# npit/video-learning-tf

Measured on AMD Instinct MI355X. Metric: clips/sec (16-frame 227x227) LRCN train step, higher is better.
Workload: dtype f32; 1 GPU; LRCN AlexNet(fc6)+LSTM(256) 16-frame 227x227x3 clips, 101 classes, UCF-101-shaped synthetic, full train step; global_batch=64, clips_per_gpu=64, frames_per_clip=16, parallelism=dp1, optimizer=sgd+clip_by_global_norm(10), init=reference (sigma 0.05), dist_world_size=1

## Files before the change

### include/vltf.h

```cpp
#ifndef VLTF_H
#define VLTF_H

#include <stddef.h>
#include <stdint.h>

#ifdef __cplusplus
extern "C" {
#endif

typedef void* vl_stream_t;
typedef struct vl_conv_desc vl_conv_desc;

typedef struct vl_step_state {
    int64_t step;
    float lr;
    uint32_t tag_origin;
    float adam_lr;
    uint32_t reserved[3];
} vl_step_state;

const char* vl_last_error(void);
int vl_version(void);
int vl_device_count(void);

int vl_input_prep_u8(const uint8_t* src, float* dst, int n, int raw_h, int raw_w, int out_h, int out_w,
                     const int32_t* crop_y, const int32_t* crop_x, const uint8_t* mirror,
                     const float* mean_bgr, int dst_halo, int dst_phase, vl_stream_t stream);
int vl_nhwc_to_nchw(const float* src, float* dst, int n, int h, int w, int c, int dst_halo, int dst_phase, vl_stream_t stream);
int vl_nchw_to_nhwc(const float* src, float* dst, int n, int c, int h, int w, vl_stream_t stream);

int vl_conv_create(vl_conv_desc** out, int cin, int h, int w, int cout, int kh, int kw, int stride, int groups);
void vl_conv_destroy(vl_conv_desc* d);
int vl_conv_out_hw(const vl_conv_desc* d, int* oh, int* ow);
int vl_conv_set_halo(vl_conv_desc* d, int x_halo, int y_halo, int dy_halo, int dx_halo);
int vl_conv_set_x_phase_split(vl_conv_desc* d, int on);
int vl_conv_x_phase(const vl_conv_desc* d);
int vl_set_conv_math(int math);
int vl_conv_math(void);
int vl_conv_fwd(const vl_conv_desc* d, const float* x, const float* w_hwio, const float* bias, float* y,
                int n, int relu, vl_stream_t stream);
int vl_conv_wt_transpose(const vl_conv_desc* d, const float* w_hwio, float* wt, vl_stream_t stream);
int vl_conv_dgrad(const vl_conv_desc* d, const float* dy, const float* wt, float* dx, const float* relu_mask,
                  int n, vl_stream_t stream);
size_t vl_conv_wgrad_ws_bytes(const vl_conv_desc* d, int n);
int vl_conv_wgrad_fuses_bias(const vl_conv_desc* d);
int vl_conv_wgrad(const vl_conv_desc* d, const float* x, const float* dy, float* dw, float* db, void* ws,
                  size_t ws_bytes, int n, vl_stream_t stream);
size_t vl_c8_bytes(int n, int c, int h, int w, int halo);
int vl_pack_c8(const float* x, void* xb, int n, int c, int h, int w, int x_halo, int xb_halo, vl_stream_t stream);
size_t vl_conv_c8_w_bytes(const vl_conv_desc* d, int bwd);
int vl_conv_c8_pack_w(const vl_conv_desc* d, const float* w_hwio, void* wb, int bwd, vl_stream_t stream);
int vl_conv_c8_fwd(vl_conv_desc* d, const void* xb, const void* wb, const float* bias, float* y, void* yb, int n, int relu,
                   vl_stream_t stream);
int vl_conv_c8_dgrad(vl_conv_desc* d, const void* dyb, const void* wbt, float* dx, void* dxb, const float* relu_mask,
                     const void* relu_mask_c8, int n, vl_stream_t stream);
size_t vl_conv_c8_wgrad_ws_bytes(const vl_conv_desc* d, int n);
int vl_conv_c8_wgrad(vl_conv_desc* d, const void* xb, const void* dyb, float* dw, void* ws, size_t ws_bytes, int n,
                     vl_stream_t stream);
int vl_bias_grad_c8(const void* dyb, float* db, float* ws, int n, int c, int h, int w, int halo, vl_stream_t stream);
int vl_pack_kc8(const float* src, void* dst, int64_t positions, int channels, int64_t pos_stride, int64_t ch_stride, vl_stream_t stream);
size_t vl_gemm_kc8_ws_bytes(int m, int n, int k);
int vl_gemm_kc8(const void* a_kc8, const void* b_kc8, float* c, int m, int n, int k, const float* bias, int relu, void* ws,
                size_t ws_bytes, vl_stream_t stream);
int vl_s2d_c8_from_x0(const vl_conv_desc* d, const float* x0, void* xb, int n, vl_stream_t stream);
int vl_input_prep_u8_s2d(const vl_conv_desc* d, const uint8_t* src, void* xb, int n, int raw_h, int raw_w, const int32_t* crop_y,
                         const int32_t* crop_x, const uint8_t* mirror, const float* mean_bgr, vl_stream_t stream);
int vl_s2d_weights(const vl_conv_desc* d, const float* src, float* dst, int grad, vl_stream_t stream);
int vl_bias_grad_nchw(const float* dy, float* db, float* ws, int n, int c, int hw, vl_stream_t stream);

int vl_lrn_fwd(const float* x, float* y, int n, int c, int hw, int radius, float alpha, float beta, float bias,
               vl_stream_t stream);
int vl_lrn_bwd(const float* x, const float* dy, float* dx, int n, int c, int hw, int radius, float alpha,
               float beta, float bias, int relu_fused, int w, int dx_halo, vl_stream_t stream);

int vl_pool_lrn_bwd(const float* x, const float* dp, const uint8_t* argmax, float* dx, int n, int c, int h, int w,
                    int p_halo, int radius, float alpha, float beta, float bias, int relu_fused, int dx_halo,
                    vl_stream_t stream);

int vl_pool_lrn_bwd_c8(const void* x, int x_packed, const float* dp, const uint8_t* argmax, void* dxb, int n, int c, int h, int w,
                       int p_halo, int radius, float alpha, float beta, float bias, int relu_fused, int dxb_halo, vl_stream_t stream);

int vl_pool_lrn_bwd_test_ranges(int ranges);

int vl_lrn_pool_fwd(const float* x, float* p, uint8_t* argmax, int n, int c, int h, int w, int p_halo, int radius,
                    float alpha, float beta, float bias, vl_stream_t stream);

int vl_lrn_pool_fwd_c8(const void* x, int x_packed, void* pb, uint8_t* argmax, int n, int c, int h, int w, int p_halo, int radius,
                       float alpha, float beta, float bias, vl_stream_t stream);

int vl_maxpool_fwd(const float* x, float* y, uint8_t* argmax, int n, int c, int h, int w, int k, int s,
                   int64_t ys_n, int64_t ys_c, int64_t ys_h, int64_t ys_w, vl_stream_t stream);
int vl_maxpool_bwd(const float* dy, const uint8_t* argmax, float* dx, const float* relu_mask, int n, int c,
                   int h, int w, int k, int s, int64_t ys_n, int64_t ys_c, int64_t ys_h, int64_t ys_w,
                   int dx_halo, vl_stream_t stream);

int vl_gemm(int transa, int transb, int m, int n, int k, const float* a, int64_t lda, const float* b, int64_t ldb,
            float* c, int64_t ldc, const float* bias, int relu, const float* relu_mask, void* ws, size_t ws_bytes,
            vl_stream_t stream);
size_t vl_gemm_split_ws_bytes(int m, int n, int k);
int vl_colsum(const float* a, int64_t lda, float* out, float* ws, int m, int n, vl_stream_t stream);

int vl_lstm_step_fwd(const float* gx, const float* gh, float* act, float* cseq, float* hseq, float* hprev,
                     int batch, int T, int t, int H, float forget_bias, vl_stream_t stream);
int vl_lstm_step_bwd(const float* dout, const float* dh_next, const float* act, const float* cseq, float* dc,
                     float* dz, int batch, int T, int t, int H, vl_stream_t stream);

size_t vl_lstm_seq_ws_bytes(int batch, int T, int H);
int vl_lstm_seq_fwd(const float* gx, const float* kh, const float* h0, const float* c0, float* act, float* cseq, float* hseq,
                    float* hprev, int batch, int T, int H, float forget_bias, void* ws, size_t ws_bytes, vl_stream_t stream);
int vl_lstm_seq_bwd(const float* dout, const float* kh, const float* act, const float* cseq, const float* c0, float* dz,
                    float* dh0, float* dc0, int batch, int T, int H, void* ws, size_t ws_bytes, vl_stream_t stream);
size_t vl_lstm_seq_tag_span(int batch, int T, int H);
int vl_lstm_seq_fwd_st(const float* gx, const float* kh, const float* h0, const float* c0, float* act, float* cseq, float* hseq,
                       float* hprev, int batch, int T, int H, float forget_bias, void* ws, size_t ws_bytes, const vl_step_state* state,
                       uint32_t tag_offset, vl_stream_t stream);
int vl_lstm_seq_bwd_st(const float* dout, const float* kh, const float* act, const float* cseq, const float* c0, float* dz,
                       float* dh0, float* dc0, int batch, int T, int H, void* ws, size_t ws_bytes, const vl_step_state* state,
                       uint32_t tag_offset, vl_stream_t stream);
int vl_lstm_seq_ws_clear(void* ws, size_t ws_bytes, vl_stream_t stream);
int vl_lstm_seq_status(void* ws, int* timed_out);
int vl_lstm_seq_test_hooks(unsigned spin_limit, int mute_workgroup);
int vl_transpose(const float* src, int64_t ld, float* dst, int rows, int cols, vl_stream_t stream);

int vl_temporal_fusion_fwd(const float* x, float* y, int batch, int T, int H, int method, vl_stream_t stream);
int vl_temporal_fusion_bwd(const float* dy, float* dx, int batch, int T, int H, int method, vl_stream_t stream);

typedef struct vl_resize_desc vl_resize_desc;
int vl_resize_create(vl_resize_desc** out, int h, int w, int oh, int ow, int channels);
void vl_resize_destroy(vl_resize_desc* d);
size_t vl_resize_tmp_bytes(const vl_resize_desc* d, int n);
int vl_resize_u8(const vl_resize_desc* d, const uint8_t* src, uint8_t* tmp, uint8_t* dst, int n, vl_stream_t stream);

int vl_copy2d(const float* src, int64_t src_ld, float* dst, int64_t dst_ld, int rows, int cols, vl_stream_t stream);
int vl_eltwise2(const float* a, const float* b, float* out, int64_t count, int op, vl_stream_t stream);
int vl_max2_grad(const float* a, const float* b, const float* d, float* da, float* db, int64_t count, vl_stream_t stream);
int vl_fuse_n(const float* const* ins, int n, float* out, int64_t count, int op, vl_stream_t stream);
int vl_fuse_n_grad(const float* const* ins, int n, const float* d, float* const* dins, int64_t count, int op, vl_stream_t stream);

int vl_dropout_fwd(const float* x, float* y, uint8_t* mask, int64_t count, float keep, uint64_t seed, vl_stream_t stream);
int vl_dropout_bwd(const float* dy, const uint8_t* mask, float* dx, int64_t count, float keep, vl_stream_t stream);
int vl_dropout_fwd_st(const float* x, float* y, uint8_t* mask, int64_t count, float keep, const vl_step_state* state,
                      vl_stream_t stream);

int vl_softmax_xent(const float* logits, const int32_t* labels, float* dlogits, float* stats, float* rows,
                    int batch, int classes, float grad_scale, vl_stream_t stream);

int vl_sumsq(const float* g, int64_t count, float* out, float* ws, int accumulate, vl_stream_t stream);
int vl_sgd_apply(float* w, const float* g, int64_t count, float lr, float clip_norm, const float* sumsq,
                 float gscale, const uint32_t* skip, vl_stream_t stream);
int vl_adam_apply(float* w, const float* g, float* m, float* v, int64_t count, float lr, float clip_norm,
                  const float* sumsq, float gscale, int step, const uint32_t* skip, vl_stream_t stream);
int vl_status_or(uint32_t* dst, const void* lstm_ws, int init, vl_stream_t stream);

size_t vl_step_state_bytes(void);
int vl_step_state_set(vl_step_state* state, int64_t step, float lr, uint32_t tag_origin, vl_stream_t stream);
int vl_sgd_apply_st(float* w, const float* g, int64_t count, const vl_step_state* state, float clip_norm, const float* sumsq,
                    float gscale, const uint32_t* skip, vl_stream_t stream);
int vl_adam_apply_st(float* w, const float* g, float* m, float* v, int64_t count, const vl_step_state* state, float clip_norm,
                     const float* sumsq, float gscale, const uint32_t* skip, vl_stream_t stream);

int vl_fill(float* p, int64_t count, float value, vl_stream_t stream);
int vl_relu_grad(float* d, const float* y, int64_t count, vl_stream_t stream);

#ifdef __cplusplus
}
#endif
#endif
```

### video-learning-tf_amd/_ffi.py

```python
import ctypes as C
import os

_HERE = os.path.dirname(os.path.abspath(__file__))
LIB_PATH = os.environ.get("VLTF_HIP_LIB") or os.path.join(_HERE, "libvltf_hip.so")

p = C.c_void_p
i32, i64, f32, u32, u64, sz = C.c_int, C.c_int64, C.c_float, C.c_uint32, C.c_uint64, C.c_size_t

SIGNATURES = {
    "vl_last_error": (C.c_char_p, []),
    "vl_version": (i32, []),
    "vl_device_count": (i32, []),
    "vl_input_prep_u8": (i32, [p, p, i32, i32, i32, i32, i32, p, p, p, p, i32, i32, p]),
    "vl_nhwc_to_nchw": (i32, [p, p, i32, i32, i32, i32, i32, i32, p]),
    "vl_nchw_to_nhwc": (i32, [p, p, i32, i32, i32, i32, p]),
    "vl_conv_create": (i32, [C.POINTER(p), i32, i32, i32, i32, i32, i32, i32, i32]),
    "vl_conv_destroy": (None, [p]),
    "vl_conv_out_hw": (i32, [p, C.POINTER(i32), C.POINTER(i32)]),
    "vl_conv_set_halo": (i32, [p, i32, i32, i32, i32]),
    "vl_conv_set_x_phase_split": (i32, [p, i32]),
    "vl_conv_x_phase": (i32, [p]),
    "vl_set_conv_math": (i32, [i32]),
    "vl_conv_math": (i32, []),
    "vl_gemm_split_ws_bytes": (C.c_size_t, [i32, i32, i32]),
    "vl_conv_fwd": (i32, [p, p, p, p, p, i32, i32, p]),
    "vl_conv_wt_transpose": (i32, [p, p, p, p]),
    "vl_conv_dgrad": (i32, [p, p, p, p, p, i32, p]),
    "vl_conv_wgrad_ws_bytes": (sz, [p, i32]),
    "vl_conv_wgrad_fuses_bias": (i32, [p]),
    "vl_conv_wgrad": (i32, [p, p, p, p, p, p, sz, i32, p]),
    "vl_c8_bytes": (sz, [i32, i32, i32, i32, i32]),
    "vl_pack_c8": (i32, [p, p, i32, i32, i32, i32, i32, i32, p]),
    "vl_conv_c8_w_bytes": (sz, [p, i32]),
    "vl_conv_c8_pack_w": (i32, [p, p, p, i32, p]),
    "vl_conv_c8_fwd": (i32, [p, p, p, p, p, p, i32, i32, p]),
    "vl_conv_c8_dgrad": (i32, [p, p, p, p, p, p, p, i32, p]),
    "vl_pack_kc8": (i32, [p, p, i64, i32, i64, i64, p]),
    "vl_gemm_kc8_ws_bytes": (sz, [i32, i32, i32]),
    "vl_gemm_kc8": (i32, [p, p, p, i32, i32, i32, p, i32, p, sz, p]),
    "vl_s2d_c8_from_x0": (i32, [p, p, p, i32, p]),
    "vl_input_prep_u8_s2d": (i32, [p, p, p, i32, i32, i32, p, p, p, p, p]),
    "vl_s2d_weights": (i32, [p, p, p, i32, p]),
    "vl_bias_grad_c8": (i32, [p, p, p, i32, i32, i32, i32, i32, p]),
    "vl_conv_c8_wgrad_ws_bytes": (sz, [p, i32]),
    "vl_conv_c8_wgrad": (i32, [p, p, p, p, p, sz, i32, p]),
    "vl_bias_grad_nchw": (i32, [p, p, p, i32, i32, i32, p]),
    "vl_lrn_fwd": (i32, [p, p, i32, i32, i32, i32, f32, f32, f32, p]),
    "vl_lrn_bwd": (i32, [p, p, p, i32, i32, i32, i32, f32, f32, f32, i32, i32, i32, p]),
    "vl_lrn_pool_fwd": (i32, [p, p, p, i32, i32, i32, i32, i32, i32, f32, f32, f32, p]),
    "vl_pool_lrn_bwd": (i32, [p, p, p, p, i32, i32, i32, i32, i32, i32, f32, f32, f32, i32, i32, p]),
    "vl_pool_lrn_bwd_test_ranges": (i32, [i32]),
    "vl_lrn_pool_fwd_c8": (i32, [p, i32, p, p, i32, i32, i32, i32, i32, i32, f32, f32, f32, p]),
    "vl_pool_lrn_bwd_c8": (i32, [p, i32, p, p, p, i32, i32, i32, i32, i32, i32, f32, f32, f32, i32, i32, p]),
    "vl_maxpool_fwd": (i32, [p, p, p, i32, i32, i32, i32, i32, i32, i64, i64, i64, i64, p]),
    "vl_maxpool_bwd": (i32, [p, p, p, p, i32, i32, i32, i32, i32, i32, i64, i64, i64, i64, i32, p]),
    "vl_gemm": (i32, [i32, i32, i32, i32, i32, p, i64, p, i64, p, i64, p, i32, p, p, sz, p]),
    "vl_colsum": (i32, [p, i64, p, p, i32, i32, p]),
    "vl_lstm_step_fwd": (i32, [p, p, p, p, p, p, i32, i32, i32, i32, f32, p]),
    "vl_lstm_step_bwd": (i32, [p, p, p, p, p, p, i32, i32, i32, i32, p]),
    "vl_lstm_seq_ws_bytes": (sz, [i32, i32, i32]),
    "vl_lstm_seq_fwd": (i32, [p, p, p, p, p, p, p, p, i32, i32, i32, f32, p, sz, p]),
    "vl_lstm_seq_bwd": (i32, [p, p, p, p, p, p, p, p, i32, i32, i32, p, sz, p]),
    "vl_lstm_seq_tag_span": (sz, [i32, i32, i32]),
    "vl_lstm_seq_fwd_st": (i32, [p, p, p, p, p, p, p, p, i32, i32, i32, f32, p, sz, p, u32, p]),
    "vl_lstm_seq_bwd_st": (i32, [p, p, p, p, p, p, p, p, i32, i32, i32, p, sz, p, u32, p]),
    "vl_lstm_seq_ws_clear": (i32, [p, sz, p]),
    "vl_lstm_seq_status": (i32, [p, C.POINTER(i32)]),
    "vl_lstm_seq_test_hooks": (i32, [C.c_uint, i32]),
    "vl_transpose": (i32, [p, i64, p, i32, i32, p]),
    "vl_temporal_fusion_fwd": (i32, [p, p, i32, i32, i32, i32, p]),
    "vl_temporal_fusion_bwd": (i32, [p, p, i32, i32, i32, i32, p]),
    "vl_dropout_fwd": (i32, [p, p, p, i64, f32, u64, p]),
    "vl_dropout_bwd": (i32, [p, p, p, i64, f32, p]),
    "vl_dropout_fwd_st": (i32, [p, p, p, i64, f32, p, p]),
    "vl_softmax_xent": (i32, [p, p, p, p, p, i32, i32, f32, p]),
    "vl_sumsq": (i32, [p, i64, p, p, i32, p]),
    "vl_sgd_apply": (i32, [p, p, i64, f32, f32, p, f32, p, p]),
    "vl_adam_apply": (i32, [p, p, p, p, i64, f32, f32, p, f32, i32, p, p]),
    "vl_status_or": (i32, [p, p, i32, p]),
    "vl_step_state_bytes": (sz, []),
    "vl_step_state_set": (i32, [p, i64, f32, u32, p]),
    "vl_sgd_apply_st": (i32, [p, p, i64, p, f32, p, f32, p, p]),
    "vl_adam_apply_st": (i32, [p, p, p, p, i64, p, f32, p, f32, p, p]),
    "vl_fill": (i32, [p, i64, f32, p]),
    "vl_resize_create": (i32, [C.POINTER(p), i32, i32, i32, i32, i32]),
    "vl_resize_destroy": (None, [p]),
    "vl_resize_tmp_bytes": (sz, [p, i32]),
    "vl_resize_u8": (i32, [p, p, p, p, i32, p]),
    "vl_copy2d": (i32, [p, i64, p, i64, i32, i32, p]),
    "vl_eltwise2": (i32, [p, p, p, i64, i32, p]),
    "vl_max2_grad": (i32, [p, p, p, p, p, i64, p]),
    "vl_fuse_n": (i32, [p, i32, p, i64, i32, p]),
    "vl_fuse_n_grad": (i32, [p, i32, p, p, i64, i32, p]),
    "vl_relu_grad": (i32, [p, p, i64, p]),
}


class VltfError(RuntimeError):
    pass


_lib = None


def lib():
    global _lib
    if _lib is None:
        if not os.path.exists(LIB_PATH):
            raise VltfError("libvltf_hip.so not found at %s -- build it with "
                            "`python -c 'import __graft_entry__ as g; g.build()'` "
                            "(there is no CPU fallback)" % LIB_PATH)
        import torch
        tl = os.path.join(os.path.dirname(torch.__file__), "lib", "libamdhip64.so")
        if os.path.exists(tl):
            C.CDLL(tl, mode=C.RTLD_GLOBAL)
        try:
            l = C.CDLL(LIB_PATH)
        except OSError as ex:
            raise VltfError("cannot load %s: %s" % (LIB_PATH, ex))
        for name, (res, args) in SIGNATURES.items():
            try:
                fn = getattr(l, name)
            except AttributeError:
                raise VltfError("libvltf_hip.so does not export %s (stale build?)" % name)
            fn.restype = res
            fn.argtypes = args
        _lib = l
    return _lib


def check(rc, what):
    if rc != 0:
        msg = lib().vl_last_error()
        raise VltfError("%s failed (rc=%d): %s" % (what, rc, msg.decode() if msg else "?"))


def call(name, *args):
    check(getattr(lib(), name)(*args), name)
```

### video-learning-tf_amd/csrc/conv_desc.h

```cpp
#pragma once
#include <hip/hip_runtime.h>
#include <stdint.h>

struct vl_conv_desc {
    int cin, h, w, cout, kh, kw, stride, groups;
    int oh, ow, pt, pl, pb, pr;
    int cig, cog;
    int K;
    int Kd;
    int x_halo, y_halo, dy_halo, dx_halo;
    int x_phase;
    int2* ktab2_fwd;
    int* ktab_fwd;
    int2* ptab2_fwd;
    int2* ptab2_bwd;
    int* ptab_fwd;
    int* ptab_bwd;
    int* rowtab_fwd;
    int* rowtab_bwd;
    int fwd_padded, bwd_padded;
    uint32_t* wsplit_fwd;
    uint32_t* wsplit_bwd;
    int* c8_toff_fwd;
    int* c8_toff_bwd;
};

void conv_c8_free_tables(vl_conv_desc* d);
int conv_c8_build_tables(vl_conv_desc* d);
```

### video-learning-tf_amd/csrc/mfma_gemm.hip

```cpp
#include <stdlib.h>
#include <string.h>

#include "common.h"
#include "conv_desc.h"

typedef float f32x16 __attribute__((ext_vector_type(16)));
typedef const __attribute__((address_space(4))) int* const_int_ptr;
__device__ __forceinline__ const_int_ptr as_const(const int* p) { return (const_int_ptr)(uintptr_t)p; }
static constexpr int NT = 256;
static constexpr int KBLK = 16;

static constexpr uint32_t OOB_OFF = 0xF0000000u;
static constexpr int64_t MAX_BUF_BYTES = 0xE0000000ll;

__device__ __forceinline__ __amdgpu_buffer_rsrc_t make_rsrc(const float* base, int64_t bytes) {
    return __builtin_amdgcn_make_buffer_rsrc(const_cast<float*>(base), 0, (int)(uint32_t)bytes, 0x00020000);
}
__device__ __forceinline__ float buf_load(__amdgpu_buffer_rsrc_t r, uint32_t voff, int soff) {
    return __builtin_bit_cast(float, __builtin_amdgcn_raw_buffer_load_b32(r, (int)voff, soff, 0));
}

template <int BX, int BR>
struct LdsTile {
    static constexpr int STR = BR + 2;
// ... 565 lines not shown
}
struct SplitBf16 {
    i32x4 p[3];
};
template <int NPC>
__device__ __forceinline__ void split_pieces(float x0, float x1, int (&out)[3]) {
    f32x2 r = {x0, x1};
#pragma unroll
    for (int k = 0; k < NPC; ++k) {
        const uint32_t h = __builtin_bit_cast(uint32_t, __builtin_convertvector(r, bf16x2));
        out[k] = (int)h;
        if (k + 1 < NPC) r = f32x2{r[0] - __uint_as_float(h << 16), r[1] - __uint_as_float(h & 0xffff0000u)};
    }
}
__device__ constexpr int kProdA[6] = {0, 0, 1, 1, 0, 2};
__device__ constexpr int kProdB[6] = {0, 1, 0, 1, 2, 0};
constexpr int split_products(int math) { return math == 6 ? 6 : math == 3 ? 3 : 1; }
constexpr int split_pieces_of(int math) { return math == 6 ? 3 : math == 3 ? 2 : 1; }
__device__ __forceinline__ f32x16 mfma_bf16(const i32x4& a, const i32x4& b, const f32x16& c) {
    return __builtin_amdgcn_mfma_f32_32x32x16_bf16(__builtin_bit_cast(bf16x8, a), __builtin_bit_cast(bf16x8, b), c, 0, 0, 0);
}

template <int BN, int WM, int WN, int MATH = 0, bool X4 = false>
__global__ __launch_bounds__(NT, 1) void wgrad_dma_kernel(const ConvGeom g, const DyParams d, const EpiRowMajor::Params pe,
                                                          int tiles_i, int tiles_j, int groups, int units, int rtiles,
                                                          int rt_per_split, float* db_slabs, int db_stride) {
    using C = WgradDmaCfg<BN>;
    constexpr int BM = C::BM, STR = C::STR, SA = BM * STR, BUF = C::BUF;
    constexpr int TM = BM / WM / 32, TN = BN / WN / 32;
    constexpr int RA = BM / 4, RB = BN / 4;
    static_assert(WM * WN == 4 && TM * WM * 32 == BM && TN * WN * 32 == BN, "tile shape");
    static_assert(RA + RB <= 10 * 2 * TM * TN, "row fetches must leave the last third of a tile's MFMAs to cover their latency");
    static_assert(!X4 || (MATH != 0 && BN == 128 && BM == 128), "the 16-byte fetch form: split-product modes, 128 x 128 tiles");
    constexpr int GSTR = 258, SA4 = 32 * GSTR, BUF4 = 64 * GSTR;
    extern __shared__ __attribute__((aligned(16))) float ldsw[];

    const int tiles = tiles_i * tiles_j;
    const int k8 = blockIdx.x >> 3;
    const int unit = (k8 / tiles) * 8 + (blockIdx.x & 7);
    if (unit >= units) return;
    const int tile_id = k8 % tiles;
    const int ti_blk = tile_id % tiles_i, tj_blk = tile_id / tiles_i;
    const int zg = unit % groups, zs = unit / groups;
    const int i0 = ti_blk * BM, j0 = tj_blk * BN;
    const int lane = threadIdx.x & 63;
    const int wave = __builtin_amdgcn_readfirstlane(threadIdx.x >> 6);
    const int wi0 = (wave / WN) * (BM / WM), wj0 = (wave % WN) * (BN / WN);

    const i32x4 rs_x = rsrc_words(g.x + (int64_t)zg * g.grp_stride, (g.total - (int64_t)zg * g.grp_stride) * 4);
    const int64_t goff = (int64_t)zg * d.Cog * d.plane;
    const i32x4 rs_dy = rsrc_words(d.dy + goff, (d.total - goff) * 4);
    const int* tab = g.ktab + i0 + wave * RA;
    const uint32_t lds0 = (uint32_t)(uintptr_t)(__attribute__((address_space(3))) float*)ldsw;
    const int row_bytes = (int)(d.plane * 4);
    const int b_row0 = j0 + wave * RB;
    const int b_last = d.Cog - 1;
    const int64_t dy_img = (int64_t)d.Cout_total * d.plane;

    uint32_t voff_x, voff_dy;
    auto decode = [&](int rt) __attribute__((always_inline)) {
        const int m = X4 ? rt * 64 + 4 * (lane & 15) : rt * 64 + lane;
        const bool vm = m < g.M;
        const uint32_t mm = vm ? m : 0;
        const uint32_t n = fd_div(mm, g.dOHW);
        const uint32_t p = mm - n * g.OHW;
        const uint32_t oh = fd_div(p, g.dOW);
        const uint32_t ow = p - oh * g.OW;
        const int ih0 = (int)oh * g.stride - g.pt + g.halo, iw0 = (int)ow * g.col_mul + g.col_add;
        const uint32_t vx = (uint32_t)((int64_t)n * g.img_stride + (int64_t)ih0 * g.Wp + iw0) * 4u;
        const uint32_t vd = (uint32_t)((int64_t)n * dy_img + (int64_t)(oh + d.halo) * d.OWp + ow + d.halo) * 4u;
        voff_x = vm ? vx : OOB_OFF;
        voff_dy = vm ? vd : OOB_OFF;
        asm volatile("" : "+v"(voff_x), "+v"(voff_dy));
    };
    int tabv[RA];
    auto load_table = [&](int rt) __attribute__((always_inline)) {
        const const_int_ptr tt = (const_int_ptr)(uintptr_t)(tab + rt * g.zero);
#pragma unroll
        for (int f = 0; f < RA; ++f) tabv[f] = tt[f];
    };
    auto pin_table = [&]() __attribute__((always_inline)) {
#pragma unroll
        for (int f = 0; f < RA; ++f) asm volatile("" : "+s"(tabv[f]));
    };
    auto dma = [&](const int nb, const int f, int rt_next) __attribute__((always_inline)) {
        const int z = rt_next * g.zero;
        if (f < RA) {
            const uint32_t la = lds0 + (uint32_t)(wave * (RA * STR) + z) * 4u;
            lds_dma_row(rs_x, la + (uint32_t)(nb * BUF + f * STR) * 4u, voff_x, tabv[f]);
        } else {
            const int r = f - RA;
            const uint32_t lb = lds0 + (uint32_t)(SA + wave * (RB * STR) + z) * 4u;
            lds_dma_row(rs_dy, lb + (uint32_t)(nb * BUF + r * STR) * 4u, voff_dy, min(b_row0 + z + r, b_last) * row_bytes);
        }
    };
    uint32_t vrow_a[8], vrow_b[8];
    if constexpr (X4) {
#pragma unroll
        for (int j = 0; j < 8; ++j) {
            const int rl = wave * 8 + j + 32 * (lane >> 4);
            vrow_a[j] = i0 + rl < g.K ? (uint32_t)g.ktab[i0 + rl] : OOB_OFF;
            vrow_b[j] = j0 + rl < d.Cog ? (uint32_t)(j0 + rl) * (uint32_t)row_bytes : OOB_OFF;
        }
    }
    auto dma_x4 = [&](const int nb, const int f, int rt_next) __attribute__((always_inline)) {
        const int z = rt_next * g.zero;
        if (f < 8) {
            const uint32_t vo = (vrow_a[f] == OOB_OFF || voff_x == OOB_OFF) ? OOB_OFF : vrow_a[f] + voff_x;
            lds_dma_row4(rs_x, lds0 + (uint32_t)(nb * BUF4 + (wave * 8 + f) * GSTR + z) * 4u, vo, 0);
        } else {
            const uint32_t vo = (vrow_b[f - 8] == OOB_OFF || voff_dy == OOB_OFF) ? OOB_OFF : vrow_b[f - 8] + voff_dy;
            lds_dma_row4(rs_dy, lds0 + (uint32_t)(nb * BUF4 + SA4 + (wave * 8 + f - 8) * GSTR + z) * 4u, vo, 0);
        }
    };
    const int ones_row = (db_slabs != nullptr && g.K >= i0 && g.K < i0 + BM) ? g.K - i0 : -1;
    auto finish_tile = [&](const int nb) __attribute__((always_inline)) {
        asm volatile("s_waitcnt vmcnt(0)" ::: "memory");
        if constexpr (X4) {
            if (ones_row >= 0 && ((ones_row & 31) >> 3) == wave) ldsw[nb * BUF4 + (ones_row & 31) * GSTR + (ones_row >> 5) * 64 + lane] = 1.0f;
        } else {
            if (ones_row >= 0 && (ones_row / RA) == wave) ldsw[nb * BUF + ones_row * STR + lane] = 1.0f;
        }
        __syncthreads();
    };

    f32x16 acc[TM][TN];
#pragma unroll
    for (int a = 0; a < TM; ++a)
#pragma unroll
        for (int b = 0; b < TN; ++b)
#pragma unroll
            for (int q = 0; q < 16; ++q) acc[a][b][q] = 0.f;

    const int rt0 = zs * rt_per_split;
    const int rt1 = min(rtiles, rt0 + rt_per_split);
    const int ntiles = rt1 - rt0;
    if (ntiles > 0) {
        decode(rt0);
        load_table(rt0);
        pin_table();
        if constexpr (X4) {
#pragma unroll
            for (int f = 0; f < 16; ++f) dma_x4(0, f, rt0);
        } else {
#pragma unroll
            for (int f = 0; f < RA + RB; ++f) dma(0, f, rt0);
        }
        decode(rt0 + 1);
        finish_tile(0);
    }
    const float* fa = ldsw + (wi0 + (lane & 31)) * STR + 2 * (lane >> 5);
    const float* fb = ldsw + SA + (wj0 + (lane & 31)) * STR + 2 * (lane >> 5);

    auto tile = [&](const int cur, int rt_next) __attribute__((always_inline)) {
        float2 af[2][TM], bf[2][TN];
#pragma unroll
        for (int a = 0; a < TM; ++a) af[0][a] = *reinterpret_cast<const float2*>(fa + cur * BUF + a * 32 * STR);
#pragma unroll
        for (int b = 0; b < TN; ++b) bf[0][b] = *reinterpret_cast<const float2*>(fb + cur * BUF + b * 32 * STR);
#pragma unroll
        for (int t = 0; t < 16; ++t) {
            const int c = t & 1, nx = c ^ 1;
            if (t + 1 < 16) {
#pragma unroll
                for (int a = 0; a < TM; ++a) af[nx][a] = *reinterpret_cast<const float2*>(fa + cur * BUF + a * 32 * STR + 4 * (t + 1));
#pragma unroll
                for (int b = 0; b < TN; ++b) bf[nx][b] = *reinterpret_cast<const float2*>(fb + cur * BUF + b * 32 * STR + 4 * (t + 1));
            }
#pragma unroll
            for (int m = 0; m < 2 * TM * TN; ++m) {
                const int a = (m % (TM * TN)) / TN, b = m % TN;
                if (m < TM * TN) acc[a][b] = __builtin_amdgcn_mfma_f32_32x32x2f32(af[c][a].x, bf[c][b].x, acc[a][b], 0, 0, 0);
                else acc[a][b] = __builtin_amdgcn_mfma_f32_32x32x2f32(af[c][a].y, bf[c][b].y, acc[a][b], 0, 0, 0);
                const int f = t * (2 * TM * TN) + m;
                if (f < RA + RB) {
                    dma(cur ^ 1, f, rt_next);
                    __builtin_amdgcn_sched_barrier(0);
                }
            }
            if (t == 10) {
                load_table(rt_next + 1);
                __builtin_amdgcn_sched_barrier(0);
            }
            if (t == 13) {
                int rtn = rt_next + 1;
                asm volatile("" : "+s"(rtn));
                decode(rtn);
                pin_table();
                __builtin_amdgcn_sched_barrier(0);
            }
        }
        finish_tile(cur ^ 1);
    };
    const float* fa3 = ldsw + (wi0 + (lane & 31)) * STR + 8 * (lane >> 5);
    const float* fb3 = ldsw + SA + (wj0 + (lane & 31)) * STR + 8 * (lane >> 5);
    auto tile_split = [&](const int cur, int rt_next) __attribute__((always_inline)) {
        constexpr int NP = split_products(MATH), NPC = split_pieces_of(MATH);
        constexpr int NMS = NP * TM * TN, NTOT = 4 * NMS, NF = X4 ? 16 : RA + RB;
        constexpr int FSPAN = NTOT >= 28 ? NTOT - 14 : NTOT / 2;
        constexpr int FPM = (NF + FSPAN - 1) / FSPAN, FEND = (NF + FPM - 1) / FPM;
        constexpr int LT = FEND > NTOT - 12 ? FEND : NTOT - 12;
        constexpr int PIN = LT + 2 > NTOT - 6 ? LT + 2 : NTOT - 6;
        static_assert(PIN < NTOT, "the tile must leave room to load and pin the next table");
        SplitBf16 As[2][TM], Bs[2][TN];
        auto load_split = [&](const int st, SplitBf16 (&A)[TM], SplitBf16 (&B)[TN]) __attribute__((always_inline)) {
#pragma unroll
            for (int a = 0; a < TM; ++a)
#pragma unroll
                for (int q = 0; q < 4; ++q) {
                    const float2 v = X4 ? *reinterpret_cast<const float2*>(ldsw + cur * BUF4 + (lane & 31) * GSTR + (wi0 / 32 + a) * 64 + 16 * st +
                                                                            8 * (lane >> 5) + 2 * q)
                                        : *reinterpret_cast<const float2*>(fa3 + cur * BUF + a * 32 * STR + 16 * st + 2 * q);
                    int pc[3] = {0, 0, 0};
                    split_pieces<NPC>(v.x, v.y, pc);
#pragma unroll
                    for (int k = 0; k < NPC; ++k) A[a].p[k][q] = pc[k];
                }
#pragma unroll
            for (int b = 0; b < TN; ++b)
#pragma unroll
                for (int q = 0; q < 4; ++q) {
                    const float2 v = X4 ? *reinterpret_cast<const float2*>(ldsw + cur * BUF4 + SA4 + (lane & 31) * GSTR + (wj0 / 32 + b) * 64 +
                                                                            16 * st + 8 * (lane >> 5) + 2 * q)
                                        : *reinterpret_cast<const float2*>(fb3 + cur * BUF + b * 32 * STR + 16 * st + 2 * q);
                    int pc[3] = {0, 0, 0};
                    split_pieces<NPC>(v.x, v.y, pc);
#pragma unroll
                    for (int k = 0; k < NPC; ++k) B[b].p[k][q] = pc[k];
                }
        };
        load_split(0, As[0], Bs[0]);
        static_for<0, 4>([&](auto SI) __attribute__((always_inline)) {
            constexpr int st = decltype(SI)::value, c = st & 1;
            if constexpr (st + 1 < 4) load_split(st + 1, As[c ^ 1], Bs[c ^ 1]);
            static_for<0, NMS>([&](auto MI) __attribute__((always_inline)) {
                constexpr int m = decltype(MI)::value;
                constexpr int prod = m / (TM * TN), a = (m % (TM * TN)) / TN, b = m % TN;
                acc[a][b] = mfma_bf16(As[c][a].p[kProdA[prod]], Bs[c][b].p[kProdB[prod]], acc[a][b]);
                constexpr int idx = st * NMS + m;
                static_for<0, FPM>([&](auto EI) __attribute__((always_inline)) {
                    constexpr int f = idx * FPM + decltype(EI)::value;
                    if constexpr (f < NF) {
                        if constexpr (X4) dma_x4(cur ^ 1, f, rt_next);
                        else dma(cur ^ 1, f, rt_next);
                    }
                });
                __builtin_amdgcn_sched_barrier(0x106);
                if constexpr (idx == LT) load_table(rt_next + 1);
                if constexpr (idx == PIN) {
                    int rtn = rt_next + 1;
                    asm volatile("" : "+s"(rtn));
                    decode(rtn);
                    pin_table();
                }
            });
        });
        finish_tile(cur ^ 1);
    };
    auto run_tile = [&](const int cur, int rt_next) __attribute__((always_inline)) {
        if constexpr (MATH != 0) tile_split(cur, rt_next);
        else tile(cur, rt_next);
    };
    int rt = rt0;
    for (int i = 0; i + 1 < ntiles; i += 2, rt += 2) {
        run_tile(0, rt + 1);
        run_tile(1, rt + 2);
    }
    if (ntiles > 0 && (ntiles & 1)) run_tile(0, rt + 1);

    EpiRowMajor::template apply<TM, TN>(pe, zg, zs, i0 + wi0, j0 + wj0, acc);
    if (ones_row >= 0) {
        float* dbs = db_slabs + (int64_t)zs * db_stride + zg * d.Cog;
        const int lr = ones_row - wi0;
        if (lr >= 0 && lr < BM / WM) {
            const int a = lr >> 5, rr = lr & 31;
            const int q = (rr & 3) + 4 * (rr >> 3);
            if (((rr >> 2) & 1) == (lane >> 5)) {
#pragma unroll
                for (int b = 0; b < TN; ++b) {
                    const int j = j0 + wj0 + 32 * b + (lane & 31);
                    float v = 0.f;
#pragma unroll
                    for (int aa = 0; aa < TM; ++aa)
#pragma unroll
                        for (int qq = 0; qq < 16; ++qq)
                            if (aa == a && qq == q) v = acc[aa][b][qq];
                    if (j < d.Cog) dbs[j] = v;
                }
            }
        }
    }
}

typedef float f32x4 __attribute__((ext_vector_type(4)));
typedef float f32x4u __attribute__((ext_vector_type(4), aligned(4)));

struct ConvDmaParams {
    const float* w;
    int64_t w_ld;
    int64_t w_grp_stride;
    int64_t w_bytes;
    const int* row_tab;
    int nblk;
};

template <int SR>
__global__ __launch_bounds__(NT, 64 / SR) void conv_dma_kernel(const ConvDmaParams pa, const ConvGeom g, const EpiConvNCHW::Params pe,
                                                               int tiles_i, int wide) {
    constexpr int BM = 128, BN = 128;
    constexpr int ABUF = SR * BM, BUF = SR * (BM + BN);
    constexpr int RW = SR / 4;
    constexpr int NF = RW * 4;
    constexpr int NT2 = SR / 4;
    constexpr int FPM = 1;
    static_assert(SR == 64 || SR == 32, "stage depth");
    extern __shared__ __attribute__((aligned(16))) float ldsc[];
    const int bid = xcd_swizzle(blockIdx.x, gridDim.x);
    const int ti_blk = bid % tiles_i, tj_blk = bid / tiles_i;
    const int zg = blockIdx.y;
    const int i0 = ti_blk * BM, j0 = tj_blk * BN;
    const int lane = threadIdx.x & 63;
    const int wave = __builtin_amdgcn_readfirstlane(threadIdx.x >> 6);
    const int wm = wave >> 1, wn = wave & 1;

    const i32x4 rs_w = rsrc_words(pa.w + (int64_t)zg * pa.w_grp_stride, pa.w_bytes - (int64_t)zg * pa.w_grp_stride * 4);
    const i32x4 rs_x = rsrc_words(g.x + (int64_t)zg * g.grp_stride, (g.total - (int64_t)zg * g.grp_stride) * 4);
    uint32_t voff_a[2], voff_b[2];
#pragma unroll
    for (int hf = 0; hf < 2; ++hf) {
        const int co = i0 + hf * 64 + lane;
        voff_a[hf] = co < pe.Cog ? (uint32_t)co * 4u : OOB_OFF;
        const int m = j0 + hf * 64 + lane;
        const bool vm = m < g.M;
        const uint32_t mm = vm ? m : 0;
        const uint32_t n = fd_div(mm, g.dOHW);
        const uint32_t p = mm - n * g.OHW;
        const uint32_t oh = fd_div(p, g.dOW);
        const uint32_t ow = p - oh * g.OW;
        const int ih0 = (int)oh * g.stride - g.pt + g.halo, iw0 = (int)ow * g.col_mul + g.col_add;
        voff_b[hf] = vm ? (uint32_t)((int64_t)n * g.img_stride + (int64_t)ih0 * g.Wp + iw0) * 4u : OOB_OFF;
    }
    const uint32_t lds0 = (uint32_t)(uintptr_t)(__attribute__((address_space(3))) float*)ldsc;
    const int ld_bytes = (int)(pa.w_ld * 4);

    int tabv[RW];
    int row0 = 0;
    bool blk_ok = false;
    const int wrow = wave * RW;
    auto load_table = [&](int st) {
        const int k0 = st * SR + wrow;
        const const_int_ptr tt = as_const(g.ktab) + k0 + st * g.zero;
#pragma unroll
        for (int f = 0; f < RW; ++f) tabv[f] = tt[f];
        row0 = as_const(pa.row_tab)[k0 / KBLK + st * g.zero] + k0 % KBLK;
        blk_ok = k0 / KBLK < pa.nblk;
    };
    auto pin_table = [&]() {
#pragma unroll
        for (int f = 0; f < RW; ++f) asm volatile("" : "+s"(tabv[f]));
        asm volatile("" : "+s"(row0));
    };
    auto dma = [&](const int nb, const int f, int st) {
        const int rr = f >> 2, kind = f & 3, hf = kind & 1;
        const int z = st * g.zero;
        const uint32_t row_lds = lds0 + (uint32_t)(nb * BUF + (wrow + rr) * 128 + hf * 64 + z) * 4u;
        const bool live = blk_ok && st * SR + wrow + rr < g.K;
        if (kind < 2) lds_dma_row(rs_w, row_lds, voff_a[hf], min(row0 + rr, g.K - 1) * ld_bytes);
        else lds_dma_row(rs_x, row_lds + ABUF * 4u, live ? voff_b[hf] : OOB_OFF, tabv[rr]);
    };
    int a_soff = 0;
    auto dma_fast = [&](const int nb, const int f, int st) {
        const int rr = f >> 2, kind = f & 3, hf = kind & 1;
        const uint32_t row_lds = lds0 + (uint32_t)(nb * BUF + (wrow + rr) * 128 + hf * 64 + st * g.zero) * 4u;
        if (f == 0) a_soff = row0 * ld_bytes;
        if (kind < 2) lds_dma_row(rs_w, row_lds, voff_a[hf], a_soff);
        else lds_dma_row(rs_x, row_lds + ABUF * 4u, voff_b[hf], tabv[rr]);
        if (kind == 1) a_soff += ld_bytes;
    };
    auto finish_stage = [&]() {
        asm volatile("s_waitcnt vmcnt(0)" ::: "memory");
        __syncthreads();
    };

    f32x16 acc[2][2];
#pragma unroll
    for (int a = 0; a < 2; ++a)
#pragma unroll
        for (int b = 0; b < 2; ++b)
#pragma unroll
            for (int q = 0; q < 16; ++q) acc[a][b][q] = 0.f;

    const int nstages = (pa.nblk * KBLK + SR - 1) / SR;
    load_table(0);
    pin_table();
#pragma unroll
    for (int f = 0; f < NF; ++f) dma(0, f, 0);
    load_table(1);
    pin_table();
    finish_stage();

    float bias_r[2][16];
#pragma unroll
    for (int a = 0; a < 2; ++a)
#pragma unroll
        for (int q = 0; q < 16; ++q) {
            const int co = i0 + wm * 64 + 2 * ((q & 3) + 8 * (q >> 2) + 4 * (lane >> 5)) + a;
            bias_r[a][q] = (pe.bias && co < pe.Cog) ? pe.bias[zg * pe.Cog + co] : 0.f;
        }

    const float* fa = ldsc + (lane >> 5) * 128 + wm * 64 + 2 * (lane & 31);
    const float* fb = ldsc + ABUF + (lane >> 5) * 128 + wn * 64 + (lane & 31);

    auto stage = [&](const int cur, const bool fast, int st_next) {
        float2 af[2], bf[2], an[2], bn[2];
        auto read_b = [&](int step) {
            const float* q = fb + cur * BUF + step * 256;
            return float2{q[0], q[32]};
        };
        af[0] = *reinterpret_cast<const float2*>(fa + cur * BUF);
        bf[0] = read_b(0);
        af[1] = *reinterpret_cast<const float2*>(fa + cur * BUF + 256);
        bf[1] = read_b(1);
#pragma unroll
        for (int t = 0; t < NT2; ++t) {
            if (t + 1 < NT2) {
#pragma unroll
                for (int u = 0; u < 2; ++u) {
                    an[u] = *reinterpret_cast<const float2*>(fa + cur * BUF + (2 * (t + 1) + u) * 256);
                    bn[u] = read_b(2 * (t + 1) + u);
                }
            }
#pragma unroll
            for (int m = 0; m < 8; ++m) {
                const int u = m >> 2, a = (m >> 1) & 1, b = m & 1;
                acc[a][b] = __builtin_amdgcn_mfma_f32_32x32x2f32(a ? af[u].y : af[u].x, b ? bf[u].y : bf[u].x, acc[a][b], 0, 0, 0);
                const int f = (t * 8 + m) * FPM;
                if (f < NF) {
#pragma unroll
                    for (int e = 0; e < FPM; ++e) {
                        if (fast) dma_fast(cur ^ 1, f + e, st_next);
                        else dma(cur ^ 1, f + e, st_next);
                    }
                    __builtin_amdgcn_sched_barrier(0);
                }
            }
            static_assert(NF / FPM / 8 <= NT2 - 4, "fetches must end before the table is replaced");
            if (t == NT2 - 4) {
                load_table(st_next + 1);
                __builtin_amdgcn_sched_barrier(0);
            }
            if (t == NT2 - 2) {
                pin_table();
                __builtin_amdgcn_sched_barrier(0);
            }
#pragma unroll
            for (int u = 0; u < 2; ++u) {
                af[u] = an[u];
                bf[u] = bn[u];
            }
        }
        finish_stage();
    };
    const int nfull = g.K / SR;
    int st = 0;
    for (; st + 2 < nfull; st += 2) {
        stage(0, true, st + 1);
        stage(1, true, st + 2);
    }
    for (; st < nstages; ++st) {
        if (st & 1) stage(1, false, st + 1);
        else stage(0, false, st + 1);
    }

    if (wide) {
        constexpr int SP = BN + 4;
        float* T = ldsc;
#pragma unroll
        for (int b = 0; b < 2; ++b)
#pragma unroll
            for (int a = 0; a < 2; ++a)
#pragma unroll
                for (int q = 0; q < 16; ++q) {
                    const int i = (q & 3) + 8 * (q >> 2) + 4 * (lane >> 5);
                    float v = acc[a][b][q] + bias_r[a][q];
                    if (pe.relu) v = fmaxf(v, 0.f);
                    T[(wm * 64 + 2 * i + a) * SP + wn * 64 + 32 * b + (lane & 31)] = v;
                }
        __syncthreads();
        const int px = 4 * (lane & 31);
        const int m = j0 + px;
        const uint32_t n = fd_div((uint32_t)min(m, pe.M - 1), pe.dOHW);
        const int p = m - (int)n * pe.OHW;
        const bool run4 = m + 3 < pe.M && p + 3 < pe.OHW;
        const int64_t cbase = ((int64_t)n * pe.Cout_total + (int64_t)zg * pe.Cog) * pe.y_plane + p;
#pragma unroll
        for (int i = 0; i < BM / 8; ++i) {
            const int cl = wave * (BM / 4) + 2 * i + (lane >> 5);
            const int co = i0 + cl;
            const f32x4 v = *reinterpret_cast<const f32x4*>(T + cl * SP + px);
            if (co >= pe.Cog) continue;
            float* dst = pe.y + cbase + (int64_t)co * pe.y_plane;
            if (run4) {
                *reinterpret_cast<f32x4u*>(dst) = v;
            } else {
#pragma unroll
                for (int e = 0; e < 4; ++e) {
                    const int me = m + e;
                    if (me < pe.M) {
                        const uint32_t ne = fd_div((uint32_t)me, pe.dOHW);
                        const int pe_ = me - (int)ne * pe.OHW;
                        pe.y[((int64_t)ne * pe.Cout_total + (int64_t)zg * pe.Cog + co) * pe.y_plane + pe_] = v[e];
                    }
                }
            }
        }
        return;
    }
#pragma unroll
    for (int b = 0; b < 2; ++b) {
        const int m = j0 + wn * 64 + 32 * b + (lane & 31);
        if (m >= pe.M) continue;
        const uint32_t n = fd_div((uint32_t)m, pe.dOHW);
        const uint32_t p = m - n * pe.OHW;
        const uint32_t oh = fd_div(p, pe.dOW);
        const uint32_t ow = p - oh * pe.OW;
        const int64_t c0 = (int64_t)n * pe.Cout_total + (int64_t)zg * pe.Cog;
        const int64_t ybase = c0 * pe.y_plane + (int64_t)(oh + pe.y_halo) * pe.y_wp + ow + pe.y_halo;
        const int64_t mbase = c0 * pe.m_plane + (int64_t)(oh + pe.m_halo) * pe.m_wp + ow + pe.m_halo;
#pragma unroll
        for (int a = 0; a < 2; ++a) {
            float mk[16];
            if (pe.mask) {
#pragma unroll
                for (int q = 0; q < 16; ++q) {
                    const int co = i0 + wm * 64 + 2 * ((q & 3) + 8 * (q >> 2) + 4 * (lane >> 5)) + a;
                    mk[q] = co < pe.Cog ? pe.mask[mbase + (int64_t)co * pe.m_plane] : 0.f;
                }
            }
#pragma unroll
            for (int q = 0; q < 16; ++q) {
                const int i = (q & 3) + 8 * (q >> 2) + 4 * (lane >> 5);
                const int co = i0 + wm * 64 + 2 * i + a;
                if (co < pe.Cog) {
                    float v = acc[a][b][q] + bias_r[a][q];
                    if (pe.relu) v = fmaxf(v, 0.f);
                    if (pe.mask) v = mk[q] > 0.f ? v : 0.f;
                    pe.y[ybase + (int64_t)co * pe.y_plane] = v;
                }
            }
        }
    }
}


__global__ void conv_wsplit_kernel(const float* __restrict__ w, int64_t w_ld, int64_t w_grp_stride, const int* __restrict__ row_tab,
                                   int K, int Cog, int CogP, int nstages, int planes, uint32_t* __restrict__ out) {
    const int st = blockIdx.x, zg = blockIdx.y;
    const int row0 = row_tab[st];
    uint32_t* o = out + ((int64_t)zg * nstages + st) * planes * 8 * CogP;
    for (int idx = threadIdx.x; idx < 8 * CogP; idx += blockDim.x) {
        const int q = idx & 3, co = (idx >> 2) % CogP, h = idx / (4 * CogP);
        const int r = 8 * h + 2 * q, p = st * 16 + r;
        float x0 = 0.f, x1 = 0.f;
        if (co < Cog) {
            const float* src = w + (int64_t)(row0 + r) * w_ld + zg * w_grp_stride + co;
            if (p < K) x0 = src[0];
            if (p + 1 < K) x1 = src[w_ld];
        }
        int pc[3] = {0, 0, 0};
        split_pieces<3>(x0, x1, pc);
        for (int k = 0; k < planes; ++k) o[(int64_t)((2 * k + h) * CogP + co) * 4 + q] = (uint32_t)pc[k];
    }
}

struct ConvRingParams {
    const uint32_t* wsplit;
    int CogP;
    int nstages;
};

template <int MATH, int BM>
__global__ __launch_bounds__(512, 1) void conv_ring_kernel(const ConvRingParams pa, const ConvGeom g, const EpiConvNCHW::Params pe,
                                                           int tiles_i, int OWp, int Mp, FastDiv dOHWp, FastDiv dOWp) {
    constexpr int BN = BM == 128 ? 256 : 512, SR = 16, NBUF = BM == 128 ? 5 : 4;
    constexpr int NH = BN / 256;
    static_assert(BM == 128 || BM == 64, "channel tile");
    constexpr int NPL = MATH == 6 ? 3 : 2;
    constexpr int ABUF = NPL * 8 * BM, BUF = ABUF + SR * BN;
    constexpr int NAF = (NPL * 2 * (BM / 64) + 7) / 8;
    constexpr int FW = NAF + 2 * NH;
    constexpr int VMW = (NBUF - 3) * FW;
    constexpr int NP = split_products(MATH), NPC = split_pieces_of(MATH);
    constexpr int NM = (BM / 32) * (BN / 256) * NP;
    static_assert(SR == KBLK, "one stage = one block of the reduction order");
    extern __shared__ __attribute__((aligned(16))) float ldsr[];
    const int bid = xcd_swizzle(blockIdx.x, gridDim.x);
    const int ti_blk = bid % tiles_i, tj_blk = bid / tiles_i;
    const int zg = blockIdx.y;
    const int i0 = ti_blk * BM, j0 = tj_blk * BN;
    const int lane = threadIdx.x & 63;
    const int wave = __builtin_amdgcn_readfirstlane(threadIdx.x >> 6);
    constexpr int TA = BM / 32, TB = BN / 8 / 32, WPX = 32 * TB;
    const int OHWp = g.OHW / g.OW * OWp;
    const int nstages = pa.nstages;

    const int64_t stage_dw = (int64_t)NPL * 8 * pa.CogP;
    const uint32_t* wbase = pa.wsplit + (int64_t)zg * nstages * stage_dw;
    const i32x4 rs_w = rsrc_words(reinterpret_cast<const float*>(wbase), nstages * stage_dw * 4);
    constexpr int NPIECE = NPL * 2 * (BM / 64);
    int piece[NAF];
    uint32_t voff_a[NAF];
#pragma unroll
    for (int e = 0; e < NAF; ++e) {
        piece[e] = e == 0 ? wave % NPIECE : 8 + (wave & 3);
        voff_a[e] = BM == 128 ? (uint32_t)(((piece[e] >> 1) * pa.CogP + i0 + (piece[e] & 1) * 64 + lane) * 16)
                              : (uint32_t)((piece[e] * pa.CogP + i0 + lane) * 16);
    }
    const int stage_bytes = (int)(stage_dw * 4);
    const i32x4 rs_x = rsrc_words(g.x + (int64_t)zg * g.grp_stride, (g.total - (int64_t)zg * g.grp_stride) * 4);
    uint32_t voff_b[NH];
#pragma unroll
    for (int hf = 0; hf < NH; ++hf) {
        const int m = j0 + 256 * hf + 4 * lane;
        const bool vm = m < Mp;
        const uint32_t mm = vm ? m : 0;
        const uint32_t n = fd_div(mm, dOHWp);
        const uint32_t p = mm - n * OHWp;
        const uint32_t oh = fd_div(p, dOWp);
        const uint32_t ow = p - oh * OWp;
        const int ih0 = (int)oh * g.stride - g.pt + g.halo, iw0 = (int)ow * g.col_mul + g.col_add;
        voff_b[hf] = vm ? (uint32_t)((int64_t)n * g.img_stride + (int64_t)ih0 * g.Wp + iw0) * 4u : OOB_OFF;
    }
    const uint32_t lds0 = (uint32_t)(uintptr_t)(__attribute__((address_space(3))) float*)ldsr;

    int tab0 = 0, tab1 = 0;
    const int wrow = wave * 2;
    auto load_table = [&](int st) __attribute__((always_inline)) {
        const int sc = min(st, nstages - 1) + st * g.zero;
        const const_int_ptr tt = as_const(g.ktab) + sc * SR + wrow;
        tab0 = tt[0];
        tab1 = tt[1];
    };
    auto pin_table = [&]() __attribute__((always_inline)) {
        asm volatile("" : "+s"(tab0));
        asm volatile("" : "+s"(tab1));
    };
    auto dma = [&](const uint32_t wr, const int f, int st) __attribute__((always_inline)) {
        if (f < NAF) {
            lds_dma_row4(rs_w, lds0 + wr + (uint32_t)piece[f] * 1024u, voff_a[f], st * stage_bytes);
        } else {
            const int r = (f - NAF) / NH, hf = (f - NAF) % NH;
            const bool live = st * SR + wrow + r < g.K;
            lds_dma_row4(rs_x, lds0 + wr + (uint32_t)(ABUF + (wrow + r) * BN + 256 * hf) * 4u, live ? voff_b[hf] : OOB_OFF,
                         r == 0 ? tab0 : tab1);
        }
    };
    auto dma_fast = [&](const uint32_t wr, const int f, int st) __attribute__((always_inline)) {
        if (f < NAF) {
            lds_dma_row4(rs_w, lds0 + wr + (uint32_t)piece[f] * 1024u, voff_a[f], st * stage_bytes);
        } else {
            const int r = (f - NAF) / NH, hf = (f - NAF) % NH;
            lds_dma_row4(rs_x, lds0 + wr + (uint32_t)(ABUF + (wrow + r) * BN + 256 * hf) * 4u, voff_b[hf], r == 0 ? tab0 : tab1);
        }
    };

    f32x16 acc[TA][TB];
#pragma unroll
    for (int a = 0; a < TA; ++a)
#pragma unroll
        for (int b = 0; b < TB; ++b)
#pragma unroll
            for (int q = 0; q < 16; ++q) acc[a][b][q] = 0.f;

    const float* fa = ldsr + ((lane >> 5) * BM + (lane & 31)) * 4;
    const float* fb = ldsr + ABUF + (lane >> 5) * 8 * BN + wave * WPX + (lane & 31);
    struct Raw {
        float b[TB][8];
    };
    auto load_raw = [&](int rd, Raw& r) __attribute__((always_inline)) {
#pragma unroll
        for (int j = 0; j < 8; ++j) {
            const float* q = fb + rd + j * BN;
#pragma unroll
            for (int b = 0; b < TB; ++b) r.b[b][j] = q[32 * b];
        }
    };
    auto load_a = [&](int rd, SplitBf16 (&A)[TA]) __attribute__((always_inline)) {
#pragma unroll
        for (int a = 0; a < TA; ++a) {
#pragma unroll
            for (int k = 0; k < NPC; ++k) A[a].p[k] = *reinterpret_cast<const i32x4*>(fa + rd + k * 2 * BM * 4 + a * 32 * 4);
        }
    };
    auto split = [&](const Raw& r, SplitBf16 (&B)[TB]) __attribute__((always_inline)) {
#pragma unroll
        for (int j = 0; j < 4; ++j)
#pragma unroll
            for (int b = 0; b < TB; ++b) {
                int pc[3] = {0, 0, 0};
                split_pieces<NPC>(r.b[b][2 * j], r.b[b][2 * j + 1], pc);
#pragma unroll
                for (int k = 0; k < NPC; ++k) B[b].p[k][j] = pc[k];
            }
    };

    for (int s0 = 0; s0 < NBUF; ++s0) {
        load_table(s0);
        pin_table();
        if (s0 < nstages) {
#pragma unroll
            for (int f = 0; f < FW; ++f) dma((uint32_t)(s0 * BUF * 4), f, s0);
        }
    }
    load_table(NBUF);
    pin_table();
    if (nstages >= NBUF) asm volatile("s_waitcnt vmcnt(%0)" ::"n"(VMW) : "memory");
    else asm volatile("s_waitcnt vmcnt(0)" ::: "memory");
    __syncthreads();
    SplitBf16 A[TA] = {}, B[TB] = {}, An[TA] = {}, Bn[TB] = {};
    Raw R0 = {}, R1 = {};
    load_a(0, A);
    load_raw(0, R0);
    load_raw(BUF, R1);
    split(R0, B);
    asm volatile("s_waitcnt lgkmcnt(0)" ::: "memory");
    __syncthreads();

    int rda = BUF, rdb = 2 * BUF;
    uint32_t wr = 0;
    constexpr int D = NBUF;
    auto stage = [&](const bool fast, int st, SplitBf16 (&Ac)[TA], SplitBf16 (&Bc)[TB], SplitBf16 (&An)[TA], SplitBf16 (&Bn)[TB],
                     const Raw& Rc, Raw& Rn) __attribute__((always_inline)) {
        load_a(rda, An);
        load_raw(rdb, Rn);
        static_for<0, (NM > FW ? NM : FW)>([&](auto MI) __attribute__((always_inline)) {
            constexpr int m = decltype(MI)::value;
            if constexpr (m < NM) {
                constexpr int prod = m / (TA * TB), a = (m % (TA * TB)) / TB, b = m % TB;
                acc[a][b] = mfma_bf16(Ac[a].p[kProdA[prod]], Bc[b].p[kProdB[prod]], acc[a][b]);
            }
            if constexpr (m < FW) {
                if (fast) dma_fast(wr, m, st + D);
                else if (st + D < nstages) dma(wr, m, st + D);
            }
            __builtin_amdgcn_sched_barrier(0x106);
        });
        split(Rc, Bn);
        load_table(st + D + 1);
        pin_table();
        rda = rda + BUF == NBUF * BUF ? 0 : rda + BUF;
        rdb = rdb + BUF == NBUF * BUF ? 0 : rdb + BUF;
        wr = wr + BUF * 4 == NBUF * BUF * 4 ? 0u : wr + BUF * 4;
    };
    auto finish = [&](int st) __attribute__((always_inline)) {
        const int after = min(st + D, nstages - 1) - (st + 3);
        if (after >= 2 && NBUF - 3 >= 2) asm volatile("s_waitcnt vmcnt(%0) lgkmcnt(0)" ::"n"(2 * FW) : "memory");
        else if (after >= 1) asm volatile("s_waitcnt vmcnt(%0) lgkmcnt(0)" ::"n"(FW) : "memory");
        else asm volatile("s_waitcnt vmcnt(0) lgkmcnt(0)" ::: "memory");
        __syncthreads();
    };
    const int nfull = g.K / SR;
    int st = 0;
    for (; st + 1 + D < nfull; st += 2) {
        stage(true, st, A, B, An, Bn, R1, R0);
        asm volatile("s_waitcnt vmcnt(%0) lgkmcnt(0)" ::"n"(VMW) : "memory");
        __syncthreads();
        stage(true, st + 1, An, Bn, A, B, R0, R1);
        asm volatile("s_waitcnt vmcnt(%0) lgkmcnt(0)" ::"n"(VMW) : "memory");
        __syncthreads();
    }
    for (; st < nstages; st += 2) {
        stage(false, st, A, B, An, Bn, R1, R0);
        finish(st);
        if (st + 1 < nstages) {
            stage(false, st + 1, An, Bn, A, B, R0, R1);
            finish(st + 1);
        }
    }

#pragma unroll
    for (int b = 0; b < TB; ++b) {
        const int m = j0 + wave * WPX + 32 * b + (lane & 31);
        if (m >= Mp) continue;
        const uint32_t n = fd_div((uint32_t)m, dOHWp);
        const uint32_t p = m - n * OHWp;
        const uint32_t oh = fd_div(p, dOWp);
        const uint32_t ow = p - oh * OWp;
        if ((int)ow >= pe.OW) continue;
        const int64_t c0 = (int64_t)n * pe.Cout_total + (int64_t)zg * pe.Cog;
        const int64_t ybase = c0 * pe.y_plane + (int64_t)(oh + pe.y_halo) * pe.y_wp + ow + pe.y_halo;
        const int64_t mbase = c0 * pe.m_plane + (int64_t)(oh + pe.m_halo) * pe.m_wp + ow + pe.m_halo;
#pragma unroll
        for (int a = 0; a < TA; ++a) {
#pragma unroll
            for (int q = 0; q < 16; ++q) {
                const int i = (q & 3) + 8 * (q >> 2) + 4 * (lane >> 5);
                const int co = i0 + 32 * a + i;
                if (co < pe.Cog) {
                    float v = acc[a][b][q];
                    if (pe.bias) v += pe.bias[zg * pe.Cog + co];
                    if (pe.relu) v = fmaxf(v, 0.f);
                    if (pe.mask) v = pe.mask[mbase + (int64_t)co * pe.m_plane] > 0.f ? v : 0.f;
                    pe.y[ybase + (int64_t)co * pe.y_plane] = v;
                }
            }
        }
    }
}

template <int MATH>
__global__ __launch_bounds__(256, 2) void conv_ring4_kernel(const ConvRingParams pa, const ConvGeom g, const EpiConvNCHW::Params pe,
                                                            int tiles_i, int OWp, int Mp, FastDiv dOHWp, FastDiv dOWp) {
    constexpr int BM = 128, BN = 256, SR = 16, NBUF = 3, D = 3;
    constexpr int ABUF = SR * BM, BUF = SR * (BM + BN);
    constexpr int TA = 4, TB = 2, WPX = 64;
    constexpr int FW = 6;
    constexpr int NP = split_products(MATH), NPC = split_pieces_of(MATH);
    static_assert(NPC <= 2, "the two-workgroup form has LDS for two weight planes");
    constexpr int NM = TA * TB * NP;
    static_assert(SR == KBLK, "one stage = one block of the reduction order");
    extern __shared__ __attribute__((aligned(16))) float ldsq[];
    const int bid = xcd_swizzle(blockIdx.x, gridDim.x);
    const int ti_blk = bid % tiles_i, tj_blk = bid / tiles_i;
    const int zg = blockIdx.y;
    const int i0 = ti_blk * BM, j0 = tj_blk * BN;
    const int lane = threadIdx.x & 63;
// ... 31 lines not shown
#pragma unroll
        for (int r = 0; r < 4; ++r) tab[r] = tt[r];
    };
    auto pin_table = [&]() __attribute__((always_inline)) {
#pragma unroll
        for (int r = 0; r < 4; ++r) asm volatile("" : "+s"(tab[r]));
    };
    auto dma = [&](const uint32_t wr, const int f, int st, const bool fast) __attribute__((always_inline)) {
        if (f < 2) {
            lds_dma_row4(rs_w, lds0 + wr + (uint32_t)(2 * wave + f) * 1024u, voff_a[f], st * stage_bytes);
        } else {
            const int r = f - 2;
            const bool live = fast || st * SR + wrow + r < g.K;
            lds_dma_row4(rs_x, lds0 + wr + (uint32_t)(ABUF + (wrow + r) * BN) * 4u, live ? voff_b : OOB_OFF, tab[r]);
        }
    };

    f32x16 acc[TA][TB];
#pragma unroll
    for (int a = 0; a < TA; ++a)
#pragma unroll
        for (int b = 0; b < TB; ++b)
#pragma unroll
            for (int q = 0; q < 16; ++q) acc[a][b][q] = 0.f;

    const float* fa = ldsq + ((lane >> 5) * BM + (lane & 31)) * 4;
    const float* fb = ldsq + ABUF + (lane >> 5) * 8 * BN + wave * WPX + (lane & 31);
    auto load_ops = [&](int rd, SplitBf16 (&A)[TA], float (&rb)[TB][8]) __attribute__((always_inline)) {
#pragma unroll
        for (int a = 0; a < TA; ++a) {
#pragma unroll
            for (int k = 0; k < NPC; ++k) A[a].p[k] = *reinterpret_cast<const i32x4*>(fa + rd + k * 2 * BM * 4 + a * 32 * 4);
        }
#pragma unroll
        for (int j = 0; j < 8; ++j)
#pragma unroll
            for (int b = 0; b < TB; ++b) rb[b][j] = fb[rd + j * BN + 32 * b];
    };
    auto split = [&](const float (&rb)[TB][8], SplitBf16 (&B)[TB]) __attribute__((always_inline)) {
#pragma unroll
        for (int j = 0; j < 4; ++j)
#pragma unroll
            for (int b = 0; b < TB; ++b) {
                int pc[3] = {0, 0, 0};
                split_pieces<NPC>(rb[b][2 * j], rb[b][2 * j + 1], pc);
#pragma unroll
                for (int k = 0; k < NPC; ++k) B[b].p[k][j] = pc[k];
            }
    };

    for (int s0 = 0; s0 < NBUF; ++s0) {
        load_table(s0);
        pin_table();
        if (s0 < nstages) {
#pragma unroll
            for (int f = 0; f < FW; ++f) dma((uint32_t)(s0 * BUF * 4), f, s0, false);
        }
    }
    load_table(NBUF);
    pin_table();
    if (nstages >= NBUF) asm volatile("s_waitcnt vmcnt(%0)" ::"n"(2 * FW) : "memory");
    else asm volatile("s_waitcnt vmcnt(0)" ::: "memory");
    __syncthreads();
    SplitBf16 A[TA] = {}, B[TB] = {}, An[TA] = {}, Bn[TB] = {};
    {
        float rb[TB][8];
        load_ops(0, A, rb);
        split(rb, B);
    }
    if (nstages >= NBUF) asm volatile("s_waitcnt vmcnt(%0) lgkmcnt(0)" ::"n"(FW) : "memory");
    else asm volatile("s_waitcnt vmcnt(0) lgkmcnt(0)" ::: "memory");
    __syncthreads();

    int rd = BUF;
    uint32_t wr = 0;
    auto stage = [&](const bool fast, int st, SplitBf16 (&Ac)[TA], SplitBf16 (&Bc)[TB], SplitBf16 (&An)[TA], SplitBf16 (&Bn)[TB])
                     __attribute__((always_inline)) {
        float rb[TB][8];
        load_ops(rd, An, rb);
        static_assert(NM >= FW, "a fetch rides on each of the first FW MFMAs");
        static_for<0, NM>([&](auto MI) __attribute__((always_inline)) {
            constexpr int m = decltype(MI)::value;
            constexpr int prod = m / (TA * TB), a = (m % (TA * TB)) / TB, b = m % TB;
            acc[a][b] = mfma_bf16(Ac[a].p[kProdA[prod]], Bc[b].p[kProdB[prod]], acc[a][b]);
            if constexpr (m < FW) {
                if (fast || st + D < nstages) dma(wr, m, st + D, fast);
            }
            __builtin_amdgcn_sched_barrier(0x106);
        });
        split(rb, Bn);
        load_table(st + D + 1);
        pin_table();
        rd = rd + BUF == NBUF * BUF ? 0 : rd + BUF;
        wr = wr + BUF * 4 == NBUF * BUF * 4 ? 0u : wr + BUF * 4;
    };
    auto finish = [&](int st) __attribute__((always_inline)) {
        if (min(st + D, nstages - 1) - (st + 2) >= 1) asm volatile("s_waitcnt vmcnt(%0) lgkmcnt(0)" ::"n"(FW) : "memory");
        else asm volatile("s_waitcnt vmcnt(0) lgkmcnt(0)" ::: "memory");
        __syncthreads();
    };
    const int nfull = g.K / SR;
    int st = 0;
    for (; st + 1 + D < nfull; st += 2) {
        stage(true, st, A, B, An, Bn);
        asm volatile("s_waitcnt vmcnt(%0) lgkmcnt(0)" ::"n"(FW) : "memory");
        __syncthreads();
        stage(true, st + 1, An, Bn, A, B);
        asm volatile("s_waitcnt vmcnt(%0) lgkmcnt(0)" ::"n"(FW) : "memory");
        __syncthreads();
    }
    for (; st < nstages; st += 2) {
        stage(false, st, A, B, An, Bn);
        finish(st);
        if (st + 1 < nstages) {
            stage(false, st + 1, An, Bn, A, B);
            finish(st + 1);
        }
    }

#pragma unroll
    for (int b = 0; b < TB; ++b) {
        const int m = j0 + wave * WPX + 32 * b + (lane & 31);
        if (m >= Mp) continue;
        const uint32_t n = fd_div((uint32_t)m, dOHWp);
        const uint32_t p = m - n * OHWp;
        const uint32_t oh = fd_div(p, dOWp);
        const uint32_t ow = p - oh * OWp;
        if ((int)ow >= pe.OW) continue;
        const int64_t c0 = (int64_t)n * pe.Cout_total + (int64_t)zg * pe.Cog;
        const int64_t ybase = c0 * pe.y_plane + (int64_t)(oh + pe.y_halo) * pe.y_wp + ow + pe.y_halo;
        const int64_t mbase = c0 * pe.m_plane + (int64_t)(oh + pe.m_halo) * pe.m_wp + ow + pe.m_halo;
#pragma unroll
        for (int a = 0; a < TA; ++a) {
#pragma unroll
            for (int q = 0; q < 16; ++q) {
                const int i = (q & 3) + 8 * (q >> 2) + 4 * (lane >> 5);
                const int co = i0 + 32 * a + i;
                if (co < pe.Cog) {
                    float v = acc[a][b][q];
                    if (pe.bias) v += pe.bias[zg * pe.Cog + co];
                    if (pe.relu) v = fmaxf(v, 0.f);
                    if (pe.mask) v = pe.mask[mbase + (int64_t)co * pe.m_plane] > 0.f ? v : 0.f;
                    pe.y[ybase + (int64_t)co * pe.y_plane] = v;
                }
            }
        }
    }
}

template <int WAYS>
__global__ __launch_bounds__(256) void reduce_slabs_kernel(const float* __restrict__ ws, float* __restrict__ out, int64_t count, int splits,
                                                          int64_t slab_stride, const float* __restrict__ bias, int ncols, int64_t ldc,
                                                          int relu, const float* __restrict__ mask) {
    __shared__ float part[3][64];
    const int lane = threadIdx.x & 63, w = threadIdx.x >> 6;
    constexpr int EPB = WAYS == 4 ? 64 : 256;
    const int per = WAYS == 4 ? (splits + 3) >> 2 : splits;
    const int z0 = WAYS == 4 ? w * per : 0, z1 = min(splits, z0 + per);
    for (int64_t e0 = (int64_t)blockIdx.x * EPB; e0 < count; e0 += (int64_t)gridDim.x * EPB) {
        const int64_t e = e0 + (WAYS == 4 ? lane : (int)threadIdx.x);
        float s = 0.f;
        if (e < count) {
            const float* p = ws + (int64_t)z0 * slab_stride + e;
            int z = z0;
            for (; z + 4 <= z1; z += 4, p += 4 * slab_stride) {
                const float a = p[0], b = p[slab_stride], c = p[2 * slab_stride], d = p[3 * slab_stride];
                s += a; s += b; s += c; s += d;
            }
            for (; z < z1; ++z, p += slab_stride) s += p[0];
        }
        if constexpr (WAYS == 4) {
            if (w > 0) part[w - 1][lane] = s;
            __syncthreads();
            if (w == 0) s = (s + part[0][lane]) + (part[1][lane] + part[2][lane]);
        }
        if ((WAYS == 1 || w == 0) && e < count) {
            int64_t o = e;
            if (ncols > 0) {
                const int64_t row = e / ncols;
                const int col = (int)(e - row * ncols);
                if (bias) s += bias[col];
                o = row * ldc + col;
            }
            if (relu) s = fmaxf(s, 0.f);
            if (mask) s = mask[o] > 0.f ? s : 0.f;
            out[o] = s;
        }
        if constexpr (WAYS == 4) __syncthreads();
    }
}

static void launch_reduce_slabs(hipStream_t s, const float* ws, float* out, int64_t count, int splits, int64_t slab_stride, const float* bias,
                                int ncols, int64_t ldc, int relu, const float* mask) {
    static const int force = vl_exp_env("VL_REDUCE_WAYS") ? atoi(vl_exp_env("VL_REDUCE_WAYS")) : 0;
    const bool four = force ? force == 4 : (splits >= 16 && count * 4 <= (int64_t)splits * 65536);
    if (four) {
        const int blocks = (int)((count + 63) / 64 < 16384 ? (count + 63) / 64 : 16384);
        hipLaunchKernelGGL(reduce_slabs_kernel<4>, dim3(blocks), dim3(256), 0, s, ws, out, count, splits, slab_stride, bias, ncols, ldc, relu, mask);
    } else {
        const int blocks = (int)((count + 255) / 256 < 4096 ? (count + 255) / 256 : 4096);
        hipLaunchKernelGGL(reduce_slabs_kernel<1>, dim3(blocks), dim3(256), 0, s, ws, out, count, splits, slab_stride, bias, ncols, ldc, relu, mask);
    }
}

static const bool kConvStaged = vl_exp_env("VL_CONV_STAGED") != nullptr;
static const bool kGemmNoSplit = vl_exp_env("VL_GEMM_NOSPLIT") != nullptr;
static const bool kConvNoWideStore = vl_exp_env("VL_CONV_NO_WIDE_STORE") != nullptr;
static const bool kConvNoTailSplit = vl_exp_env("VL_CONV_NO_TAIL_SPLIT") != nullptr;
static const bool kConvNoLoadPick = vl_exp_env("VL_CONV_NO_LOAD_PICK") != nullptr;
static const bool kWgradDword = vl_exp_env("VL_WGRAD_DWORD") != nullptr;
static const bool kRing8 = vl_exp_env("VL_CONV_RING8") != nullptr;

static int g_conv_math = [] {
    const char* e = vl_exp_env("VL_CONV_MATH");
    return e == nullptr ? 0 : strcmp(e, "bf16x3") == 0 ? 3 : strcmp(e, "bf16x6") == 0 ? 6 : strcmp(e, "bf16") == 0 ? 1 : 0;
}();

extern "C" int vl_set_conv_math(int math) {
    VL_CHECK(math == 0 || math == 1 || math == 3 || math == 6, "vl_set_conv_math: 0 (fp32), 1 (bf16), 3 (bf16x3) or 6 (bf16x6)");
    g_conv_math = math;
    return 0;
}

extern "C" int vl_conv_math(void) { return g_conv_math; }


static void tf_same_pad(int in, int k, int s, int* out, int* before, int* after) {
    *out = (in + s - 1) / s;
    int total = (*out - 1) * s + k - in;
    if (total < 0) total = 0;
    *before = total / 2;
    *after = total - *before;
}


static void k_to_row(int k, int kh, int kw, int cg, bool permuted, int* ky, int* kx, int* c) {
    if (permuted) {
        const int cl = k % KBLK, t = k / KBLK;
        *kx = t % kw;
        *ky = (t / kw) % kh;
        *c = (t / (kw * kh)) * KBLK + cl;
    } else {
        *c = k % cg;
        *kx = (k / cg) % kw;
        *ky = k / (cg * kw);
    }
}

static void free_dev(void* p) {
    if (p) (void)hipFree(p);
}

template <class T>
static int upload(T** dev, const T* host, size_t count) {
    free_dev(*dev);
    *dev = nullptr;
    hipError_t e = hipMalloc((void**)dev, sizeof(T) * count);
    if (e == hipSuccess) e = hipMemcpy(*dev, host, sizeof(T) * count, hipMemcpyHostToDevice);
    return e == hipSuccess ? 0 : 2;
}

static int build_ktabs(int** dev1, int2** dev2, int** rowtab, int kh, int kw, int cg, int H, int W, int halo, bool permuted,
                       int phase = 1, int col_shift = 0) {
    const int K = kh * kw * cg;
    const int pad = ((K + 127) / 128) * 128 + 256;
    const int Wp = phase > 1 ? (W + 2 * halo + phase - 1) / phase : W + 2 * halo;
    const int64_t Pp = (int64_t)(H + 2 * halo) * Wp;
    const int ntiles = pad / KBLK;
    int* h1 = (int*)malloc(sizeof(int) * pad);
    int2* h2 = (int2*)malloc(sizeof(int2) * pad);
    int* h3 = (int*)malloc(sizeof(int) * ntiles);
    if (!h1 || !h2 || !h3) {
        free(h1);
        free(h2);
        free(h3);
        return 1;
    }
    for (int k = 0; k < pad; ++k) {
        if (k < K) {
            int ky, kx, c;
            k_to_row(k, kh, kw, cg, permuted, &ky, &kx, &c);
            int64_t off = ((int64_t)c * Pp + (int64_t)ky * Wp + kx) * 4;
            if (phase > 1) off = (((int64_t)c * phase + (kx + col_shift) % phase) * Pp + (int64_t)ky * Wp + (kx + col_shift) / phase) * 4;
            h1[k] = (int)off;
            h2[k].x = (int)off;
            h2[k].y = (ky << 16) | kx;
            if (k % KBLK == 0) h3[k / KBLK] = (ky * kw + kx) * cg + c;
        } else {
            h1[k] = 0;
            h2[k].x = 0;
            h2[k].y = 0x4000 << 16;
            if (k % KBLK == 0) h3[k / KBLK] = 0;
        }
    }
    int rc = upload(dev1, h1, pad);
    if (rc == 0) rc = upload(dev2, h2, pad);
    if (rc == 0 && rowtab) rc = upload(rowtab, h3, ntiles);
    free(h1);
    free(h2);
    free(h3);
    return rc;
}

static int rebuild_tables(vl_conv_desc* d) {
    d->fwd_padded = d->x_halo >= d->pt && d->x_halo >= d->pb && d->x_halo >= d->pl && d->x_halo >= d->pr;
    if (!d->fwd_padded) d->x_phase = 1;
    const int ph = d->x_phase > 1 ? d->x_phase : 1, shift = d->x_halo - d->pl;
    int rc = build_ktabs(&d->ktab_fwd, &d->ktab2_fwd, nullptr, d->kh, d->kw, d->cig, d->h, d->w, d->x_halo, false, ph, shift);
    if (rc == 0)
        rc = build_ktabs(&d->ptab_fwd, &d->ptab2_fwd, &d->rowtab_fwd, d->kh, d->kw, d->cig, d->h, d->w, d->x_halo, d->cig % KBLK == 0, ph,
                         shift);
    if (rc == 0 && d->stride == 1) {
        rc = build_ktabs(&d->ptab_bwd, &d->ptab2_bwd, &d->rowtab_bwd, d->kh, d->kw, d->cog, d->oh, d->ow, d->dy_halo, d->cog % KBLK == 0);
        const int need = (d->kh - 1 - d->pt > d->pt ? d->kh - 1 - d->pt : d->pt);
        const int needw = (d->kw - 1 - d->pl > d->pl ? d->kw - 1 - d->pl : d->pl);
        d->bwd_padded = d->dy_halo >= need && d->dy_halo >= needw;
    }
    if (rc == 0) rc = conv_c8_build_tables(d);
    return rc;
}

extern "C" int vl_conv_create(vl_conv_desc** out, int cin, int h, int w, int cout, int kh, int kw, int stride, int groups) {
    VL_CHECK(out, "vl_conv_create: null out");
    VL_CHECK(cin > 0 && cout > 0 && h > 0 && w > 0 && kh > 0 && kw > 0 && stride > 0 && groups > 0, "vl_conv_create: bad geometry");
    VL_CHECK(cin % groups == 0 && cout % groups == 0, "vl_conv_create: channels not divisible by groups");
    VL_CHECK(h < 0x4000 && w < 0x4000 && kh < 256 && kw < 256, "vl_conv_create: plane too large");
    vl_conv_desc* d = (vl_conv_desc*)calloc(1, sizeof(vl_conv_desc));
    VL_CHECK(d, "vl_conv_create: out of host memory");
    d->cin = cin; d->h = h; d->w = w; d->cout = cout; d->kh = kh; d->kw = kw; d->stride = stride; d->groups = groups;
    tf_same_pad(h, kh, stride, &d->oh, &d->pt, &d->pb);
    tf_same_pad(w, kw, stride, &d->ow, &d->pl, &d->pr);
    d->cig = cin / groups;
    d->cog = cout / groups;
    d->K = kh * kw * d->cig;
    d->Kd = kh * kw * d->cog;
    const size_t sf = (size_t)groups * ceil_div(d->K, KBLK) * 24 * (ceil_div(d->cog, 128) * 128) * 4;
    const size_t sb = (size_t)groups * ceil_div(d->Kd, KBLK) * 24 * (ceil_div(d->cig, 128) * 128) * 4;
    const bool images = sf <= (64u << 20) && sb <= (64u << 20);
    if (rebuild_tables(d) || (images && (hipMalloc((void**)&d->wsplit_fwd, sf) != hipSuccess || hipMalloc((void**)&d->wsplit_bwd, sb) != hipSuccess))) {
        vl_conv_destroy(d);
        vl_set_error("vl_conv_create: device table allocation failed");
        return 2;
    }
    *out = d;
    return 0;
}

extern "C" int vl_conv_set_halo(vl_conv_desc* d, int x_halo, int y_halo, int dy_halo, int dx_halo) {
    VL_CHECK(d, "vl_conv_set_halo: null descriptor");
    VL_CHECK(x_halo >= 0 && y_halo >= 0 && dy_halo >= 0 && dx_halo >= 0 && x_halo < 64 && y_halo < 64 && dy_halo < 64 && dx_halo < 64,
             "vl_conv_set_halo: bad halo");
    d->x_halo = x_halo; d->y_halo = y_halo; d->dy_halo = dy_halo; d->dx_halo = dx_halo;
    VL_CHECK(rebuild_tables(d) == 0, "vl_conv_set_halo: device table allocation failed");
    return 0;
}

extern "C" int vl_conv_set_x_phase_split(vl_conv_desc* d, int on) {
    VL_CHECK(d, "vl_conv_set_x_phase_split: null descriptor");
    VL_CHECK(!on || d->fwd_padded, "vl_conv_set_x_phase_split: needs the padded x layout (set the halo first)");
    d->x_phase = (on && d->stride > 1) ? d->stride : 1;
    VL_CHECK(rebuild_tables(d) == 0, "vl_conv_set_x_phase_split: device table allocation failed");
    return 0;
}

extern "C" int vl_conv_x_phase(const vl_conv_desc* d) { return d && d->x_phase > 1 ? d->x_phase : 1; }

extern "C" void vl_conv_destroy(vl_conv_desc* d) {
    if (!d) return;
    free_dev(d->ktab_fwd);
    free_dev(d->ktab2_fwd);
    free_dev(d->ptab_fwd);
    free_dev(d->ptab2_fwd);
    free_dev(d->ptab_bwd);
    free_dev(d->ptab2_bwd);
    free_dev(d->rowtab_fwd);
    free_dev(d->rowtab_bwd);
    free_dev(d->wsplit_fwd);
    free_dev(d->wsplit_bwd);
    conv_c8_free_tables(d);
    free(d);
}

extern "C" int vl_conv_out_hw(const vl_conv_desc* d, int* oh, int* ow) {
    VL_CHECK(d, "vl_conv_out_hw: null descriptor");
    if (oh) *oh = d->oh;
    if (ow) *ow = d->ow;
    return 0;
}

struct ConvOut {
    float* y;
    const float* bias;
    const float* mask;
    int relu;
    int y_halo, m_halo, OH, OW;
};

template <int BM, int WM, int WN, bool PADDED>
static int launch_conv(const ConvGeom& g, const float* w, int64_t w_ld, int w_grp_stride, const int* row_tab, int Cog,
                       int Cout_total, const ConvOut& o, hipStream_t s) {
    constexpr int BN = 128, BR = KBLK;
    using LA = ConvWeightKX<BM, BR>;
    using LB = ConvGather<BN, BR, PADDED>;
    typename LA::Params pa{w, w_ld, Cog, g.K, (int64_t)w_grp_stride, row_tab};
    EpiConvNCHW::Params pe;
    pe.y = o.y; pe.bias = o.bias; pe.mask = o.mask; pe.relu = o.relu;
    pe.Cog = Cog; pe.Cout_total = Cout_total; pe.OHW = g.OHW; pe.OW = g.OW; pe.M = g.M;
    pe.dOHW = g.dOHW; pe.dOW = g.dOW;
    pe.y_halo = o.y_halo; pe.y_wp = o.OW + 2 * o.y_halo; pe.y_plane = (int64_t)(o.OH + 2 * o.y_halo) * pe.y_wp;
    pe.m_halo = o.m_halo; pe.m_wp = o.OW + 2 * o.m_halo; pe.m_plane = (int64_t)(o.OH + 2 * o.m_halo) * pe.m_wp;
    const int tiles_i = ceil_div(Cog, BM), tiles_j = ceil_div(g.M, BN);
    const int rtiles = ceil_div(g.K, BR);
    dim3 grid(tiles_i * tiles_j, (unsigned)(Cout_total / Cog), 1);
    hipLaunchKernelGGL((mfma_contract<BM, BN, BR, WM, WN, LA, LB, EpiConvNCHW>), grid, dim3(NT), 0, s, pa, g, pe,
                       tiles_i, rtiles, rtiles);
    VL_LAUNCH_CHECK();
    return 0;
}


template <int TA>
__global__ __launch_bounds__(NT, 2) void conv_dma16_kernel(const ConvDmaParams pa, const ConvGeom g, const EpiConvNCHW::Params pe,
                                                           int tiles_i, int wide) {
    constexpr int BM = 16 * TA, BN = 128, SR = 32;
    constexpr int NA = (BM + 63) / 64;
    constexpr int SA = NA * 64 + 16, SB = 144;
    constexpr int ABUF = SR * SA, BUF = SR * (SA + SB);
    constexpr int RW = SR / 4, FPR = NA + 2, NF = RW * FPR, NSTEP = SR / 4;
    constexpr int NM = 2 * TA;
    extern __shared__ __attribute__((aligned(16))) float ldsc[];
    const int bid = xcd_swizzle(blockIdx.x, gridDim.x);
    const int ti_blk = bid % tiles_i, tj_blk = bid / tiles_i;
    const int zg = blockIdx.y;
    const int i0 = ti_blk * BM, j0 = tj_blk * BN;
    const int lane = threadIdx.x & 63;
    const int wave = __builtin_amdgcn_readfirstlane(threadIdx.x >> 6);

    const i32x4 rs_w = rsrc_words(pa.w + (int64_t)zg * pa.w_grp_stride, pa.w_bytes - (int64_t)zg * pa.w_grp_stride * 4);
    const i32x4 rs_x = rsrc_words(g.x + (int64_t)zg * g.grp_stride, (g.total - (int64_t)zg * g.grp_stride) * 4);
    uint32_t voff_a[NA];
#pragma unroll
    for (int hf = 0; hf < NA; ++hf) {
        const int cl = hf * 64 + lane;
        voff_a[hf] = (cl < BM && i0 + cl < pe.Cog) ? (uint32_t)(i0 + cl) * 4u : OOB_OFF;
    }
    uint32_t voff_b[2];
#pragma unroll
    for (int hf = 0; hf < 2; ++hf) {
        const int m = j0 + hf * 64 + lane;
        const bool vm = m < g.M;
        const uint32_t mm = vm ? m : 0;
        const uint32_t n = fd_div(mm, g.dOHW);
        const uint32_t p = mm - n * g.OHW;
        const uint32_t oh = fd_div(p, g.dOW);
        const uint32_t ow = p - oh * g.OW;
        const int ih0 = (int)oh * g.stride - g.pt + g.halo, iw0 = (int)ow * g.col_mul + g.col_add;
        voff_b[hf] = vm ? (uint32_t)((int64_t)n * g.img_stride + (int64_t)ih0 * g.Wp + iw0) * 4u : OOB_OFF;
    }
    float bias_r[TA][4];
#pragma unroll
    for (int a = 0; a < TA; ++a)
#pragma unroll
        for (int q = 0; q < 4; ++q) {
            const int co = i0 + 16 * a + 4 * (lane >> 4) + q;
            bias_r[a][q] = (pe.bias && co < pe.Cog) ? pe.bias[zg * pe.Cog + co] : 0.f;
        }
    const uint32_t lds0 = (uint32_t)(uintptr_t)(__attribute__((address_space(3))) float*)ldsc;
    const int ld_bytes = (int)(pa.w_ld * 4);

    int tabv[RW];
    int row0 = 0;
    bool blk_ok = false;
    const int wrow = wave * RW;
    auto load_table = [&](int st) {
        const int k0 = st * SR + wrow;
        const const_int_ptr tt = as_const(g.ktab) + k0 + st * g.zero;
#pragma unroll
        for (int f = 0; f < RW; ++f) tabv[f] = tt[f];
        row0 = as_const(pa.row_tab)[k0 / KBLK + st * g.zero] + k0 % KBLK;
        blk_ok = k0 / KBLK < pa.nblk;
    };
    auto pin_table = [&]() {
#pragma unroll
        for (int f = 0; f < RW; ++f) asm volatile("" : "+s"(tabv[f]));
        asm volatile("" : "+s"(row0));
    };
    auto dma = [&](const int nb, const int f, int st) {
        const int rr = f / FPR, kind = f % FPR;
        const int z = st * g.zero;
        const bool live = blk_ok && st * SR + wrow + rr < g.K;
        if (kind < NA) {
            lds_dma_row(rs_w, lds0 + (uint32_t)(nb * BUF + (wrow + rr) * SA + kind * 64 + z) * 4u, voff_a[kind],
                        min(row0 + rr, g.K - 1) * ld_bytes);
        } else {
            const int hf = kind - NA;
            lds_dma_row(rs_x, lds0 + (uint32_t)(nb * BUF + ABUF + (wrow + rr) * SB + hf * 64 + z) * 4u, live ? voff_b[hf] : OOB_OFF,
                        tabv[rr]);
        }
    };
    int a_soff = 0;
    auto dma_fast = [&](const int nb, const int f, int st) {
        const int rr = f / FPR, kind = f % FPR;
        const int z = st * g.zero;
        if (f == 0) a_soff = row0 * ld_bytes;
        if (kind < NA) {
            lds_dma_row(rs_w, lds0 + (uint32_t)(nb * BUF + (wrow + rr) * SA + kind * 64 + z) * 4u, voff_a[kind], a_soff);
        } else {
            const int hf = kind - NA;
            lds_dma_row(rs_x, lds0 + (uint32_t)(nb * BUF + ABUF + (wrow + rr) * SB + hf * 64 + z) * 4u, voff_b[hf], tabv[rr]);
        }
        if (kind == NA - 1) a_soff += ld_bytes;
    };
    auto finish_stage = [&]() {
        asm volatile("s_waitcnt vmcnt(0)" ::: "memory");
        __syncthreads();
    };

    f32x4 acc[TA][2];
#pragma unroll
    for (int a = 0; a < TA; ++a)
#pragma unroll
        for (int b = 0; b < 2; ++b)
#pragma unroll
            for (int q = 0; q < 4; ++q) acc[a][b][q] = 0.f;

    const int nstages = (pa.nblk * KBLK + SR - 1) / SR;
    load_table(0);
    pin_table();
#pragma unroll
    for (int f = 0; f < NF; ++f) dma(0, f, 0);
    load_table(1);
    pin_table();
    finish_stage();

    const float* fa = ldsc + (lane >> 4) * SA + (lane & 15);
    const float* fb = ldsc + ABUF + (lane >> 4) * SB + wave * 32 + (lane & 15);

    auto stage = [&](const int cur, const bool fast, int st_next, const int nsteps) {
        float af[2][TA], bf[2][2];
        auto read = [&](int step, float (&a)[TA], float (&b)[2]) {
            const float* pa_ = fa + cur * BUF + step * 4 * SA;
            const float* pb_ = fb + cur * BUF + step * 4 * SB;
#pragma unroll
            for (int i = 0; i < TA; ++i) a[i] = pa_[16 * i];
#pragma unroll
            for (int i = 0; i < 2; ++i) b[i] = pb_[16 * i];
        };
        read(0, af[0], bf[0]);
#pragma unroll
        for (int t = 0; t < NSTEP; ++t) {
            const int c = t & 1;
            if (t + 1 < NSTEP) read(t + 1, af[c ^ 1], bf[c ^ 1]);
            if (t < nsteps) {
#pragma unroll
                for (int m = 0; m < NM; ++m) {
                    const int a = m >> 1, b = m & 1;
                    acc[a][b] = __builtin_amdgcn_mfma_f32_16x16x4f32(af[c][a], bf[c][b], acc[a][b], 0, 0, 0);
                    const int f = t * NM + m;
                    if (f < NF) {
                        if (fast) dma_fast(cur ^ 1, f, st_next);
                        else dma(cur ^ 1, f, st_next);
                        __builtin_amdgcn_sched_barrier(0);
                    }
                }
            } else {
#pragma unroll
                for (int m = 0; m < NM; ++m) {
                    const int f = t * NM + m;
                    if (f < NF) dma(cur ^ 1, f, st_next);
                }
            }
            static_assert(NF <= NM * (NSTEP - 3), "fetches must end before the table is replaced");
            if (t == NSTEP - 3) {
                load_table(st_next + 1);
                __builtin_amdgcn_sched_barrier(0);
            }
            if (t == NSTEP - 1) {
                pin_table();
                __builtin_amdgcn_sched_barrier(0);
            }
        }
        finish_stage();
    };
    const int nfull = g.K / SR;
    const int last_steps = (g.K - (nstages - 1) * SR + 3) / 4;
    int st = 0;
    for (; st + 2 < nfull; st += 2) {
        stage(0, true, st + 1, NSTEP);
        stage(1, true, st + 2, NSTEP);
    }
    for (; st < nstages; ++st) {
        const int ns = st == nstages - 1 ? last_steps : NSTEP;
        if (st & 1) stage(1, false, st + 1, ns);
        else stage(0, false, st + 1, ns);
    }

    if (wide) {
        constexpr int SP = BN + 4;
        float* T = ldsc;
#pragma unroll
        for (int b = 0; b < 2; ++b)
#pragma unroll
            for (int a = 0; a < TA; ++a)
#pragma unroll
                for (int q = 0; q < 4; ++q) {
                    float v = acc[a][b][q] + bias_r[a][q];
                    if (pe.relu) v = fmaxf(v, 0.f);
                    T[(16 * a + 4 * (lane >> 4) + q) * SP + wave * 32 + 16 * b + (lane & 15)] = v;
                }
        __syncthreads();
        const int px = 4 * (lane & 31);
        const int m = j0 + px;
        const uint32_t n = fd_div((uint32_t)min(m, pe.M - 1), pe.dOHW);
        const int p = m - (int)n * pe.OHW;
        const bool run4 = m + 3 < pe.M && p + 3 < pe.OHW;
        const int64_t cbase = ((int64_t)n * pe.Cout_total + (int64_t)zg * pe.Cog) * pe.y_plane + p;
#pragma unroll
        for (int i = 0; i < BM / 8; ++i) {
            const int cl = wave * (BM / 4) + 2 * i + (lane >> 5);
            const int co = i0 + cl;
            const f32x4 v = *reinterpret_cast<const f32x4*>(T + cl * SP + px);
            if (co >= pe.Cog) continue;
            float* dst = pe.y + cbase + (int64_t)co * pe.y_plane;
            if (run4) {
                *reinterpret_cast<f32x4u*>(dst) = v;
            } else {
#pragma unroll
                for (int e = 0; e < 4; ++e) {
                    const int me = m + e;
                    if (me < pe.M) {
                        const uint32_t ne = fd_div((uint32_t)me, pe.dOHW);
                        const int pe_ = me - (int)ne * pe.OHW;
                        pe.y[((int64_t)ne * pe.Cout_total + (int64_t)zg * pe.Cog + co) * pe.y_plane + pe_] = v[e];
                    }
                }
            }
        }
        return;
    }
#pragma unroll
    for (int b = 0; b < 2; ++b) {
        const int m = j0 + wave * 32 + 16 * b + (lane & 15);
        if (m >= pe.M) continue;
        const uint32_t n = fd_div((uint32_t)m, pe.dOHW);
        const uint32_t p = m - n * pe.OHW;
        const uint32_t oh = fd_div(p, pe.dOW);
        const uint32_t ow = p - oh * pe.OW;
        const int64_t c0 = (int64_t)n * pe.Cout_total + (int64_t)zg * pe.Cog;
        const int64_t ybase = c0 * pe.y_plane + (int64_t)(oh + pe.y_halo) * pe.y_wp + ow + pe.y_halo;
        const int64_t mbase = c0 * pe.m_plane + (int64_t)(oh + pe.m_halo) * pe.m_wp + ow + pe.m_halo;
        float mk[TA][4];
        if (pe.mask) {
#pragma unroll
            for (int a = 0; a < TA; ++a)
#pragma unroll
                for (int q = 0; q < 4; ++q) {
                    const int co = i0 + 16 * a + 4 * (lane >> 4) + q;
                    mk[a][q] = co < pe.Cog ? pe.mask[mbase + (int64_t)co * pe.m_plane] : 0.f;
                }
        }
#pragma unroll
        for (int a = 0; a < TA; ++a) {
#pragma unroll
            for (int q = 0; q < 4; ++q) {
                const int co = i0 + 16 * a + 4 * (lane >> 4) + q;
                if (co < pe.Cog) {
                    float v = acc[a][b][q] + bias_r[a][q];
                    if (pe.relu) v = fmaxf(v, 0.f);
                    if (pe.mask) v = mk[a][q] > 0.f ? v : 0.f;
                    pe.y[ybase + (int64_t)co * pe.y_plane] = v;
                }
            }
        }
    }
}


static int device_cus();

template <int BM>
static int launch_conv_dma(const ConvGeom& g, const float* w, int64_t w_ld, int w_grp_stride, const int* row_tab, int Cog,
                           int Cout_total, const ConvOut& o, hipStream_t s) {
    constexpr int BN = 128, SR = 32;
    constexpr size_t lds = BM == 128 ? (size_t)BM * (BN + 4) * sizeof(float)
                                     : (size_t)2 * SR * ((BM + 63) / 64 * 64 + 16 + 144) * sizeof(float);
    static_assert(BM != 128 || (size_t)2 * SR * (BM + BN) * sizeof(float) <= (size_t)BM * (BN + 4) * sizeof(float), "stage buffers fit");
    ConvDmaParams pa{w, w_ld, (int64_t)w_grp_stride, (int64_t)g.K * w_ld * 4, row_tab, ceil_div(g.K, KBLK)};
    EpiConvNCHW::Params pe;
    pe.y = o.y; pe.bias = o.bias; pe.mask = o.mask; pe.relu = o.relu;
    pe.Cog = Cog; pe.Cout_total = Cout_total; pe.OHW = g.OHW; pe.OW = g.OW; pe.M = g.M;
    pe.dOHW = g.dOHW; pe.dOW = g.dOW;
    pe.y_halo = o.y_halo; pe.y_wp = o.OW + 2 * o.y_halo; pe.y_plane = (int64_t)(o.OH + 2 * o.y_halo) * pe.y_wp;
    pe.m_halo = o.m_halo; pe.m_wp = o.OW + 2 * o.m_halo; pe.m_plane = (int64_t)(o.OH + 2 * o.m_halo) * pe.m_wp;
    static bool attr_set = false;
    if (!attr_set) {
        const void* kern;
        if constexpr (BM == 128) kern = reinterpret_cast<const void*>(conv_dma_kernel<SR>);
        else kern = reinterpret_cast<const void*>(conv_dma16_kernel<BM / 16>);
        VL_HIP(hipFuncSetAttribute(kern, hipFuncAttributeMaxDynamicSharedMemorySize, (int)lds));
        attr_set = true;
    }
    const int tiles_i = ceil_div(Cog, BM), tiles_j = ceil_div(g.M, BN);
    dim3 grid(tiles_i * tiles_j, (unsigned)(Cout_total / Cog), 1);
    const int wide = (o.y_halo == 0 && !o.mask && !kConvNoWideStore && (size_t)BM * (BN + 4) * sizeof(float) <= lds) ? 1 : 0;
    if constexpr (BM == 128) {
        hipLaunchKernelGGL(conv_dma_kernel<SR>, grid, dim3(NT), lds, s, pa, g, pe, tiles_i, wide);
    } else {
        hipLaunchKernelGGL((conv_dma16_kernel<BM / 16>), grid, dim3(NT), lds, s, pa, g, pe, tiles_i, wide);
    }
    VL_LAUNCH_CHECK();
    return 0;
}

template <int BM>
static int launch_conv_ring(const ConvGeom& g, const float* w, int64_t w_ld, int w_grp_stride, const int* row_tab, int Cog,
                            int Cout_total, const ConvOut& o, uint32_t* wsplit, hipStream_t s) {
    constexpr int BN = BM == 128 ? 256 : 512;
    const int math = g_conv_math, planes = math == 6 ? 3 : 2;
    const int groups = Cout_total / Cog, nstages = ceil_div(g.K, KBLK), CogP = ceil_div(Cog, BM) * BM;
    hipLaunchKernelGGL(conv_wsplit_kernel, dim3(nstages, groups), dim3(256), 0, s, w, w_ld, (int64_t)w_grp_stride, row_tab, g.K, Cog,
                       CogP, nstages, planes, wsplit);
    VL_LAUNCH_CHECK();
    ConvRingParams pa{wsplit, CogP, nstages};
    EpiConvNCHW::Params pe;
    pe.y = o.y; pe.bias = o.bias; pe.mask = o.mask; pe.relu = o.relu;
    pe.Cog = Cog; pe.Cout_total = Cout_total; pe.OHW = g.OHW; pe.OW = g.OW; pe.M = g.M;
    pe.dOHW = g.dOHW; pe.dOW = g.dOW;
    pe.y_halo = o.y_halo; pe.y_wp = o.OW + 2 * o.y_halo; pe.y_plane = (int64_t)(o.OH + 2 * o.y_halo) * pe.y_wp;
    pe.m_halo = o.m_halo; pe.m_wp = o.OW + 2 * o.m_halo; pe.m_plane = (int64_t)(o.OH + 2 * o.m_halo) * pe.m_wp;
    const int OH = g.OHW / g.OW, OWp = (g.OW + 3) / 4 * 4, Mp = g.M / g.OW * OWp;
    const int tiles_i = ceil_div(Cog, BM), tiles_j = ceil_div(Mp, BN);
    dim3 grid(tiles_i * tiles_j, (unsigned)groups, 1);
    if (BM == 128 && math != 6 && !kRing8) {
        constexpr size_t lds4 = (size_t)3 * 16 * (128 + 256) * sizeof(float);
        static bool attr4[2] = {false, false};
        const int v4 = math == 3;
        auto k4 = v4 ? conv_ring4_kernel<3> : conv_ring4_kernel<1>;
        if (!attr4[v4]) {
            VL_HIP(hipFuncSetAttribute(reinterpret_cast<const void*>(k4), hipFuncAttributeMaxDynamicSharedMemorySize, (int)lds4));
            attr4[v4] = true;
        }
        hipLaunchKernelGGL(k4, grid, dim3(256), lds4, s, pa, g, pe, tiles_i, OWp, Mp, make_fastdiv(OH * OWp), make_fastdiv(OWp));
        VL_LAUNCH_CHECK();
        return 0;
    }
    const size_t lds = (size_t)(BM == 128 ? 5 : 4) * (planes * 8 * BM + 16 * BN) * sizeof(float);
    static bool attr_set[3] = {false, false, false};
    const int v8 = math == 6 ? 2 : math == 3 ? 1 : 0;
    auto kern = v8 == 2 ? conv_ring_kernel<6, BM> : v8 == 1 ? conv_ring_kernel<3, BM> : conv_ring_kernel<1, BM>;
    if (!attr_set[v8]) {
        VL_HIP(hipFuncSetAttribute(reinterpret_cast<const void*>(kern), hipFuncAttributeMaxDynamicSharedMemorySize, (int)lds));
        attr_set[v8] = true;
    }
    hipLaunchKernelGGL(kern, grid, dim3(512), lds, s, pa, g, pe, tiles_i, OWp, Mp, make_fastdiv(OH * OWp), make_fastdiv(OWp));
    VL_LAUNCH_CHECK();
    return 0;
}

template <bool PADDED>
static int dispatch_conv(const ConvGeom& g, const float* w, int64_t w_ld, int w_grp_stride, const int* row_tab, int Cog,
                         int Cout_total, const ConvOut& o, uint32_t* wsplit, hipStream_t s) {
    const int w128 = ceil_div(Cog, 128) * 128, w96 = ceil_div(Cog, 96) * 96, w64 = ceil_div(Cog, 64) * 64;
    if (g_conv_math != 0 && PADDED && g.col_mul == 1 && wsplit != nullptr) {
        if (Cog >= 96) return launch_conv_ring<128>(g, w, w_ld, w_grp_stride, row_tab, Cog, Cout_total, o, wsplit, s);
        if (Cog >= 40 && Cog <= 64) return launch_conv_ring<64>(g, w, w_ld, w_grp_stride, row_tab, Cog, Cout_total, o, wsplit, s);
    }
    const int64_t px = ceil_div(g.M, 128), cus = device_cus(), ngrp = Cout_total / Cog;
    const bool few = px * ceil_div(Cog, 128) * ngrp < 8 * cus;
    if (PADDED && few && (int64_t)g.K * w_ld * 4 < MAX_BUF_BYTES && !kConvStaged && !kConvNoLoadPick) {
        const int widths[3] = {128, 96, 48};
        auto pick = [&](int64_t pxt, int64_t& load) {
            int b = 0;
            for (int i = 0; i < 3; ++i) {
                const int64_t l = ceil_div(pxt * ceil_div(Cog, widths[i]) * ngrp, cus) * widths[i];
                if (i == 0 || l < load) { b = i; load = l; }
            }
            return b;
        };
        auto run = [&](int wi, const ConvGeom& gg, const ConvOut& oo) {
            if (wi == 0) return launch_conv_dma<128>(gg, w, w_ld, w_grp_stride, row_tab, Cog, Cout_total, oo, s);
            if (wi == 1) return launch_conv_dma<96>(gg, w, w_ld, w_grp_stride, row_tab, Cog, Cout_total, oo, s);
            return launch_conv_dma<48>(gg, w, w_ld, w_grp_stride, row_tab, Cog, Cout_total, oo, s);
        };
        int64_t best_load = 0;
        const int best = pick(px, best_load);
        const int nimg = g.M / g.OHW;
        const int64_t wgs_per_px = (int64_t)ceil_div(Cog, widths[best]) * ngrp;
        const int64_t rounds = px * wgs_per_px / cus;
        if (rounds >= 6 && !kConvNoTailSplit) {
            const int64_t px_a = rounds * cus / wgs_per_px;
            const int n_a = (int)(px_a * 128 / g.OHW);
            const int n_b = nimg - n_a;
            if (n_a > 0 && n_b > 0) {
                int64_t load_b = 0;
                const int64_t px_b = ceil_div((int64_t)n_b * g.OHW, 128);
                const int wb = pick(px_b, load_b);
                const int64_t load_a = ceil_div(ceil_div((int64_t)n_a * g.OHW, 128) * wgs_per_px, cus) * widths[best];
                if ((load_a + (load_b > 64 ? load_b : 64) + 16) * 100 <= best_load * 95) {
                    ConvGeom ga = g, gb = g;
                    ga.M = n_a * g.OHW; ga.total = g.img_stride * n_a;
                    gb.x = g.x + (int64_t)n_a * g.img_stride; gb.M = n_b * g.OHW; gb.total = g.img_stride * n_b;
                    ConvOut ob = o;
                    ob.y = o.y + (int64_t)n_a * Cout_total * (o.OH + 2 * o.y_halo) * (o.OW + 2 * o.y_halo);
                    if (o.mask) ob.mask = o.mask + (int64_t)n_a * Cout_total * (o.OH + 2 * o.m_halo) * (o.OW + 2 * o.m_halo);
                    if (int rc = run(best, ga, o)) return rc;
                    return run(wb, gb, ob);
                }
            }
        }
        return run(best, g, o);
    }
    if (w128 <= w96 && w128 <= w64) {
        if (PADDED && (int64_t)g.K * w_ld * 4 < MAX_BUF_BYTES && !kConvStaged) {
            return launch_conv_dma<128>(g, w, w_ld, w_grp_stride, row_tab, Cog, Cout_total, o, s);
        }
        return launch_conv<128, 2, 2, PADDED>(g, w, w_ld, w_grp_stride, row_tab, Cog, Cout_total, o, s);
    }
    if (PADDED && ceil_div(Cog, 48) * 48 < w64 && ceil_div(Cog, 48) * 48 < w96 &&
        (int64_t)g.K * w_ld * 4 < MAX_BUF_BYTES && !kConvStaged)
        return launch_conv_dma<48>(g, w, w_ld, w_grp_stride, row_tab, Cog, Cout_total, o, s);
    if (w96 <= w64) {
        if (PADDED && (int64_t)g.K * w_ld * 4 < MAX_BUF_BYTES && !kConvStaged)
            return launch_conv_dma<96>(g, w, w_ld, w_grp_stride, row_tab, Cog, Cout_total, o, s);
        return launch_conv<96, 1, 4, PADDED>(g, w, w_ld, w_grp_stride, row_tab, Cog, Cout_total, o, s);
    }
    return launch_conv<64, 1, 4, PADDED>(g, w, w_ld, w_grp_stride, row_tab, Cog, Cout_total, o, s);
}

static void fill_geom(ConvGeom& g, const float* x, int n, int cin_total, int cig, int H, int W, int halo, int OH, int OW,
                      int stride, int pt, int pl, int K, const int* tab, const int2* tab2, int phase = 1) {
    g.x = x; g.ktab = tab; g.ktab2 = tab2; g.K = K; g.M = n * OH * OW; g.H = H; g.W = W;
    g.halo = halo;
    g.Wp = phase > 1 ? (W + 2 * halo + phase - 1) / phase : W + 2 * halo;
    g.col_mul = phase > 1 ? 1 : stride;
    g.col_add = phase > 1 ? 0 : halo - pl;
    g.stride = stride; g.pt = pt; g.pl = pl; g.OHW = OH * OW; g.OW = OW;
    g.dOHW = make_fastdiv(g.OHW); g.dOW = make_fastdiv(g.OW);
    const int64_t Pp = (int64_t)(H + 2 * halo) * g.Wp;
    g.img_stride = (int64_t)cin_total * phase * Pp;
    g.grp_stride = (int64_t)cig * phase * Pp;
    g.total = g.img_stride * n;
    g.zero = 0;
}

extern "C" int vl_conv_fwd(const vl_conv_desc* d, const float* x, const float* w, const float* bias, float* y, int n,
                           int relu, vl_stream_t stream) {
    VL_CHECK(d && x && w && y, "vl_conv_fwd: null argument");
    VL_CHECK(n > 0 && (int64_t)n * d->oh * d->ow < (1ll << 31), "vl_conv_fwd: bad batch %d", n);
    ConvGeom g;
    fill_geom(g, x, n, d->cin, d->cig, d->h, d->w, d->x_halo, d->oh, d->ow, d->stride, d->pt, d->pl, d->K, d->ptab_fwd, d->ptab2_fwd,
              d->x_phase > 1 ? d->x_phase : 1);
    VL_CHECK(g.total * 4 < MAX_BUF_BYTES, "vl_conv_fwd: input of %lld elements exceeds the buffer-offset range", (long long)g.total);
    ConvOut o{y, bias, nullptr, relu, d->y_halo, 0, d->oh, d->ow};
    if (d->fwd_padded) return dispatch_conv<true>(g, w, d->cout, d->cog, d->rowtab_fwd, d->cog, d->cout, o, d->wsplit_fwd, (hipStream_t)stream);
    return dispatch_conv<false>(g, w, d->cout, d->cog, d->rowtab_fwd, d->cog, d->cout, o, d->wsplit_fwd, (hipStream_t)stream);
}

__global__ __launch_bounds__(256) void conv_wt_transpose_kernel(const float* __restrict__ w, float* __restrict__ wt, int KH, int KW,
                                                                int cig, int cog, int groups) {
    __shared__ float tile[64][65];
    const int cin = cig * groups, cout = cog * groups;
    const int tci = (cig + 63) / 64, tco = (cog + 63) / 64;
    int b = blockIdx.x;
    const int co0 = (b % tco) * 64; b /= tco;
    const int ci0 = (b % tci) * 64; b /= tci;
    const int g = b % groups;       b /= groups;
    const int kx = b % KW, ky = b / KW;
    const int lx = threadIdx.x & 63, ly = threadIdx.x >> 6;
    const float* src = w + ((int64_t)(ky * KW + kx) * cig) * cout + g * cog;
    for (int r = ly; r < 64; r += 4) {
        const int ci = ci0 + r, co = co0 + lx;
        if (ci < cig && co < cog) tile[r][lx] = src[(int64_t)ci * cout + co];
    }
    __syncthreads();
    float* dst = wt + ((int64_t)((KH - 1 - ky) * KW + (KW - 1 - kx)) * cog) * cin + g * cig;
    for (int r = ly; r < 64; r += 4) {
        const int co = co0 + r, ci = ci0 + lx;
        if (co < cog && ci < cig) dst[(int64_t)co * cin + ci] = tile[lx][r];
    }
}

extern "C" int vl_conv_wt_transpose(const vl_conv_desc* d, const float* w, float* wt, vl_stream_t stream) {
    VL_CHECK(d && w && wt, "vl_conv_wt_transpose: null argument");
    const int blocks = d->kh * d->kw * d->groups * ((d->cig + 63) / 64) * ((d->cog + 63) / 64);
    hipLaunchKernelGGL(conv_wt_transpose_kernel, dim3(blocks), dim3(256), 0, (hipStream_t)stream, w, wt, d->kh, d->kw, d->cig,
                       d->cog, d->groups);
    VL_LAUNCH_CHECK();
    return 0;
}

extern "C" int vl_conv_dgrad(const vl_conv_desc* d, const float* dy, const float* wt, float* dx, const float* relu_mask,
                             int n, vl_stream_t stream) {
    VL_CHECK(d && dy && wt && dx, "vl_conv_dgrad: null argument");
    VL_CHECK(d->stride == 1, "vl_conv_dgrad: only stride-1 layers (conv1 needs no input gradient)");
    VL_CHECK(n > 0 && (int64_t)n * d->h * d->w < (1ll << 31), "vl_conv_dgrad: bad batch %d", n);
    ConvGeom g;
    fill_geom(g, dy, n, d->cout, d->cog, d->oh, d->ow, d->dy_halo, d->h, d->w, 1, d->kh - 1 - d->pt, d->kw - 1 - d->pl, d->Kd,
              d->ptab_bwd, d->ptab2_bwd);
    VL_CHECK(g.total * 4 < MAX_BUF_BYTES, "vl_conv_dgrad: dy of %lld elements exceeds the buffer-offset range", (long long)g.total);
    ConvOut o{dx, nullptr, relu_mask, 0, d->dx_halo, d->x_halo, d->h, d->w};
    if (d->bwd_padded) return dispatch_conv<true>(g, wt, d->cin, d->cig, d->rowtab_bwd, d->cig, d->cin, o, d->wsplit_bwd, (hipStream_t)stream);
    return dispatch_conv<false>(g, wt, d->cin, d->cig, d->rowtab_bwd, d->cig, d->cin, o, d->wsplit_bwd, (hipStream_t)stream);
}

static void dy_params(const vl_conv_desc* d, const ConvGeom& g, const float* dy, DyParams& pb) {
    pb.dy = dy; pb.M = g.M; pb.OHW = g.OHW; pb.OW = g.OW; pb.Cog = d->cog; pb.Cout_total = d->cout; pb.halo = d->dy_halo;
    pb.OWp = d->ow + 2 * d->dy_halo; pb.dOHW = g.dOHW; pb.dOW = g.dOW;
    pb.plane = (int64_t)(d->oh + 2 * d->dy_halo) * pb.OWp;
    pb.total = (int64_t)d->cout * pb.plane * (g.M / g.OHW);
    pb.zero = 0;
}

static int reduce_wgrad(const vl_conv_desc* d, float* dw, const float* ws, int splits, hipStream_t s) {
    const int64_t slab = (int64_t)d->K * d->cout;
    if (splits > 1) {
        launch_reduce_slabs(s, ws, dw, slab, splits, slab, nullptr, 0, 0, 0, nullptr);
        VL_LAUNCH_CHECK();
    }
    return 0;
}

template <int BN, int WM, int WN>
static int launch_wgrad(const vl_conv_desc* d, const ConvGeom& g, const float* dy, float* dw, float* ws, int splits,
                        hipStream_t s) {
    constexpr int BM = 128, BR = 32;
    using LA = WgradGather<BM, BR, false>;
    using LB = DyRows<BN, BR>;
    DyParams pb;
    dy_params(d, g, dy, pb);
    const int64_t slab = (int64_t)d->K * d->cout;
    EpiRowMajor::Params pe{splits > 1 ? ws : dw, d->cout, d->K, d->cog, nullptr, nullptr, 0, d->cog, splits > 1 ? slab : 0};
    const int tiles_i = ceil_div(d->K, BM), tiles_j = ceil_div(d->cog, BN);
    const int rtiles = ceil_div(g.M, BR);
    dim3 grid(tiles_i * tiles_j, d->groups, splits);
    hipLaunchKernelGGL((mfma_contract<BM, BN, BR, WM, WN, LA, LB, EpiRowMajor>), grid, dim3(NT), 0, s, g, pb, pe, tiles_i, rtiles,
                       ceil_div(rtiles, splits));
    VL_LAUNCH_CHECK();
    return reduce_wgrad(d, dw, ws, splits, s);
}

template <int BN, int WM, int WN>
static int launch_wgrad_dma(const vl_conv_desc* d, const ConvGeom& g, const float* dy, float* dw, float* db, float* ws, int splits,
                            hipStream_t s) {
    using C = WgradDmaCfg<BN>;
    DyParams pb;
    dy_params(d, g, dy, pb);
    const int64_t slab = (int64_t)d->K * d->cout;
    EpiRowMajor::Params pe{splits > 1 ? ws : dw, d->cout, d->K, d->cog, nullptr, nullptr, 0, d->cog, splits > 1 ? slab : 0};
    const int tiles_i = ceil_div(d->K, C::BM), tiles_j = ceil_div(d->cog, BN);
    const int rtiles = ceil_div(g.M, C::BR);
    static bool attr_set[8] = {false, false, false, false, false, false, false, false};
    int v = g_conv_math == 6 ? 3 : g_conv_math == 3 ? 2 : g_conv_math == 1 ? 1 : 0;
    auto kern = v == 3 ? wgrad_dma_kernel<BN, WM, WN, 6> : v == 2 ? wgrad_dma_kernel<BN, WM, WN, 3>
              : v == 1 ? wgrad_dma_kernel<BN, WM, WN, 1> : wgrad_dma_kernel<BN, WM, WN, 0>;
    if constexpr (BN == 128) {
        if (v != 0 && g.OW % 4 == 0 && g.col_mul == 1 && !kWgradDword) {
            kern = v == 3 ? wgrad_dma_kernel<BN, WM, WN, 6, true> : v == 2 ? wgrad_dma_kernel<BN, WM, WN, 3, true> : wgrad_dma_kernel<BN, WM, WN, 1, true>;
            v += 4;
        }
    }
    if (!attr_set[v]) {
        VL_HIP(hipFuncSetAttribute(reinterpret_cast<const void*>(kern), hipFuncAttributeMaxDynamicSharedMemorySize, (int)C::LDS_BYTES));
        attr_set[v] = true;
    }
    float* db_slabs = db ? (splits > 1 ? ws + (int64_t)splits * slab : db) : nullptr;
    const int units = d->groups * splits;
    dim3 grid((unsigned)(ceil_div(units, 8) * 8 * tiles_i * tiles_j), 1, 1);
    hipLaunchKernelGGL(kern, grid, dim3(NT), C::LDS_BYTES, s, g, pb, pe, tiles_i, tiles_j, d->groups, units, rtiles,
                       ceil_div(rtiles, splits), db_slabs, d->cout);
    VL_LAUNCH_CHECK();
    if (db && splits > 1) {
        launch_reduce_slabs(s, db_slabs, db, (int64_t)d->cout, splits, (int64_t)d->cout, nullptr, 0, 0, 0, nullptr);
        VL_LAUNCH_CHECK();
    }
    return reduce_wgrad(d, dw, ws, splits, s);
}

static int device_cus() {
    static int cus = 0;
    if (!cus) {
        int dev = 0;
        hipDeviceProp_t p;
        if (hipGetDevice(&dev) == hipSuccess && hipGetDeviceProperties(&p, dev) == hipSuccess) cus = p.multiProcessorCount;
        if (cus <= 0) cus = 256;
    }
    return cus;
}

static int wgrad_splits(const vl_conv_desc* d, int n) {
    const int64_t M = (int64_t)n * d->oh * d->ow;
    const int tiles = ceil_div(d->K, 128) * ceil_div(d->cog, d->cog % 128 == 0 ? 128 : 96) * d->groups;
    if (!d->fwd_padded) {
        const int rtiles = ceil_div(M, 32);
        int splits = ceil_div(2048, tiles);
        return splits > rtiles ? rtiles : (splits < 1 ? 1 : splits);
    }
    const int rtiles = ceil_div(M, 64);
    static const int forced = vl_exp_env("VL_WGRAD_SPLITS") ? atoi(vl_exp_env("VL_WGRAD_SPLITS")) : 0;
    if (forced >= 1 && forced <= rtiles) return forced;
    const int per_xcd = device_cus() / 8 > 0 ? device_cus() / 8 : 1;
    const int64_t slab_bytes = ((int64_t)d->K + 1) * d->cout * 4;
    int best = 1;
    int64_t best_cost = -1;
    for (int s = 1; s <= rtiles && s <= 4096; ++s) {
        if (s > 1 && slab_bytes * s > (512ll << 20)) break;
        const bool balanced = ((int64_t)d->groups * s) % 8 == 0;
        const int64_t wgs_xcd = (int64_t)ceil_div((int64_t)d->groups * s, 8) * (tiles / d->groups);
        const int64_t cost = (int64_t)ceil_div(wgs_xcd, per_xcd) * (ceil_div(rtiles, s) + 2) + (balanced ? 0 : 1);
        if (best_cost < 0 || cost < best_cost) {
            best_cost = cost;
            best = s;
        }
    }
    return best;
}

extern "C" size_t vl_conv_wgrad_ws_bytes(const vl_conv_desc* d, int n) {
    if (!d || n <= 0) return 0;
    return (size_t)wgrad_splits(d, n) * ((size_t)d->K + 1) * d->cout * sizeof(float);
}

extern "C" int vl_conv_wgrad_fuses_bias(const vl_conv_desc* d) { return d && d->fwd_padded && d->K % 128 != 0 ? 1 : 0; }

extern "C" int vl_conv_wgrad(const vl_conv_desc* d, const float* x, const float* dy, float* dw, float* db, void* ws,
                             size_t ws_bytes, int n, vl_stream_t stream) {
    VL_CHECK(d && x && dy && dw, "vl_conv_wgrad: null argument");
    VL_CHECK(!db || vl_conv_wgrad_fuses_bias(d), "vl_conv_wgrad: no fused bias gradient for this layer (see vl_conv_wgrad_fuses_bias)");
    VL_CHECK(n > 0 && (int64_t)n * d->oh * d->ow < (1ll << 31), "vl_conv_wgrad: bad batch %d", n);
    const int splits = wgrad_splits(d, n);
    VL_CHECK(splits == 1 || (ws && ws_bytes >= vl_conv_wgrad_ws_bytes(d, n)), "vl_conv_wgrad: workspace too small (%zu < %zu)",
             ws_bytes, vl_conv_wgrad_ws_bytes(d, n));
    ConvGeom g;
    fill_geom(g, x, n, d->cin, d->cig, d->h, d->w, d->x_halo, d->oh, d->ow, d->stride, d->pt, d->pl, d->K, d->ktab_fwd, d->ktab2_fwd,
              d->x_phase > 1 ? d->x_phase : 1);
    const int64_t dy_total = (int64_t)n * d->cout * (d->oh + 2 * d->dy_halo) * (d->ow + 2 * d->dy_halo);
    VL_CHECK(g.total * 4 < MAX_BUF_BYTES && dy_total * 4 < MAX_BUF_BYTES, "vl_conv_wgrad: operand exceeds the buffer-offset range");
    hipStream_t s = (hipStream_t)stream;
    if (d->cog % 128 == 0) {
        if (d->fwd_padded) return launch_wgrad_dma<128, 2, 2>(d, g, dy, dw, db, (float*)ws, splits, s);
        return launch_wgrad<128, 2, 2>(d, g, dy, dw, (float*)ws, splits, s);
    }
    if (d->fwd_padded) return launch_wgrad_dma<96, 4, 1>(d, g, dy, dw, db, (float*)ws, splits, s);
    return launch_wgrad<96, 4, 1>(d, g, dy, dw, (float*)ws, splits, s);
}

template <int BM, int WM, int WN, class LA, class LB>
static int launch_gemm(int m, int n, int k, const float* a, int64_t lda, const float* b, int64_t ldb, float* c, int64_t ldc,
                       const float* bias, int relu, const float* mask, float* ws, int splits, hipStream_t s) {
    constexpr int BN = 128, BR = 16;
    typename LA::Params pa{a, lda, m, k, 0};
    typename LB::Params pb{b, ldb, n, k, 0};
    const int tiles_i = ceil_div(m, BM), tiles_j = ceil_div(n, BN);
    const int rtiles = ceil_div(k, BR);
    const int per = ceil_div(rtiles, splits);
    EpiRowMajor::Params pe;
    if (splits > 1)
        pe = EpiRowMajor::Params{ws, n, m, n, nullptr, nullptr, 0, 0, (int64_t)m * n};
    else
        pe = EpiRowMajor::Params{c, ldc, m, n, bias, mask, relu, 0, 0};
    dim3 grid(tiles_i * tiles_j, 1, splits);
    hipLaunchKernelGGL((mfma_contract<BM, BN, BR, WM, WN, LA, LB, EpiRowMajor>), grid, dim3(NT), 0, s, pa, pb, pe, tiles_i, rtiles, per);
    VL_LAUNCH_CHECK();
    if (splits > 1) {
        const int64_t cnt = (int64_t)m * n;
        launch_reduce_slabs(s, ws, c, cnt, splits, cnt, bias, n, ldc, relu, mask);
        VL_LAUNCH_CHECK();
    }
    return 0;
}

template <int BM, int WM, int WN>
static int dispatch_gemm_t(int ta, int tb, int m, int n, int k, const float* a, int64_t lda, const float* b, int64_t ldb,
                           float* c, int64_t ldc, const float* bias, int relu, const float* mask, float* ws, int splits,
                           hipStream_t s) {
    constexpr int BN = 128, BR = 16;
    if (!ta && !tb) return launch_gemm<BM, WM, WN, DenseXK<BM, BR>, DenseKX<BN, BR>>(m, n, k, a, lda, b, ldb, c, ldc, bias, relu, mask, ws, splits, s);
    if (!ta && tb) return launch_gemm<BM, WM, WN, DenseXK<BM, BR>, DenseXK<BN, BR>>(m, n, k, a, lda, b, ldb, c, ldc, bias, relu, mask, ws, splits, s);
    if (ta && !tb) return launch_gemm<BM, WM, WN, DenseKX<BM, BR>, DenseKX<BN, BR>>(m, n, k, a, lda, b, ldb, c, ldc, bias, relu, mask, ws, splits, s);
    return launch_gemm<BM, WM, WN, DenseKX<BM, BR>, DenseXK<BN, BR>>(m, n, k, a, lda, b, ldb, c, ldc, bias, relu, mask, ws, splits, s);
}

__global__ void gemm_split_image_kernel(const float* __restrict__ x, int64_t sk, int64_t sr, int K, int R, int Rp, int planes,
                                        uint32_t* __restrict__ out) {
    const int st = blockIdx.y;
    uint32_t* o = out + (int64_t)st * planes * 8 * Rp;
    const int r0 = blockIdx.x * 64;
    if (sk == 1) {
        const int rr = threadIdx.x >> 2, kq = threadIdx.x & 3, r = r0 + rr, k0 = st * 16 + 4 * kq;
        float v[4] = {0.f, 0.f, 0.f, 0.f};
        if (r < R) {
#pragma unroll
            for (int e = 0; e < 4; ++e)
                if (k0 + e < K) v[e] = x[(int64_t)r * sr + k0 + e];
        }
        const int h = kq >> 1;
#pragma unroll
        for (int e = 0; e < 2; ++e) {
            int pc[3] = {0, 0, 0};
            split_pieces<3>(v[2 * e], v[2 * e + 1], pc);
            const int q = (kq & 1) * 2 + e;
            for (int pl = 0; pl < planes; ++pl) o[(int64_t)((2 * pl + h) * Rp + r) * 4 + q] = (uint32_t)pc[pl];
        }
    } else {
        for (int idx = threadIdx.x; idx < 8 * 64; idx += blockDim.x) {
            const int rr = idx & 63, hq = idx >> 6, h = hq >> 2, q = hq & 3, r = r0 + rr, k = st * 16 + 8 * h + 2 * q;
            float x0 = 0.f, x1 = 0.f;
            if (r < R) {
                if (k < K) x0 = x[(int64_t)k * sk + r];
                if (k + 1 < K) x1 = x[(int64_t)(k + 1) * sk + r];
            }
            int pc[3] = {0, 0, 0};
            split_pieces<3>(x0, x1, pc);
            for (int pl = 0; pl < planes; ++pl) o[(int64_t)((2 * pl + h) * Rp + r) * 4 + q] = (uint32_t)pc[pl];
        }
    }
}

struct GemmSplitParams {
    const uint32_t* ia;
    const uint32_t* ib;
    int Mp, Np, nstages, stages_per_split;
    float* c;
    int64_t ldc, slab_stride;
    const float* bias;
    const float* mask;
    int relu, m, n, splits;
};

template <int MATH>
__global__ __launch_bounds__(256, MATH == 6 ? 1 : 2) void gemm_split_kernel(const GemmSplitParams P) {
    constexpr int BM = 128, BN = 256, NBUF = 3, D = 3, TA = 4, TB = 2;
    constexpr int NP = split_products(MATH), NPC = split_pieces_of(MATH), NPL = MATH == 6 ? 3 : 2;
    constexpr int APC = NPL * 2 * 2, BPC = NPL * 2 * 4;
    constexpr int ABUF = APC * 256, BUF = (APC + BPC) * 256;
    constexpr int FA = APC / 4, FB = BPC / 4, FW = FA + FB;
    constexpr int NM = TA * TB * NP;
    static_assert(NM >= FW, "a fetch rides on each of the first FW MFMAs");
    extern __shared__ __attribute__((aligned(16))) float ldsg[];
    const int tiles_i = P.Mp / BM;
    const int bid = xcd_swizzle(blockIdx.x, gridDim.x);
    const int i0 = (bid % tiles_i) * BM, j0 = (bid / tiles_i) * BN;
    const int zs = blockIdx.z;
    const int lane = threadIdx.x & 63;
    const int wave = __builtin_amdgcn_readfirstlane(threadIdx.x >> 6);
    const int s_begin = zs * P.stages_per_split;
    const int nst = min(P.nstages, s_begin + P.stages_per_split) - s_begin;

    const int64_t sdw_a = (int64_t)NPL * 8 * P.Mp, sdw_b = (int64_t)NPL * 8 * P.Np;
    const i32x4 rs_a = rsrc_words(reinterpret_cast<const float*>(P.ia), P.nstages * sdw_a * 4);
    const i32x4 rs_b = rsrc_words(reinterpret_cast<const float*>(P.ib), P.nstages * sdw_b * 4);
    uint32_t voff[FW];
#pragma unroll
    for (int f = 0; f < FA; ++f) {
        const int p = wave * FA + f;
        voff[f] = (uint32_t)(((p >> 1) * P.Mp + i0 + (p & 1) * 64 + lane) * 16);
    }
#pragma unroll
    for (int f = 0; f < FB; ++f) {
        const int p = wave * FB + f;
        voff[FA + f] = (uint32_t)(((p >> 2) * P.Np + j0 + (p & 3) * 64 + lane) * 16);
    }
    const uint32_t lds0 = (uint32_t)(uintptr_t)(__attribute__((address_space(3))) float*)ldsg;
    const int sb_a = (int)(sdw_a * 4), sb_b = (int)(sdw_b * 4);
    auto dma = [&](const uint32_t wr, const int f, int st) __attribute__((always_inline)) {
        if (f < FA) lds_dma_row4(rs_a, lds0 + wr + (uint32_t)(wave * FA + f) * 1024u, voff[f], st * sb_a);
        else lds_dma_row4(rs_b, lds0 + wr + (uint32_t)(ABUF * 4 + (wave * FB + f - FA) * 1024), voff[f], st * sb_b);
    };

    f32x16 acc[TA][TB];
#pragma unroll
    for (int a = 0; a < TA; ++a)
#pragma unroll
        for (int b = 0; b < TB; ++b)
#pragma unroll
            for (int q = 0; q < 16; ++q) acc[a][b][q] = 0.f;

    const float* fa = ldsg + ((lane >> 5) * BM + (lane & 31)) * 4;
    const float* fb = ldsg + ABUF + ((lane >> 5) * BN + wave * 64 + (lane & 31)) * 4;
    auto load_ops = [&](int rd, SplitBf16 (&A)[TA], SplitBf16 (&B)[TB]) __attribute__((always_inline)) {
#pragma unroll
        for (int k = 0; k < NPC; ++k) {
#pragma unroll
            for (int a = 0; a < TA; ++a) A[a].p[k] = *reinterpret_cast<const i32x4*>(fa + rd + k * 2 * BM * 4 + a * 32 * 4);
#pragma unroll
            for (int b = 0; b < TB; ++b) B[b].p[k] = *reinterpret_cast<const i32x4*>(fb + rd + k * 2 * BN * 4 + b * 32 * 4);
        }
    };

    for (int s0 = 0; s0 < NBUF; ++s0) {
        if (s0 < nst) {
#pragma unroll
            for (int f = 0; f < FW; ++f) dma((uint32_t)(s0 * BUF * 4), f, s_begin + s0);
        }
    }
    if (nst >= NBUF) asm volatile("s_waitcnt vmcnt(%0)" ::"n"(2 * FW) : "memory");
    else asm volatile("s_waitcnt vmcnt(0)" ::: "memory");
    __syncthreads();
    SplitBf16 A[TA] = {}, B[TB] = {}, An[TA] = {}, Bn[TB] = {};
    load_ops(0, A, B);
    if (nst >= NBUF) asm volatile("s_waitcnt vmcnt(%0) lgkmcnt(0)" ::"n"(FW) : "memory");
    else asm volatile("s_waitcnt vmcnt(0) lgkmcnt(0)" ::: "memory");
    __syncthreads();

    int rd = BUF;
    uint32_t wr = 0;
// ... 130 lines not shown
```

### video-learning-tf_amd/ops.py

```python
import ctypes as C

import torch

from . import _ffi

F32 = torch.float32


def stream():
    return torch.cuda.current_stream().cuda_stream


def _p(t):
    return None if t is None else t.data_ptr()


def _f32(*ts):
    for t in ts:
        if t is None:
            continue
        if not (t.is_cuda and t.dtype == F32):
            raise _ffi.VltfError("expected a CUDA/HIP float32 tensor, got %s on %s" % (t.dtype, t.device))


def _dense(*ts):
    for t in ts:
        if t is not None and not t.is_contiguous():
            raise _ffi.VltfError("expected a contiguous tensor")


def phase_split_shape(n, c, h, w, halo, phase):
    if phase <= 1:
        return (n, c, h + 2 * halo, w + 2 * halo)
    return (n, c * phase, h + 2 * halo, -(-(w + 2 * halo) // phase))


def input_prep_u8(src, dst, crop_y=None, crop_x=None, mirror=None, mean_bgr=None, halo=0, phase=1, out_hw=None):
    if src.dtype != torch.uint8 or not src.is_cuda:
        raise _ffi.VltfError("input_prep_u8: src must be a device uint8 tensor")
    _f32(dst, mean_bgr)
    _dense(src, dst, crop_y, crop_x, mirror, mean_bgr)
    n, rh, rw, c = src.shape
    if out_hw is None:
        if phase > 1:
            raise _ffi.VltfError("input_prep_u8: out_hw is required with a phase-split destination")
        out_hw = (dst.shape[2] - 2 * halo, dst.shape[3] - 2 * halo)
    if c != 3 or tuple(dst.shape) != phase_split_shape(n, 3, out_hw[0], out_hw[1], halo, phase):
        raise _ffi.VltfError("input_prep_u8: shape mismatch %s -> %s" % (tuple(src.shape), tuple(dst.shape)))
    _ffi.call("vl_input_prep_u8", _p(src), _p(dst), n, rh, rw, out_hw[0], out_hw[1], _p(crop_y), _p(crop_x), _p(mirror),
              _p(mean_bgr), halo, phase, stream())


def nhwc_to_nchw(src, dst, halo=0, phase=1):
    _f32(src, dst); _dense(src, dst)
    n, h, w, c = src.shape
    if tuple(dst.shape) != phase_split_shape(n, c, h, w, halo, phase):
        raise _ffi.VltfError("nhwc_to_nchw: shape mismatch %s -> %s (halo %d)" % (tuple(src.shape), tuple(dst.shape), halo))
    _ffi.call("vl_nhwc_to_nchw", _p(src), _p(dst), n, h, w, c, halo, phase, stream())


def nchw_to_nhwc(src, dst):
    _f32(src, dst); _dense(src, dst)
    n, c, h, w = src.shape
    _ffi.call("vl_nchw_to_nhwc", _p(src), _p(dst), n, c, h, w, stream())


class Conv:

    def __init__(self, cin, h, w, cout, kh, kw, stride, groups):
        self.cin, self.h, self.w, self.cout = cin, h, w, cout
        self.kh, self.kw, self.stride, self.groups = kh, kw, stride, groups
        self._d = C.c_void_p()
        _ffi.check(_ffi.lib().vl_conv_create(C.byref(self._d), cin, h, w, cout, kh, kw, stride, groups), "vl_conv_create")
        oh, ow = C.c_int(), C.c_int()
        _ffi.check(_ffi.lib().vl_conv_out_hw(self._d, C.byref(oh), C.byref(ow)), "vl_conv_out_hw")
        self.oh, self.ow = oh.value, ow.value
        self.w_shape = (kh, kw, cin // groups, cout)
        self.x_halo = self.y_halo = self.dy_halo = self.dx_halo = 0

    def same_pad(self):
        def one(n, k, s):
            out = -(-n // s)
            tot = max((out - 1) * s + k - n, 0)
            return tot - tot // 2
        return max(one(self.h, self.kh, self.stride), one(self.w, self.kw, self.stride))

    def set_halo(self, x_halo=0, y_halo=0, dy_halo=0, dx_halo=0):
        _ffi.call("vl_conv_set_halo", self._d, x_halo, y_halo, dy_halo, dx_halo)
        self.x_halo, self.y_halo, self.dy_halo, self.dx_halo = x_halo, y_halo, dy_halo, dx_halo
        self.x_phase = int(_ffi.lib().vl_conv_x_phase(self._d))

    def set_x_phase_split(self, on=True):
        _ffi.call("vl_conv_set_x_phase_split", self._d, int(on))
        self.x_phase = int(_ffi.lib().vl_conv_x_phase(self._d))
        return self.x_phase

    def _shape(self, n, c, h, w, halo):
        return (n, c, h + 2 * halo, w + 2 * halo)

    def x_shape(self, n):
        return phase_split_shape(n, self.cin, self.h, self.w, self.x_halo, getattr(self, "x_phase", 1))

    def __del__(self):
        try:
            if self._d:
                _ffi.lib().vl_conv_destroy(self._d)
                self._d = None
        except Exception:
            pass

    def fwd(self, x, w, bias, y, relu=True):
        _f32(x, w, bias, y); _dense(x, w, bias, y)
        n = x.shape[0]
        if tuple(x.shape) != self.x_shape(n) or tuple(y.shape) != self._shape(n, self.cout, self.oh, self.ow, self.y_halo):
            raise _ffi.VltfError("conv.fwd: shape mismatch x=%s y=%s (halos %d, %d)" % (tuple(x.shape), tuple(y.shape),
                                                                                        self.x_halo, self.y_halo))
        _ffi.call("vl_conv_fwd", self._d, _p(x), _p(w), _p(bias), _p(y), n, int(relu), stream())

    def wt_transpose(self, w, wt):
        _f32(w, wt); _dense(w, wt)
        _ffi.call("vl_conv_wt_transpose", self._d, _p(w), _p(wt), stream())

    def dgrad(self, dy, wt, dx, relu_mask=None):
        _f32(dy, wt, dx, relu_mask); _dense(dy, wt, dx, relu_mask)
        n = dy.shape[0]
        if tuple(dy.shape) != self._shape(n, self.cout, self.oh, self.ow, self.dy_halo) or \
                tuple(dx.shape) != self._shape(n, self.cin, self.h, self.w, self.dx_halo) or \
                (relu_mask is not None and tuple(relu_mask.shape) != self._shape(n, self.cin, self.h, self.w, self.x_halo)):
            raise _ffi.VltfError("conv.dgrad: shape mismatch dy=%s dx=%s" % (tuple(dy.shape), tuple(dx.shape)))
        _ffi.call("vl_conv_dgrad", self._d, _p(dy), _p(wt), _p(dx), _p(relu_mask), dy.shape[0], stream())

    def wgrad_ws_bytes(self, n):
        return int(_ffi.lib().vl_conv_wgrad_ws_bytes(self._d, n))

    def fuses_bias(self):
        return bool(_ffi.lib().vl_conv_wgrad_fuses_bias(self._d))

    def wgrad(self, x, dy, dw, ws, db=None):
        _f32(x, dy, dw, db); _dense(x, dy, dw, ws, db)
        n = x.shape[0]
        if tuple(x.shape) != self.x_shape(n) or tuple(dy.shape) != self._shape(n, self.cout, self.oh, self.ow, self.dy_halo):
            raise _ffi.VltfError("conv.wgrad: shape mismatch x=%s dy=%s" % (tuple(x.shape), tuple(dy.shape)))
        nbytes = 0 if ws is None else ws.numel() * ws.element_size()
        _ffi.call("vl_conv_wgrad", self._d, _p(x), _p(dy), _p(dw), _p(db), _p(ws), nbytes, x.shape[0], stream())


    def c8_w_bytes(self, bwd=False):
        return int(_ffi.lib().vl_conv_c8_w_bytes(self._d, int(bwd)))

    def c8_pack_w(self, w, wb, bwd=False):
        _f32(w); _dense(w, wb)
        if wb.numel() * wb.element_size() < self.c8_w_bytes(bwd):
            raise _ffi.VltfError("conv.c8_pack_w: weight buffer too small")
        _ffi.call("vl_conv_c8_pack_w", self._d, _p(w), _p(wb), int(bwd), stream())

    def _c8_check(self, t, n, c, h, w, halo, what):
        if t is not None and (t.dtype != torch.bfloat16 or tuple(t.shape) != c8_shape(n, c, h, w, halo) or not t.is_contiguous()):
            raise _ffi.VltfError("conv: %s must be a contiguous bf16 c8 tensor %s, got %s %s" % (what, c8_shape(n, c, h, w, halo),
                                                                                                 t.dtype, tuple(t.shape)))

    def c8_fwd(self, xb, wb, bias, y=None, yb=None, relu=True):
        n = xb.shape[0]
        _f32(bias, y); _dense(bias, y, wb)
        self._c8_check(xb, n, self.cin, self.h, self.w, self.x_halo, "xb")
        self._c8_check(yb, n, self.cout, self.oh, self.ow, self.y_halo, "yb")
        if y is not None and tuple(y.shape) != self._shape(n, self.cout, self.oh, self.ow, self.y_halo):
            raise _ffi.VltfError("conv.c8_fwd: y shape %s" % (tuple(y.shape),))
        _ffi.call("vl_conv_c8_fwd", self._d, _p(xb), _p(wb), _p(bias), _p(y), _p(yb), n, int(relu), stream())

    def c8_dgrad(self, dyb, wbt, dx=None, dxb=None, relu_mask=None, relu_mask_c8=None):
        n = dyb.shape[0]
        self._c8_check(relu_mask_c8, n, self.cin, self.h, self.w, self.x_halo, "relu_mask_c8")
        _f32(dx, relu_mask); _dense(dx, relu_mask, wbt)
        self._c8_check(dyb, n, self.cout, self.oh, self.ow, self.dy_halo, "dyb")
        self._c8_check(dxb, n, self.cin, self.h, self.w, self.dx_halo, "dxb")
        for t in (dx, relu_mask):
            if t is not None and tuple(t.shape) != self._shape(n, self.cin, self.h, self.w, self.dx_halo):
                raise _ffi.VltfError("conv.c8_dgrad: dx / relu_mask shape %s" % (tuple(t.shape),))
        _ffi.call("vl_conv_c8_dgrad", self._d, _p(dyb), _p(wbt), _p(dx), _p(dxb), _p(relu_mask), _p(relu_mask_c8), n, stream())

    def s2d_layer(self):
        s, ka = self.stride, (self.kh - 1) // self.stride + 1
        eq = Conv(self.cin * s * s, self.oh, self.ow, self.cout, ka, ka, 1, 1)
        eq.set_halo((ka - 1) // 2, 0, (ka - 1) // 2, 0)
        return eq

    def s2d_c8_from_x0(self, x0, xb):
        _f32(x0); _dense(x0, xb)
        n = x0.shape[0]
        s, ka = self.stride, (self.kh - 1) // self.stride + 1
        if tuple(x0.shape) != self.x_shape(n) or xb.dtype != torch.bfloat16 or \
                tuple(xb.shape) != c8_shape(n, self.cin * s * s, self.oh, self.ow, (ka - 1) // 2):
            raise _ffi.VltfError("conv.s2d_c8_from_x0: shape mismatch x0=%s xb=%s" % (tuple(x0.shape), tuple(xb.shape)))
        _ffi.call("vl_s2d_c8_from_x0", self._d, _p(x0), _p(xb), n, stream())

    def input_prep_u8_s2d(self, src, xb, crop_y=None, crop_x=None, mirror=None, mean_bgr=None):
        if src.dtype != torch.uint8 or not src.is_cuda or src.dim() != 4 or src.shape[3] != self.cin:
            raise _ffi.VltfError("conv.input_prep_u8_s2d: src must be a device uint8 [n, h, w, %d] tensor" % self.cin)
        _f32(mean_bgr); _dense(src, xb, mean_bgr)
        n = src.shape[0]
        s, ka = self.stride, (self.kh - 1) // self.stride + 1
        if xb.dtype != torch.bfloat16 or tuple(xb.shape) != c8_shape(n, self.cin * s * s, self.oh, self.ow, (ka - 1) // 2):
            raise _ffi.VltfError("conv.input_prep_u8_s2d: xb shape %s" % (tuple(xb.shape),))
        for t, dt in ((crop_y, torch.int32), (crop_x, torch.int32), (mirror, torch.uint8)):
            if t is not None and (t.dtype != dt or t.numel() < n or not t.is_contiguous()):
                raise _ffi.VltfError("conv.input_prep_u8_s2d: crop / mirror must be contiguous int32 / uint8 tensors of n entries")
        _ffi.call("vl_input_prep_u8_s2d", self._d, _p(src), _p(xb), n, src.shape[1], src.shape[2], _p(crop_y), _p(crop_x), _p(mirror),
                  _p(mean_bgr), stream())

    def s2d_weights(self, src, dst, grad=False):
        _f32(src, dst); _dense(src, dst)
        s, ka = self.stride, (self.kh - 1) // self.stride + 1
        big, small = (ka, ka, self.cin * s * s, self.cout), self.w_shape
        if (tuple(src.shape), tuple(dst.shape)) != ((big, small) if grad else (small, big)):
            raise _ffi.VltfError("conv.s2d_weights: shape mismatch %s -> %s" % (tuple(src.shape), tuple(dst.shape)))
        _ffi.call("vl_s2d_weights", self._d, _p(src), _p(dst), int(grad), stream())

    def c8_wgrad_ws_bytes(self, n):
        return int(_ffi.lib().vl_conv_c8_wgrad_ws_bytes(self._d, n))

    def c8_wgrad(self, xb, dyb, dw, ws):
        n = xb.shape[0]
        _f32(dw); _dense(dw, ws)
        self._c8_check(xb, n, self.cin, self.h, self.w, self.x_halo, "xb")
        self._c8_check(dyb, n, self.cout, self.oh, self.ow, self.dy_halo, "dyb")
        if tuple(dw.shape) != self.w_shape:
            raise _ffi.VltfError("conv.c8_wgrad: dw shape %s" % (tuple(dw.shape),))
        _ffi.call("vl_conv_c8_wgrad", self._d, _p(xb), _p(dyb), _p(dw), _p(ws), ws.numel() * ws.element_size(), n, stream())


def bias_grad_c8(dyb, db, ws, c, halo):
    _f32(db, ws); _dense(dyb, db, ws)
    n, cb, hp, wp, _ = dyb.shape
    if dyb.dtype != torch.bfloat16 or cb != (c + 7) // 8 or ws.numel() < 64 * 8 * cb:
        raise _ffi.VltfError("bias_grad_c8: dyb must be bf16 c8 of %d channels, ws >= 64 * 8 * blocks floats" % c)
    _ffi.call("vl_bias_grad_c8", _p(dyb), _p(db), _p(ws), n, c, hp - 2 * halo, wp - 2 * halo, halo, stream())


def kc8_shape(positions, channels):
    return ((channels + 7) // 8, positions, 8)


def pack_kc8(src, dst, positions, channels, pos_stride, ch_stride):
    _f32(src); _dense(dst)
    if dst.dtype != torch.bfloat16 or tuple(dst.shape) != kc8_shape(positions, channels):
        raise _ffi.VltfError("pack_kc8: dst must be bf16 %s, got %s %s" % (kc8_shape(positions, channels), dst.dtype, tuple(dst.shape)))
    if (positions - 1) * pos_stride + (channels - 1) * ch_stride >= src.numel():
        raise _ffi.VltfError("pack_kc8: strides reach past the source")
    _ffi.call("vl_pack_kc8", _p(src), _p(dst), positions, channels, pos_stride, ch_stride, stream())


def gemm_kc8_ws_bytes(m, n, k):
    return int(_ffi.lib().vl_gemm_kc8_ws_bytes(m, n, k))


def gemm_kc8(a, b, c, m, n, k, bias=None, relu=False, ws=None):
    _f32(c, bias); _dense(a, b, c, bias, ws)
    if a.dtype != torch.bfloat16 or b.dtype != torch.bfloat16 or tuple(a.shape) != kc8_shape(k, m) or tuple(b.shape) != kc8_shape(k, n) \
            or c.numel() < m * n:
        raise _ffi.VltfError("gemm_kc8: operand shapes a=%s b=%s for m=%d n=%d k=%d" % (tuple(a.shape), tuple(b.shape), m, n, k))
    _ffi.call("vl_gemm_kc8", _p(a), _p(b), _p(c), m, n, k, _p(bias), int(relu), _p(ws), 0 if ws is None else ws.numel() * ws.element_size(),
              stream())


def c8_shape(n, c, h, w, halo):
    return (n, (c + 7) // 8, h + 2 * halo, w + 2 * halo, 8)


def pack_c8(x, xb, x_halo, xb_halo):
    _f32(x); _dense(x, xb)
    n, c = x.shape[0], x.shape[1]
    h, w = x.shape[2] - 2 * x_halo, x.shape[3] - 2 * x_halo
    if xb.dtype != torch.bfloat16 or tuple(xb.shape) != c8_shape(n, c, h, w, xb_halo):
        raise _ffi.VltfError("pack_c8: xb must be bf16 %s, got %s %s" % (c8_shape(n, c, h, w, xb_halo), xb.dtype, tuple(xb.shape)))
    _ffi.call("vl_pack_c8", _p(x), _p(xb), n, c, h, w, x_halo, xb_halo, stream())


def bias_grad_nchw(dy, db, ws):
    _f32(dy, db, ws); _dense(dy, db, ws)
    n, c = dy.shape[0], dy.shape[1]
    hw = dy.numel() // (n * c)
    if ws.numel() < 64 * c:
        raise _ffi.VltfError("bias_grad_nchw: workspace needs 64*c floats")
    _ffi.call("vl_bias_grad_nchw", _p(dy), _p(db), _p(ws), n, c, hw, stream())


def lrn_fwd(x, y, radius=2, alpha=2e-5, beta=0.75, bias=1.0):
    _f32(x, y); _dense(x, y)
    n, c = x.shape[0], x.shape[1]
    _ffi.call("vl_lrn_fwd", _p(x), _p(y), n, c, x.numel() // (n * c), radius, alpha, beta, bias, stream())


def lrn_bwd(x, dy, dx, radius=2, alpha=2e-5, beta=0.75, bias=1.0, relu_fused=False, dx_halo=0):
    _f32(x, dy, dx); _dense(x, dy, dx)
    n, c, h, w = x.shape
    if tuple(dx.shape) != (n, c, h + 2 * dx_halo, w + 2 * dx_halo):
        raise _ffi.VltfError("lrn_bwd: dx shape %s does not match x %s with halo %d" % (tuple(dx.shape), tuple(x.shape), dx_halo))
    _ffi.call("vl_lrn_bwd", _p(x), _p(dy), _p(dx), n, c, h * w, radius, alpha, beta, bias, int(relu_fused), w, dx_halo, stream())


def pool_out(h, k=3, s=2):
    return (h - k) // s + 1


def _pool_layout(c, oh, ow, hwc, halo):
    if hwc:
        return 0, (oh * ow * c, 1, ow * c, c)
    wp = ow + 2 * halo
    pp = (oh + 2 * halo) * wp
    return halo * wp + halo, (c * pp, pp, wp, 1)


def maxpool_fwd(x, y, argmax, k=3, s=2, hwc=False, y_halo=0):
    _f32(x, y); _dense(x, y, argmax)
    n, c, h, w = x.shape
    o, st = _pool_layout(c, pool_out(h, k, s), pool_out(w, k, s), hwc, y_halo)
    _ffi.call("vl_maxpool_fwd", _p(x), _p(y) + 4 * o, None if argmax is None else _p(argmax) + o, n, c, h, w, k, s, st[0], st[1],
              st[2], st[3], stream())


def maxpool_bwd(dy, argmax, dx, relu_mask=None, k=3, s=2, hwc=False, dy_halo=0, dx_halo=0):
    _f32(dy, dx, relu_mask); _dense(dy, dx, argmax, relu_mask)
    n, c = dx.shape[0], dx.shape[1]
    h, w = dx.shape[2] - 2 * dx_halo, dx.shape[3] - 2 * dx_halo
    o, st = _pool_layout(c, pool_out(h, k, s), pool_out(w, k, s), hwc, dy_halo)
    _ffi.call("vl_maxpool_bwd", _p(dy) + 4 * o, _p(argmax) + o, _p(dx), _p(relu_mask), n, c, h, w, k, s, st[0], st[1], st[2], st[3],
              dx_halo, stream())


def lrn_pool_fwd(x, p, argmax, p_halo=0, radius=2, alpha=2e-5, beta=0.75, bias=1.0):
    _f32(x, p); _dense(x, p, argmax)
    n, c, h, w = x.shape
    want = (n, c, pool_out(h) + 2 * p_halo, pool_out(w) + 2 * p_halo)
    if tuple(p.shape) != want or tuple(argmax.shape) != want:
        raise _ffi.VltfError("lrn_pool_fwd: shape mismatch x=%s p=%s argmax=%s" % (tuple(x.shape), tuple(p.shape), tuple(argmax.shape)))
    _ffi.call("vl_lrn_pool_fwd", _p(x), _p(p), _p(argmax), n, c, h, w, p_halo, radius, alpha, beta, bias, stream())


def _x_or_packed(x, c):
    if x.dtype == torch.bfloat16:
        if x.dim() != 5 or x.shape[4] != 8 or c is None or x.shape[1] != (c + 7) // 8 or not x.is_contiguous():
            raise _ffi.VltfError("packed pool input must be a contiguous bf16 [n][c/8][h][w][8] tensor and needs channels=")
        return 1, x.shape[0], x.shape[2], x.shape[3]
    _f32(x)
    return 0, x.shape[0], x.shape[2], x.shape[3]


def lrn_pool_fwd_c8(x, pb, argmax, p_halo=0, radius=2, alpha=2e-5, beta=0.75, bias=1.0, channels=None):
    _dense(x, pb, argmax)
    c = channels if channels is not None else x.shape[1]
    packed, n, h, w = _x_or_packed(x, c)
    oh, ow = pool_out(h), pool_out(w)
    if pb.dtype != torch.bfloat16 or tuple(pb.shape) != c8_shape(n, c, oh, ow, p_halo) or \
            tuple(argmax.shape) != (n, c, oh + 2 * p_halo, ow + 2 * p_halo):
        raise _ffi.VltfError("lrn_pool_fwd_c8: shape mismatch x=%s pb=%s argmax=%s" % (tuple(x.shape), tuple(pb.shape), tuple(argmax.shape)))
    _ffi.call("vl_lrn_pool_fwd_c8", _p(x), packed, _p(pb), _p(argmax), n, c, h, w, p_halo, radius, alpha, beta, bias, stream())


def pool_lrn_bwd(x, dp, argmax, dx, p_halo=0, dx_halo=0, radius=2, alpha=2e-5, beta=0.75, bias=1.0, relu_fused=True):
    _f32(x, dp, dx); _dense(x, dp, argmax, dx)
    n, c, h, w = x.shape
    oh, ow = pool_out(h), pool_out(w)
    if tuple(dp.shape) != (n, c, oh + 2 * p_halo, ow + 2 * p_halo) or tuple(argmax.shape) != tuple(dp.shape) or \
            tuple(dx.shape) != (n, c, h + 2 * dx_halo, w + 2 * dx_halo):
        raise _ffi.VltfError("pool_lrn_bwd: shape mismatch x=%s dp=%s dx=%s" % (tuple(x.shape), tuple(dp.shape), tuple(dx.shape)))
    _ffi.call("vl_pool_lrn_bwd", _p(x), _p(dp), _p(argmax), _p(dx), n, c, h, w, p_halo, radius, alpha, beta, bias, int(relu_fused),
              dx_halo, stream())


def pool_lrn_bwd_test_ranges(ranges=0):
    _ffi.call("vl_pool_lrn_bwd_test_ranges", int(ranges))


def pool_lrn_bwd_c8(x, dp, argmax, dxb, p_halo=0, dxb_halo=0, radius=2, alpha=2e-5, beta=0.75, bias=1.0, relu_fused=True):
    _f32(dp); _dense(x, dp, argmax, dxb)
    c = dp.shape[1]
    packed, n, h, w = _x_or_packed(x, c)
    oh, ow = pool_out(h), pool_out(w)
    if tuple(dp.shape) != (n, c, oh + 2 * p_halo, ow + 2 * p_halo) or tuple(argmax.shape) != tuple(dp.shape) or \
            dxb.dtype != torch.bfloat16 or tuple(dxb.shape) != c8_shape(n, c, h, w, dxb_halo):
        raise _ffi.VltfError("pool_lrn_bwd_c8: shape mismatch x=%s dp=%s dxb=%s" % (tuple(x.shape), tuple(dp.shape), tuple(dxb.shape)))
    _ffi.call("vl_pool_lrn_bwd_c8", _p(x), packed, _p(dp), _p(argmax), _p(dxb), n, c, h, w, p_halo, radius, alpha, beta, bias, int(relu_fused),
              dxb_halo, stream())


def gemm(a, b, c, m, n, k, transa=False, transb=False, lda=None, ldb=None, ldc=None, bias=None, relu=False,
         relu_mask=None, ws=None):
    _f32(a, b, c, bias, relu_mask)
    lda = lda if lda is not None else (m if transa else k)
    ldb = ldb if ldb is not None else (k if transb else n)
    ldc = ldc if ldc is not None else n
    nbytes = 0 if ws is None else ws.numel() * ws.element_size()
    _ffi.call("vl_gemm", int(transa), int(transb), m, n, k, _p(a), lda, _p(b), ldb, _p(c), ldc, _p(bias), int(relu),
              _p(relu_mask), _p(ws), nbytes, stream())


def gemm_split_ws_bytes(m, n, k):
    return int(_ffi.lib().vl_gemm_split_ws_bytes(int(m), int(n), int(k)))
# ... 293 lines not shown
```

Baseline: 1878 clips/s.

## Skip zero-padding taps in convolutions via per-border-class reduced tap tables

Groups output pixels into classes by which kernel taps fall inside the input plane (by rows, or rows by columns). Each class gets its own reduced K table, so the implicit-GEMM conv kernel skips taps that would only read halo zeros, and output tiles are remapped through a per-class pixel list. The goal is to cut wasted MFMA work and loads at image borders for small-spatial layers such as 13x13 and 27x27. The cost is per-pixel table lookups, tiles that may be partly empty for small classes, and the tail-split path being disabled when classes are used.

```diff
diff --git a/include/vltf.h b/include/vltf.h
--- a/include/vltf.h
+++ b/include/vltf.h
@@ -35,6 +35,9 @@
 int vl_conv_set_halo(vl_conv_desc* d, int x_halo, int y_halo, int dy_halo, int dx_halo);
 int vl_conv_set_x_phase_split(vl_conv_desc* d, int on);
 int vl_conv_x_phase(const vl_conv_desc* d);
+int vl_conv_set_tap_skip(vl_conv_desc* d, int mode);
+int vl_conv_set_tap_partition(vl_conv_desc* d, int fwd_part, int bwd_part);
+int vl_conv_tap_counts(const vl_conv_desc* d, int bwd, int64_t* executed, int64_t* nominal, int* classes, int* partition);
 int vl_set_conv_math(int math);
 int vl_conv_math(void);
 int vl_conv_fwd(const vl_conv_desc* d, const float* x, const float* w_hwio, const float* bias, float* y,
diff --git a/video-learning-tf_amd/_ffi.py b/video-learning-tf_amd/_ffi.py
--- a/video-learning-tf_amd/_ffi.py
+++ b/video-learning-tf_amd/_ffi.py
@@ -20,6 +20,9 @@
     "vl_conv_set_halo": (i32, [p, i32, i32, i32, i32]),
     "vl_conv_set_x_phase_split": (i32, [p, i32]),
     "vl_conv_x_phase": (i32, [p]),
+    "vl_conv_set_tap_skip": (i32, [p, i32]),
+    "vl_conv_set_tap_partition": (i32, [p, i32, i32]),
+    "vl_conv_tap_counts": (i32, [p, i32, C.POINTER(i64), C.POINTER(i64), C.POINTER(i32), C.POINTER(i32)]),
     "vl_set_conv_math": (i32, [i32]),
     "vl_conv_math": (i32, []),
     "vl_gemm_split_ws_bytes": (C.c_size_t, [i32, i32, i32]),
diff --git a/video-learning-tf_amd/csrc/conv_desc.h b/video-learning-tf_amd/csrc/conv_desc.h
--- a/video-learning-tf_amd/csrc/conv_desc.h
+++ b/video-learning-tf_amd/csrc/conv_desc.h
@@ -23,6 +23,14 @@
     uint32_t* wsplit_bwd;
     int* c8_toff_fwd;
     int* c8_toff_bwd;
+    int tap_skip;
+    int tap_part[2];
+    struct Classes {
+        int* dev;
+        int ncls, part;
+        int map_off;
+        int64_t executed, nominal;
+    } cls[2];
 };
 
 void conv_c8_free_tables(vl_conv_desc* d);
diff --git a/video-learning-tf_amd/csrc/mfma_gemm.hip b/video-learning-tf_amd/csrc/mfma_gemm.hip
--- a/video-learning-tf_amd/csrc/mfma_gemm.hip
+++ b/video-learning-tf_amd/csrc/mfma_gemm.hip
@@ -891,9 +891,63 @@
     int64_t w_bytes;
     const int* row_tab;
     int nblk;
+    const int* cls;
+    int map_off, nimg;
 };
 
-template <int SR>
+static constexpr int CLS_HDR = 8, CLS_GROUP = 128;
+struct ConvTile {
+    const_int_ptr ktab, rtab, pix;
+    int K, nblk;
+    int M, j0;
+    int n0;
+    uint32_t P, dm, ds;
+};
+template <bool CLS>
+__device__ __forceinline__ ConvTile conv_tile(const ConvDmaParams& pa, const ConvGeom& g, int tj) {
+    ConvTile t;
+    t.ktab = as_const(g.ktab); t.rtab = as_const(pa.row_tab); t.pix = nullptr;
+    t.K = g.K; t.nblk = pa.nblk; t.M = g.M; t.j0 = tj * 128;
+    t.P = 0; t.dm = 0; t.ds = 0; t.n0 = 0;
+    if constexpr (CLS) {
+        const const_int_ptr H = as_const(pa.cls);
+        const int grp = (int)fd_div((uint32_t)tj, g.dOHW);
+        const int e = H[pa.map_off + tj - grp * g.OHW];
+        const const_int_ptr h = H + (e & 255) * CLS_HDR;
+        t.P = h[0]; t.pix = H + h[1]; t.ktab = H + h[2]; t.rtab = H + h[3];
+        t.K = h[4]; t.nblk = h[5]; t.dm = h[6]; t.ds = h[7];
+        t.n0 = grp * CLS_GROUP;
+        t.M = min(CLS_GROUP, pa.nimg - t.n0) * (int)t.P; t.j0 = (e >> 8) * 128;
+    }
+    return t;
+}
+template <bool CLS>
+__device__ __forceinline__ void conv_tile_pixel(const ConvTile& t, const FastDiv& dOHW, int OHW, uint32_t m, uint32_t& n, uint32_t& p) {
+    if constexpr (CLS) {
+        const uint32_t q = (__umulhi(m, t.dm) + m) >> t.ds;
+        p = (uint32_t)t.pix[m - q * t.P];
+        n = t.n0 + q;
+    } else {
+        n = fd_div(m, dOHW);
+        p = m - n * OHW;
+    }
+}
+template <bool CLS>
+__device__ __forceinline__ bool conv_tile_run4(const ConvTile& t, const FastDiv& dOHW, int OHW, int m, uint32_t& n, int& p) {
+    if constexpr (CLS) {
+        const uint32_t mc = (uint32_t)min(m, t.M - 1);
+        const uint32_t q = (__umulhi(mc, t.dm) + mc) >> t.ds;
+        const int i = (int)(mc - q * t.P);
+        n = t.n0 + q;
+        p = t.pix[i];
+        return m + 3 < t.M && i + 3 < (int)t.P && t.pix[min(i + 3, (int)t.P - 1)] == p + 3;
+    }
+    n = fd_div((uint32_t)min(m, t.M - 1), dOHW);
+    p = m - (int)n * OHW;
+    return m + 3 < t.M && p + 3 < OHW;
+}
+
+template <int SR, bool CLS = false>
 __global__ __launch_bounds__(NT, 64 / SR) void conv_dma_kernel(const ConvDmaParams pa, const ConvGeom g, const EpiConvNCHW::Params pe,
                                                                int tiles_i, int wide) {
     constexpr int BM = 128, BN = 128;
@@ -907,7 +961,9 @@
     const int bid = xcd_swizzle(blockIdx.x, gridDim.x);
     const int ti_blk = bid % tiles_i, tj_blk = bid / tiles_i;
     const int zg = blockIdx.y;
-    const int i0 = ti_blk * BM, j0 = tj_blk * BN;
+    const ConvTile T_ = conv_tile<CLS>(pa, g, tj_blk);
+    if (CLS && T_.j0 >= T_.M) return;
+    const int i0 = ti_blk * BM, j0 = T_.j0;
     const int lane = threadIdx.x & 63;
     const int wave = __builtin_amdgcn_readfirstlane(threadIdx.x >> 6);
     const int wm = wave >> 1, wn = wave & 1;
@@ -920,10 +976,10 @@
         const int co = i0 + hf * 64 + lane;
         voff_a[hf] = co < pe.Cog ? (uint32_t)co * 4u : OOB_OFF;
         const int m = j0 + hf * 64 + lane;
-        const bool vm = m < g.M;
+        const bool vm = m < T_.M;
         const uint32_t mm = vm ? m : 0;
-        const uint32_t n = fd_div(mm, g.dOHW);
-        const uint32_t p = mm - n * g.OHW;
+        uint32_t n, p;
+        conv_tile_pixel<CLS>(T_, g.dOHW, g.OHW, mm, n, p);
         const uint32_t oh = fd_div(p, g.dOW);
         const uint32_t ow = p - oh * g.OW;
         const int ih0 = (int)oh * g.stride - g.pt + g.halo, iw0 = (int)ow * g.col_mul + g.col_add;
@@ -938,11 +994,11 @@
     const int wrow = wave * RW;
     auto load_table = [&](int st) {
         const int k0 = st * SR + wrow;
-        const const_int_ptr tt = as_const(g.ktab) + k0 + st * g.zero;
+        const const_int_ptr tt = T_.ktab + k0 + st * g.zero;
 #pragma unroll
         for (int f = 0; f < RW; ++f) tabv[f] = tt[f];
-        row0 = as_const(pa.row_tab)[k0 / KBLK + st * g.zero] + k0 % KBLK;
-        blk_ok = k0 / KBLK < pa.nblk;
+        row0 = T_.rtab[k0 / KBLK + st * g.zero] + k0 % KBLK;
+        blk_ok = k0 / KBLK < T_.nblk;
     };
     auto pin_table = [&]() {
 #pragma unroll
@@ -953,7 +1009,7 @@
         const int rr = f >> 2, kind = f & 3, hf = kind & 1;
         const int z = st * g.zero;
         const uint32_t row_lds = lds0 + (uint32_t)(nb * BUF + (wrow + rr) * 128 + hf * 64 + z) * 4u;
-        const bool live = blk_ok && st * SR + wrow + rr < g.K;
+        const bool live = blk_ok && st * SR + wrow + rr < T_.K;
         if (kind < 2) lds_dma_row(rs_w, row_lds, voff_a[hf], min(row0 + rr, g.K - 1) * ld_bytes);
         else lds_dma_row(rs_x, row_lds + ABUF * 4u, live ? voff_b[hf] : OOB_OFF, tabv[rr]);
     };
@@ -979,7 +1035,7 @@
 #pragma unroll
             for (int q = 0; q < 16; ++q) acc[a][b][q] = 0.f;
 
-    const int nstages = (pa.nblk * KBLK + SR - 1) / SR;
+    const int nstages = (T_.nblk * KBLK + SR - 1) / SR;
     load_table(0);
     pin_table();
 #pragma unroll
@@ -1050,7 +1106,7 @@
         }
         finish_stage();
     };
-    const int nfull = g.K / SR;
+    const int nfull = T_.K / SR;
     int st = 0;
     for (; st + 2 < nfull; st += 2) {
         stage(0, true, st + 1);
@@ -1061,6 +1117,7 @@
         else stage(0, false, st + 1);
     }
 
+    const ConvTile E_ = conv_tile<CLS>(pa, g, tj_blk);
     if (wide) {
         constexpr int SP = BN + 4;
         float* T = ldsc;
@@ -1078,9 +1135,9 @@
         __syncthreads();
         const int px = 4 * (lane & 31);
         const int m = j0 + px;
-        const uint32_t n = fd_div((uint32_t)min(m, pe.M - 1), pe.dOHW);
-        const int p = m - (int)n * pe.OHW;
-        const bool run4 = m + 3 < pe.M && p + 3 < pe.OHW;
+        uint32_t n;
+        int p;
+        const bool run4 = conv_tile_run4<CLS>(E_, pe.dOHW, pe.OHW, m, n, p);
         const int64_t cbase = ((int64_t)n * pe.Cout_total + (int64_t)zg * pe.Cog) * pe.y_plane + p;
 #pragma unroll
         for (int i = 0; i < BM / 8; ++i) {
@@ -1095,9 +1152,9 @@
 #pragma unroll
                 for (int e = 0; e < 4; ++e) {
                     const int me = m + e;
-                    if (me < pe.M) {
-                        const uint32_t ne = fd_div((uint32_t)me, pe.dOHW);
-                        const int pe_ = me - (int)ne * pe.OHW;
+                    if (me < E_.M) {
+                        uint32_t ne, pe_;
+                        conv_tile_pixel<CLS>(E_, pe.dOHW, pe.OHW, (uint32_t)me, ne, pe_);
                         pe.y[((int64_t)ne * pe.Cout_total + (int64_t)zg * pe.Cog + co) * pe.y_plane + pe_] = v[e];
                     }
                 }
@@ -1108,9 +1165,9 @@
 #pragma unroll
     for (int b = 0; b < 2; ++b) {
         const int m = j0 + wn * 64 + 32 * b + (lane & 31);
-        if (m >= pe.M) continue;
-        const uint32_t n = fd_div((uint32_t)m, pe.dOHW);
-        const uint32_t p = m - n * pe.OHW;
+        if (m >= E_.M) continue;
+        uint32_t n, p;
+        conv_tile_pixel<CLS>(E_, pe.dOHW, pe.OHW, (uint32_t)m, n, p);
         const uint32_t oh = fd_div(p, pe.dOW);
         const uint32_t ow = p - oh * pe.OW;
         const int64_t c0 = (int64_t)n * pe.Cout_total + (int64_t)zg * pe.Cog;
@@ -1748,6 +1805,129 @@
     return rc;
 }
 
+static int default_tap_partition(const vl_conv_desc* d, int bwd) {
+    if (!bwd && d->kh * d->kw == 9 && d->cog % 128 == 0) return 0;
+    return 2;
+}
+
+static int build_classes(vl_conv_desc::Classes* c, int part, int kh, int kw, int cg, int H, int W, int halo, int OH, int OW, int pt, int pl) {
+    free_dev(c->dev);
+    memset(c, 0, sizeof(*c));
+    c->ncls = 1;
+    c->nominal = c->executed = (int64_t)OH * OW * kh * kw * ceil_div(cg, KBLK);
+    if (part == 0 || cg % KBLK != 0 || kh * kw == 1 || kh > 32 || kw > 32) return 0;
+    auto masks = [](int O, int I, int k, int pad, uint32_t* mask, int* cls_of, uint32_t* cls_mask) {
+        int n = 0;
+        for (int o = 0; o < O; ++o) {
+            uint32_t m = 0;
+            for (int t = 0; t < k; ++t) if (o - pad + t >= 0 && o - pad + t < I) m |= 1u << t;
+            mask[o] = m;
+            int j = 0;
+            while (j < n && cls_mask[j] != m) ++j;
+            if (j == n) cls_mask[n++] = m;
+            cls_of[o] = j;
+        }
+        return n;
+    };
+    uint32_t* rmask = (uint32_t*)malloc(sizeof(uint32_t) * (2 * OH + 2 * OW));
+    int* rcls = (int*)malloc(sizeof(int) * (OH + OW));
+    if (!rmask || !rcls) { free(rmask); free(rcls); return 1; }
+    uint32_t *rcm = rmask + OH, *cmask = rcm + OH, *ccm = cmask + OW;
+    int* ccls = rcls + OH;
+    const int nr = masks(OH, H, kh, pt, rmask, rcls, rcm);
+    int nc = masks(OW, W, kw, pl, cmask, ccls, ccm);
+    if (part == 2) {
+        nc = 1;
+        ccm[0] = kw == 32 ? 0xffffffffu : (1u << kw) - 1;
+        for (int o = 0; o < OW; ++o) ccls[o] = 0;
+    }
+    const int ncls = nr * nc;
+    if (ncls < 2 || ncls > 64) { free(rmask); free(rcls); return 0; }
+    const int Wp = W + 2 * halo;
+    const int64_t Pp = (int64_t)(H + 2 * halo) * Wp;
+    const int K = kh * kw * cg;
+    auto up64 = [](int64_t v) { return (v + 63) / 64 * 64; };
+    int64_t size = up64((int64_t)ncls * CLS_HDR);
+    const int map_off = (int)size;
+    size += up64((int64_t)OH * OW);
+    int hdr[64][CLS_HDR];
+    for (int ci = 0; ci < ncls; ++ci) {
+        const uint32_t rm = rcm[ci / nc], cm = ccm[ci % nc];
+        int P = 0;
+        for (int oh = 0; oh < OH; ++oh)
+            for (int ow = 0; ow < OW; ++ow) P += rcls[oh] == ci / nc && ccls[ow] == ci % nc;
+        const int ntaps = __builtin_popcount(rm) * __builtin_popcount(cm);
+        const int Kc = ntaps * cg, pad = (Kc + 127) / 128 * 128 + 256;
+        hdr[ci][0] = P;
+        hdr[ci][1] = (int)size; size += up64(P);
+        hdr[ci][2] = (int)size; size += up64(pad);
+        hdr[ci][3] = (int)size; size += up64(pad / KBLK);
+        hdr[ci][4] = Kc;
+        hdr[ci][5] = Kc / KBLK;
+        const FastDiv fd = make_fastdiv((uint32_t)P);
+        hdr[ci][6] = (int)fd.m;
+        hdr[ci][7] = (int)fd.s;
+    }
+    int* h = (int*)calloc((size_t)size, sizeof(int));
+    if (!h) { free(rmask); free(rcls); return 1; }
+    memcpy(h, hdr, sizeof(int) * ncls * CLS_HDR);
+    {
+        int next[64] = {0};
+        for (int e = 0; e < OH * OW; ++e) {
+            int best = -1;
+            for (int ci = 0; ci < ncls; ++ci)
+                if (next[ci] < hdr[ci][0] &&
+                    (best < 0 || (int64_t)(2 * next[ci] + 1) * hdr[best][0] < (int64_t)(2 * next[best] + 1) * hdr[ci][0])) best = ci;
+            h[map_off + e] = best | next[best] << 8;
+            ++next[best];
+        }
+    }
+    int64_t executed = 0;
+    bool ok = true;
+    for (int ci = 0; ci < ncls; ++ci) {
+        const uint32_t rm = rcm[ci / nc], cm = ccm[ci % nc];
+        int* pix = h + hdr[ci][1];
+        int* kt = h + hdr[ci][2];
+        int* rt = h + hdr[ci][3];
+        int np = 0, nb = 0;
+        for (int oh = 0; oh < OH; ++oh)
+            for (int ow = 0; ow < OW; ++ow)
+                if (rcls[oh] == ci / nc && ccls[ow] == ci % nc) {
+                    pix[np++] = oh * OW + ow;
+                    for (int ky = 0; ky < kh; ++ky)
+                        for (int kx = 0; kx < kw; ++kx) {
+                            const int ih = oh - pt + ky, iw = ow - pl + kx;
+                            const bool inplane = ih >= 0 && ih < H && iw >= 0 && iw < W;
+                            const bool kept = (rm >> ky & 1) && (cm >> kx & 1);
+                            if (inplane && !kept) ok = false;
+                            if (kept && (ih + halo < 0 || ih + halo >= H + 2 * halo || iw + halo < 0 || iw + halo >= W + 2 * halo)) ok = false;
+                        }
+                }
+        for (int t = 0; t < K / KBLK; ++t) {
+            int ky, kx, ch;
+            k_to_row(t * KBLK, kh, kw, cg, true, &ky, &kx, &ch);
+            if (!((rm >> ky & 1) && (cm >> kx & 1))) continue;
+            for (int j = 0; j < KBLK; ++j) kt[nb * KBLK + j] = (int)((((int64_t)ch + j) * Pp + (int64_t)ky * Wp + kx) * 4);
+            rt[nb++] = (ky * kw + kx) * cg + ch;
+        }
+        if (np != hdr[ci][0] || nb != hdr[ci][5]) ok = false;
+        executed += (int64_t)np * nb;
+    }
+    free(rmask);
+    free(rcls);
+    if (!ok || executed > c->nominal) {
+        free(h);
+        vl_set_error("build_classes: inconsistent border classes");
+        return 1;
+    }
+    int* dev = nullptr;
+    const int rc = upload(&dev, h, (size_t)size);
+    free(h);
+    if (rc) return rc;
+    c->dev = dev; c->ncls = ncls; c->part = part; c->executed = executed; c->map_off = map_off;
+    return 0;
+}
+
 static int rebuild_tables(vl_conv_desc* d) {
     d->fwd_padded = d->x_halo >= d->pt && d->x_halo >= d->pb && d->x_halo >= d->pl && d->x_halo >= d->pr;
     if (!d->fwd_padded) d->x_phase = 1;
@@ -1761,6 +1941,12 @@
         const int need = (d->kh - 1 - d->pt > d->pt ? d->kh - 1 - d->pt : d->pt);
         const int needw = (d->kw - 1 - d->pl > d->pl ? d->kw - 1 - d->pl : d->pl);
         d->bwd_padded = d->dy_halo >= need && d->dy_halo >= needw;
+    }
+    for (int bwd = 0; bwd < 2 && rc == 0; ++bwd) {
+        const bool on = d->stride == 1 && d->x_phase <= 1 && (bwd ? d->bwd_padded : d->fwd_padded);
+        const int part = !on ? 0 : d->tap_part[bwd] ? d->tap_part[bwd] : default_tap_partition(d, bwd);
+        if (bwd) rc = build_classes(&d->cls[1], part, d->kh, d->kw, d->cog, d->oh, d->ow, d->dy_halo, d->h, d->w, d->kh - 1 - d->pt, d->kw - 1 - d->pl);
+        else rc = build_classes(&d->cls[0], part, d->kh, d->kw, d->cig, d->h, d->w, d->x_halo, d->oh, d->ow, d->pt, d->pl);
     }
     if (rc == 0) rc = conv_c8_build_tables(d);
     return rc;
@@ -1780,6 +1966,7 @@
     d->cog = cout / groups;
     d->K = kh * kw * d->cig;
     d->Kd = kh * kw * d->cog;
+    d->tap_skip = 1;
     const size_t sf = (size_t)groups * ceil_div(d->K, KBLK) * 24 * (ceil_div(d->cog, 128) * 128) * 4;
     const size_t sb = (size_t)groups * ceil_div(d->Kd, KBLK) * 24 * (ceil_div(d->cig, 128) * 128) * 4;
     const bool images = sf <= (64u << 20) && sb <= (64u << 20);
@@ -1810,6 +1997,32 @@
 }
 
 extern "C" int vl_conv_x_phase(const vl_conv_desc* d) { return d && d->x_phase > 1 ? d->x_phase : 1; }
+
+extern "C" int vl_conv_set_tap_skip(vl_conv_desc* d, int mode) {
+    VL_CHECK(d, "vl_conv_set_tap_skip: null descriptor");
+    VL_CHECK(mode >= 0 && mode <= 2, "vl_conv_set_tap_skip: mode %d (0 off, 1 auto, 2 force)", mode);
+    d->tap_skip = mode;
+    return 0;
+}
+
+extern "C" int vl_conv_set_tap_partition(vl_conv_desc* d, int fwd_part, int bwd_part) {
+    VL_CHECK(d, "vl_conv_set_tap_partition: null descriptor");
+    VL_CHECK(fwd_part >= 0 && fwd_part <= 2 && bwd_part >= 0 && bwd_part <= 2, "vl_conv_set_tap_partition: 0 default, 1 rows x columns, 2 rows");
+    d->tap_part[0] = fwd_part; d->tap_part[1] = bwd_part;
+    VL_CHECK(rebuild_tables(d) == 0, "vl_conv_set_tap_partition: device table allocation failed");
+    return 0;
+}
+
+extern "C" int vl_conv_tap_counts(const vl_conv_desc* d, int bwd, int64_t* executed, int64_t* nominal, int* classes, int* partition) {
+    VL_CHECK(d, "vl_conv_tap_counts: null descriptor");
+    const vl_conv_desc::Classes& c = d->cls[bwd ? 1 : 0];
+    const bool on = d->tap_skip != 0 && c.dev;
+    if (executed) *executed = on ? c.executed : c.nominal;
+    if (nominal) *nominal = c.nominal;
+    if (classes) *classes = on ? c.ncls : 1;
+    if (partition) *partition = on ? c.part : 0;
+    return 0;
+}
 
 extern "C" void vl_conv_destroy(vl_conv_desc* d) {
     if (!d) return;
@@ -1823,6 +2036,8 @@
     free_dev(d->rowtab_bwd);
     free_dev(d->wsplit_fwd);
     free_dev(d->wsplit_bwd);
+    free_dev(d->cls[0].dev);
+    free_dev(d->cls[1].dev);
     conv_c8_free_tables(d);
     free(d);
 }
@@ -1865,7 +2080,7 @@
 }
 
 
-template <int TA>
+template <int TA, bool CLS = false>
 __global__ __launch_bounds__(NT, 2) void conv_dma16_kernel(const ConvDmaParams pa, const ConvGeom g, const EpiConvNCHW::Params pe,
                                                            int tiles_i, int wide) {
     constexpr int BM = 16 * TA, BN = 128, SR = 32;
@@ -1878,7 +2093,9 @@
     const int bid = xcd_swizzle(blockIdx.x, gridDim.x);
     const int ti_blk = bid % tiles_i, tj_blk = bid / tiles_i;
     const int zg = blockIdx.y;
-    const int i0 = ti_blk * BM, j0 = tj_blk * BN;
+    const ConvTile T_ = conv_tile<CLS>(pa, g, tj_blk);
+    if (CLS && T_.j0 >= T_.M) return;
+    const int i0 = ti_blk * BM, j0 = T_.j0;
     const int lane = threadIdx.x & 63;
     const int wave = __builtin_amdgcn_readfirstlane(threadIdx.x >> 6);
 
@@ -1894,10 +2111,10 @@
 #pragma unroll
     for (int hf = 0; hf < 2; ++hf) {
         const int m = j0 + hf * 64 + lane;
-        const bool vm = m < g.M;
+        const bool vm = m < T_.M;
         const uint32_t mm = vm ? m : 0;
-        const uint32_t n = fd_div(mm, g.dOHW);
-        const uint32_t p = mm - n * g.OHW;
+        uint32_t n, p;
+        conv_tile_pixel<CLS>(T_, g.dOHW, g.OHW, mm, n, p);
         const uint32_t oh = fd_div(p, g.dOW);
         const uint32_t ow = p - oh * g.OW;
         const int ih0 = (int)oh * g.stride - g.pt + g.halo, iw0 = (int)ow * g.col_mul + g.col_add;
@@ -1920,11 +2137,11 @@
     const int wrow = wave * RW;
     auto load_table = [&](int st) {
         const int k0 = st * SR + wrow;
-        const const_int_ptr tt = as_const(g.ktab) + k0 + st * g.zero;
+        const const_int_ptr tt = T_.ktab + k0 + st * g.zero;
 #pragma unroll
         for (int f = 0; f < RW; ++f) tabv[f] = tt[f];
-        row0 = as_const(pa.row_tab)[k0 / KBLK + st * g.zero] + k0 % KBLK;
-        blk_ok = k0 / KBLK < pa.nblk;
+        row0 = T_.rtab[k0 / KBLK + st * g.zero] + k0 % KBLK;
+        blk_ok = k0 / KBLK < T_.nblk;
     };
     auto pin_table = [&]() {
 #pragma unroll
@@ -1934,7 +2151,7 @@
     auto dma = [&](const int nb, const int f, int st) {
         const int rr = f / FPR, kind = f % FPR;
         const int z = st * g.zero;
-        const bool live = blk_ok && st * SR + wrow + rr < g.K;
+        const bool live = blk_ok && st * SR + wrow + rr < T_.K;
         if (kind < NA) {
             lds_dma_row(rs_w, lds0 + (uint32_t)(nb * BUF + (wrow + rr) * SA + kind * 64 + z) * 4u, voff_a[kind],
                         min(row0 + rr, g.K - 1) * ld_bytes);
@@ -1970,7 +2187,7 @@
 #pragma unroll
             for (int q = 0; q < 4; ++q) acc[a][b][q] = 0.f;
 
-    const int nstages = (pa.nblk * KBLK + SR - 1) / SR;
+    const int nstages = (T_.nblk * KBLK + SR - 1) / SR;
     load_table(0);
     pin_table();
 #pragma unroll
@@ -2028,8 +2245,8 @@
         }
         finish_stage();
     };
-    const int nfull = g.K / SR;
-    const int last_steps = (g.K - (nstages - 1) * SR + 3) / 4;
+    const int nfull = T_.K / SR;
+    const int last_steps = (T_.K - (nstages - 1) * SR + 3) / 4;
     int st = 0;
     for (; st + 2 < nfull; st += 2) {
         stage(0, true, st + 1, NSTEP);
@@ -2041,6 +2258,7 @@
         else stage(0, false, st + 1, ns);
     }
 
+    const ConvTile E_ = conv_tile<CLS>(pa, g, tj_blk);
     if (wide) {
         constexpr int SP = BN + 4;
         float* T = ldsc;
@@ -2057,9 +2275,9 @@
         __syncthreads();
         const int px = 4 * (lane & 31);
         const int m = j0 + px;
-        const uint32_t n = fd_div((uint32_t)min(m, pe.M - 1), pe.dOHW);
-        const int p = m - (int)n * pe.OHW;
-        const bool run4 = m + 3 < pe.M && p + 3 < pe.OHW;
+        uint32_t n;
+        int p;
+        const bool run4 = conv_tile_run4<CLS>(E_, pe.dOHW, pe.OHW, m, n, p);
         const int64_t cbase = ((int64_t)n * pe.Cout_total + (int64_t)zg * pe.Cog) * pe.y_plane + p;
 #pragma unroll
         for (int i = 0; i < BM / 8; ++i) {
@@ -2074,9 +2292,9 @@
 #pragma unroll
                 for (int e = 0; e < 4; ++e) {
                     const int me = m + e;
-                    if (me < pe.M) {
-                        const uint32_t ne = fd_div((uint32_t)me, pe.dOHW);
-                        const int pe_ = me - (int)ne * pe.OHW;
+                    if (me < E_.M) {
+                        uint32_t ne, pe_;
+                        conv_tile_pixel<CLS>(E_, pe.dOHW, pe.OHW, (uint32_t)me, ne, pe_);
                         pe.y[((int64_t)ne * pe.Cout_total + (int64_t)zg * pe.Cog + co) * pe.y_plane + pe_] = v[e];
                     }
                 }
@@ -2087,9 +2305,9 @@
 #pragma unroll
     for (int b = 0; b < 2; ++b) {
         const int m = j0 + wave * 32 + 16 * b + (lane & 15);
-        if (m >= pe.M) continue;
-        const uint32_t n = fd_div((uint32_t)m, pe.dOHW);
-        const uint32_t p = m - n * pe.OHW;
+        if (m >= E_.M) continue;
+        uint32_t n, p;
+        conv_tile_pixel<CLS>(E_, pe.dOHW, pe.OHW, (uint32_t)m, n, p);
         const uint32_t oh = fd_div(p, pe.dOW);
         const uint32_t ow = p - oh * pe.OW;
         const int64_t c0 = (int64_t)n * pe.Cout_total + (int64_t)zg * pe.Cog;
@@ -2124,35 +2342,46 @@
 
 static int device_cus();
 
+static int conv_pixel_tiles(const ConvGeom& g, const vl_conv_desc::Classes* cls) {
+    if (!cls || !cls->dev) return ceil_div(g.M, 128);
+    return ceil_div(g.M / g.OHW, CLS_GROUP) * g.OHW;
+}
+
 template <int BM>
 static int launch_conv_dma(const ConvGeom& g, const float* w, int64_t w_ld, int w_grp_stride, const int* row_tab, int Cog,
-                           int Cout_total, const ConvOut& o, hipStream_t s) {
+                           int Cout_total, const ConvOut& o, hipStream_t s, const vl_conv_desc::Classes* cls = nullptr) {
     constexpr int BN = 128, SR = 32;
     constexpr size_t lds = BM == 128 ? (size_t)BM * (BN + 4) * sizeof(float)
                                      : (size_t)2 * SR * ((BM + 63) / 64 * 64 + 16 + 144) * sizeof(float);
     static_assert(BM != 128 || (size_t)2 * SR * (BM + BN) * sizeof(float) <= (size_t)BM * (BN + 4) * sizeof(float), "stage buffers fit");
-    ConvDmaParams pa{w, w_ld, (int64_t)w_grp_stride, (int64_t)g.K * w_ld * 4, row_tab, ceil_div(g.K, KBLK)};
+    const int nimg = g.M / g.OHW;
+    if (cls && !cls->dev) cls = nullptr;
+    ConvDmaParams pa{w, w_ld, (int64_t)w_grp_stride, (int64_t)g.K * w_ld * 4, row_tab, ceil_div(g.K, KBLK), cls ? cls->dev : nullptr,
+                     cls ? cls->map_off : 0, nimg};
     EpiConvNCHW::Params pe;
     pe.y = o.y; pe.bias = o.bias; pe.mask = o.mask; pe.relu = o.relu;
     pe.Cog = Cog; pe.Cout_total = Cout_total; pe.OHW = g.OHW; pe.OW = g.OW; pe.M = g.M;
     pe.dOHW = g.dOHW; pe.dOW = g.dOW;
     pe.y_halo = o.y_halo; pe.y_wp = o.OW + 2 * o.y_halo; pe.y_plane = (int64_t)(o.OH + 2 * o.y_halo) * pe.y_wp;
     pe.m_halo = o.m_halo; pe.m_wp = o.OW + 2 * o.m_halo; pe.m_plane = (int64_t)(o.OH + 2 * o.m_halo) * pe.m_wp;
-    static bool attr_set = false;
-    if (!attr_set) {
+    static bool attr_set[2] = {false, false};
+    const int v = cls ? 1 : 0;
+    if (!attr_set[v]) {
         const void* kern;
-        if constexpr (BM == 128) kern = reinterpret_cast<const void*>(conv_dma_kernel<SR>);
-        else kern = reinterpret_cast<const void*>(conv_dma16_kernel<BM / 16>);
+        if constexpr (BM == 128) kern = cls ? reinterpret_cast<const void*>(conv_dma_kernel<SR, true>) : reinterpret_cast<const void*>(conv_dma_kernel<SR, false>);
+        else kern = cls ? reinterpret_cast<const void*>(conv_dma16_kernel<BM / 16, true>) : reinterpret_cast<const void*>(conv_dma16_kernel<BM / 16, false>);
         VL_HIP(hipFuncSetAttribute(kern, hipFuncAttributeMaxDynamicSharedMemorySize, (int)lds));
-        attr_set = true;
-    }
-    const int tiles_i = ceil_div(Cog, BM), tiles_j = ceil_div(g.M, BN);
+        attr_set[v] = true;
+    }
+    const int tiles_i = ceil_div(Cog, BM), tiles_j = conv_pixel_tiles(g, cls);
     dim3 grid(tiles_i * tiles_j, (unsigned)(Cout_total / Cog), 1);
     const int wide = (o.y_halo == 0 && !o.mask && !kConvNoWideStore && (size_t)BM * (BN + 4) * sizeof(float) <= lds) ? 1 : 0;
     if constexpr (BM == 128) {
-        hipLaunchKernelGGL(conv_dma_kernel<SR>, grid, dim3(NT), lds, s, pa, g, pe, tiles_i, wide);
+        if (cls) hipLaunchKernelGGL((conv_dma_kernel<SR, true>), grid, dim3(NT), lds, s, pa, g, pe, tiles_i, wide);
+        else hipLaunchKernelGGL((conv_dma_kernel<SR, false>), grid, dim3(NT), lds, s, pa, g, pe, tiles_i, wide);
     } else {
-        hipLaunchKernelGGL((conv_dma16_kernel<BM / 16>), grid, dim3(NT), lds, s, pa, g, pe, tiles_i, wide);
+        if (cls) hipLaunchKernelGGL((conv_dma16_kernel<BM / 16, true>), grid, dim3(NT), lds, s, pa, g, pe, tiles_i, wide);
+        else hipLaunchKernelGGL((conv_dma16_kernel<BM / 16, false>), grid, dim3(NT), lds, s, pa, g, pe, tiles_i, wide);
     }
     VL_LAUNCH_CHECK();
     return 0;
@@ -2205,14 +2434,17 @@
 
 template <bool PADDED>
 static int dispatch_conv(const ConvGeom& g, const float* w, int64_t w_ld, int w_grp_stride, const int* row_tab, int Cog,
-                         int Cout_total, const ConvOut& o, uint32_t* wsplit, hipStream_t s) {
+                         int Cout_total, const ConvOut& o, uint32_t* wsplit, hipStream_t s, const vl_conv_desc::Classes* cls, int tap_skip) {
+    const vl_conv_desc::Classes* cls_many = (PADDED && tap_skip >= 1 && cls && cls->dev) ? cls : nullptr;
+    const vl_conv_desc::Classes* cls_few = tap_skip == 2 ? cls_many : nullptr;
     const int w128 = ceil_div(Cog, 128) * 128, w96 = ceil_div(Cog, 96) * 96, w64 = ceil_div(Cog, 64) * 64;
     if (g_conv_math != 0 && PADDED && g.col_mul == 1 && wsplit != nullptr) {
         if (Cog >= 96) return launch_conv_ring<128>(g, w, w_ld, w_grp_stride, row_tab, Cog, Cout_total, o, wsplit, s);
         if (Cog >= 40 && Cog <= 64) return launch_conv_ring<64>(g, w, w_ld, w_grp_stride, row_tab, Cog, Cout_total, o, wsplit, s);
     }
-    const int64_t px = ceil_div(g.M, 128), cus = device_cus(), ngrp = Cout_total / Cog;
-    const bool few = px * ceil_div(Cog, 128) * ngrp < 8 * cus;
+    const int64_t cus = device_cus(), ngrp = Cout_total / Cog;
+    const bool few = (int64_t)ceil_div(g.M, 128) * ceil_div(Cog, 128) * ngrp < 8 * cus;
+    const int64_t px = conv_pixel_tiles(g, cls_few);
     if (PADDED && few && (int64_t)g.K * w_ld * 4 < MAX_BUF_BYTES && !kConvStaged && !kConvNoLoadPick) {
         const int widths[3] = {128, 96, 48};
         auto pick = [&](int64_t pxt, int64_t& load) {
@@ -2224,16 +2456,16 @@
             return b;
         };
         auto run = [&](int wi, const ConvGeom& gg, const ConvOut& oo) {
-            if (wi == 0) return launch_conv_dma<128>(gg, w, w_ld, w_grp_stride, row_tab, Cog, Cout_total, oo, s);
-            if (wi == 1) return launch_conv_dma<96>(gg, w, w_ld, w_grp_stride, row_tab, Cog, Cout_total, oo, s);
-            return launch_conv_dma<48>(gg, w, w_ld, w_grp_stride, row_tab, Cog, Cout_total, oo, s);
+            if (wi == 0) return launch_conv_dma<128>(gg, w, w_ld, w_grp_stride, row_tab, Cog, Cout_total, oo, s, cls_few);
+            if (wi == 1) return launch_conv_dma<96>(gg, w, w_ld, w_grp_stride, row_tab, Cog, Cout_total, oo, s, cls_few);
+            return launch_conv_dma<48>(gg, w, w_ld, w_grp_stride, row_tab, Cog, Cout_total, oo, s, cls_few);
         };
         int64_t best_load = 0;
         const int best = pick(px, best_load);
         const int nimg = g.M / g.OHW;
         const int64_t wgs_per_px = (int64_t)ceil_div(Cog, widths[best]) * ngrp;
         const int64_t rounds = px * wgs_per_px / cus;
-        if (rounds >= 6 && !kConvNoTailSplit) {
+        if (rounds >= 6 && !kConvNoTailSplit && !cls_few) {
             const int64_t px_a = rounds * cus / wgs_per_px;
             const int n_a = (int)(px_a * 128 / g.OHW);
             const int n_b = nimg - n_a;
@@ -2258,16 +2490,16 @@
     }
     if (w128 <= w96 && w128 <= w64) {
         if (PADDED && (int64_t)g.K * w_ld * 4 < MAX_BUF_BYTES && !kConvStaged) {
-            return launch_conv_dma<128>(g, w, w_ld, w_grp_stride, row_tab, Cog, Cout_total, o, s);
+            return launch_conv_dma<128>(g, w, w_ld, w_grp_stride, row_tab, Cog, Cout_total, o, s, cls_many);
         }
         return launch_conv<128, 2, 2, PADDED>(g, w, w_ld, w_grp_stride, row_tab, Cog, Cout_total, o, s);
     }
     if (PADDED && ceil_div(Cog, 48) * 48 < w64 && ceil_div(Cog, 48) * 48 < w96 &&
         (int64_t)g.K * w_ld * 4 < MAX_BUF_BYTES && !kConvStaged)
-        return launch_conv_dma<48>(g, w, w_ld, w_grp_stride, row_tab, Cog, Cout_total, o, s);
+        return launch_conv_dma<48>(g, w, w_ld, w_grp_stride, row_tab, Cog, Cout_total, o, s, cls_many);
     if (w96 <= w64) {
         if (PADDED && (int64_t)g.K * w_ld * 4 < MAX_BUF_BYTES && !kConvStaged)
-            return launch_conv_dma<96>(g, w, w_ld, w_grp_stride, row_tab, Cog, Cout_total, o, s);
+            return launch_conv_dma<96>(g, w, w_ld, w_grp_stride, row_tab, Cog, Cout_total, o, s, cls_many);
         return launch_conv<96, 1, 4, PADDED>(g, w, w_ld, w_grp_stride, row_tab, Cog, Cout_total, o, s);
     }
     return launch_conv<64, 1, 4, PADDED>(g, w, w_ld, w_grp_stride, row_tab, Cog, Cout_total, o, s);
@@ -2298,8 +2530,8 @@
               d->x_phase > 1 ? d->x_phase : 1);
     VL_CHECK(g.total * 4 < MAX_BUF_BYTES, "vl_conv_fwd: input of %lld elements exceeds the buffer-offset range", (long long)g.total);
     ConvOut o{y, bias, nullptr, relu, d->y_halo, 0, d->oh, d->ow};
-    if (d->fwd_padded) return dispatch_conv<true>(g, w, d->cout, d->cog, d->rowtab_fwd, d->cog, d->cout, o, d->wsplit_fwd, (hipStream_t)stream);
-    return dispatch_conv<false>(g, w, d->cout, d->cog, d->rowtab_fwd, d->cog, d->cout, o, d->wsplit_fwd, (hipStream_t)stream);
+    if (d->fwd_padded) return dispatch_conv<true>(g, w, d->cout, d->cog, d->rowtab_fwd, d->cog, d->cout, o, d->wsplit_fwd, (hipStream_t)stream, &d->cls[0], d->tap_skip);
+    return dispatch_conv<false>(g, w, d->cout, d->cog, d->rowtab_fwd, d->cog, d->cout, o, d->wsplit_fwd, (hipStream_t)stream, &d->cls[0], d->tap_skip);
 }
 
 __global__ __launch_bounds__(256) void conv_wt_transpose_kernel(const float* __restrict__ w, float* __restrict__ wt, int KH, int KW,
@@ -2345,8 +2577,8 @@
               d->ptab_bwd, d->ptab2_bwd);
     VL_CHECK(g.total * 4 < MAX_BUF_BYTES, "vl_conv_dgrad: dy of %lld elements exceeds the buffer-offset range", (long long)g.total);
     ConvOut o{dx, nullptr, relu_mask, 0, d->dx_halo, d->x_halo, d->h, d->w};
-    if (d->bwd_padded) return dispatch_conv<true>(g, wt, d->cin, d->cig, d->rowtab_bwd, d->cig, d->cin, o, d->wsplit_bwd, (hipStream_t)stream);
-    return dispatch_conv<false>(g, wt, d->cin, d->cig, d->rowtab_bwd, d->cig, d->cin, o, d->wsplit_bwd, (hipStream_t)stream);
+    if (d->bwd_padded) return dispatch_conv<true>(g, wt, d->cin, d->cig, d->rowtab_bwd, d->cig, d->cin, o, d->wsplit_bwd, (hipStream_t)stream, &d->cls[1], d->tap_skip);
+    return dispatch_conv<false>(g, wt, d->cin, d->cig, d->rowtab_bwd, d->cig, d->cin, o, d->wsplit_bwd, (hipStream_t)stream, &d->cls[1], d->tap_skip);
 }
 
 static void dy_params(const vl_conv_desc* d, const ConvGeom& g, const float* dy, DyParams& pb) {
diff --git a/video-learning-tf_amd/ops.py b/video-learning-tf_amd/ops.py
--- a/video-learning-tf_amd/ops.py
+++ b/video-learning-tf_amd/ops.py
@@ -94,6 +94,17 @@
         _ffi.call("vl_conv_set_x_phase_split", self._d, int(on))
         self.x_phase = int(_ffi.lib().vl_conv_x_phase(self._d))
         return self.x_phase
+
+    def set_tap_skip(self, mode=1):
+        _ffi.call("vl_conv_set_tap_skip", self._d, int(mode))
+
+    def set_tap_partition(self, fwd=0, bwd=0):
+        _ffi.call("vl_conv_set_tap_partition", self._d, int(fwd), int(bwd))
+
+    def tap_counts(self, bwd=False):
+        ex, nom, ncls, part = C.c_int64(), C.c_int64(), C.c_int(), C.c_int()
+        _ffi.call("vl_conv_tap_counts", self._d, int(bwd), C.byref(ex), C.byref(nom), C.byref(ncls), C.byref(part))
+        return ex.value, nom.value, ncls.value, part.value
 
     def _shape(self, n, c, h, w, halo):
         return (n, c, h + 2 * halo, w + 2 * halo)
```

Result: no change. 1893 clips/s (median of 6 runs) (+0.8%).
